# wenet-e2e/wesep

Measured on AMD Instinct MI355X. Metric: utterances/sec (4 s, 16 kHz, 2-spk) fwd+bwd, pBSRNN, higher is better.
Workload: dtype bf16x3+fp16x2+fp16x1 split products (+fp8 lo terms), fp32 accumulate; 1 GPU; pBSRNN FiLM multi-fuse, 6 repeats, feature_dim 128, fixed 256-d embeddings; fwd + SI-SDR + bwd + per-tensor clip + Adam-L2; bf16x3 (x-projections, projections, d(hcat), BN / mask GEMMs) + fp16x2 (recurrent products of all four recurrence kernels, d(xn)) + fp16x1 (LSTM weight gradients); 2-byte saved gates / d(gates); fp32 accumulate; BPTT kernels: W_hh as fp16 hi + block-scaled FP8 lo; the lo term; rows_per_gpu=32, global_rows=32, samples_per_row=64000, parallelism=dp1

## Files before the change

### include/wesep_hip.h

```cpp
#ifndef WESEP_HIP_H_
#define WESEP_HIP_H_

#ifdef __cplusplus
extern "C" {
#endif

#define WS_ABI_VERSION 20
#define WS_OK 0
#define WS_ERR_INVALID (-1)
#define WS_ERR_LAUNCH (-2)

int ws_abi_version(void);
const char* ws_last_error(void);

#define WS_PROF_LSTM_FWD 0
#define WS_PROF_LSTM_BWD 1
#define WS_PROF_GEMM_NT 2
#define WS_PROF_GEMM_TN 3
#define WS_PROF_NKINDS 4
int ws_prof_enable(int on);
int ws_prof_collect(int kind, double* total_ms, long long* launches);
int ws_debug_dirty_lds(float value, int nblocks, int spins, float* sink, void* stream);
int ws_debug_occupy(int nblocks, int usec, const unsigned* stop, float* sink, void* stream);

// ... 28 lines not shown
  const float* stats;
  const float* gamma;
  const float* beta;
  const ws_group_nt* groups;
  long long a_s1, a_s2, c_s1, c_s2, st_m1, st_m2, st_base;
  int a_div, c_div, st_div1, st_div2;
  int M, N, K, ldw;
  int act, ngroups, max_n, vec;
  ws_conv_view conv;
} ws_gemm_nt_args;
int ws_gemm_nt(const ws_gemm_nt_args* a, void* stream);

typedef struct ws_group_tn {
  const float* gamma;
  const float* beta;
  long long g_off, a_off, st_base, out_off, bout_off;
  int Nn, Kk, pad0_, pad1_;
} ws_group_tn;

typedef struct ws_gemm_tn_args {
  const float* G;
  const float* A;
  float* slab;
  float* bslab;
  const float* stats;
  const float* gamma;
  const float* beta;
  const ws_group_tn* groups;
  long long g_s1, g_s2, a_s1, a_s2, st_m1, st_m2, st_base;
  long long slab_stride, bslab_stride, out_off, bout_off;
  int g_div, a_div, st_div1, st_div2;
  int M, Nn, Kk, rows_per_split, nsplit;
  int shift_rows, seq_div, seq_len;
  int ngroups, max_n, max_k, vec;
  ws_conv_view conv;
} ws_gemm_tn_args;
int ws_gemm_tn(const ws_gemm_tn_args* a, void* stream);

typedef struct ws_conv_wgrad_args {
  const float* G;
  const float* X;
  float* slab;
  float* bslab;
  long long ldg, slab_stride, bslab_stride;
  int M, Nn, nsplit, tiles_per_split;
  ws_conv_view conv;
} ws_conv_wgrad_args;
int ws_conv_wgrad(const ws_conv_wgrad_args* a, void* stream);

int ws_reduce_slabs(const float* slab, int nsplit, long long stride, long long count,
                    float* out, int w, long long ldo, void* stream);

int ws_transpose(const float* src, int rows, int cols, long long lds, float* dst, void* stream);

typedef struct ws_groups_geom {
  const int* band_w;
  const int* band_off;
  long long gs1, gs2, rs;
  int ngroups, gdiv, L, W;
  int nbands, pad_;
} ws_groups_geom;
int ws_group_stats(const float* x, const ws_groups_geom* geo, float eps, float* stats, void* stream);
int ws_group_stats_len(const float* x, const ws_groups_geom* geo, const int* glen, int glen_div, float eps, float* stats,
                       void* stream);

int ws_gn_bwd_reduce(const float* x, const float* dxn, const float* stats, const float* gamma,
                     const float* const* gamma_tab, const ws_groups_geom* geo, float* ab,
                     void* stream);
int ws_gn_bwd_apply(const float* x, const float* dxn, const float* stats, const float* ab,
                    const float* gamma, const float* const* gamma_tab, const float* res,
                    const ws_groups_geom* geo, float* dx, void* stream);
int ws_gn_param_grad(const float* x, const float* dxn, const float* stats,
                     const ws_groups_geom* geo, int nsplit, float* slab, void* stream);

int ws_gn_bwd_fused(const float* x, const float* dxn, const float* stats, const float* gamma,
                    const float* res, const ws_groups_geom* geo, int nwg, float* dx, float* pslab,
                    float* pout, unsigned* counter, void* stream);
int ws_gn_bwd_fused2(const float* x, const float* dxn, const float* dxn2, const float* stats, const float* gamma,
                     const float* res, const ws_groups_geom* geo, int nwg, float* dx, float* pslab,
                     float* pout, unsigned* counter, void* stream);
int ws_gn_bwd_apply_pg(const float* x, const float* dxn, const float* stats, const float* ab,
                       const float* gamma, const float* res, const ws_groups_geom* geo, float* dx,
                       float* pslab, float* pout, unsigned* counter, void* stream);

typedef struct ws_lstm_args {
  float* gates;
  float* cbuf;
  float* hcat;
  const float* dhcat;
  const float* wpack;
  long long sq_s1, sq_s2, step_rows;
  int nseq, sq_div, L, mode;
  const unsigned* run_if;
  const float* gates_in;
  float* dgates;
  int gfmt;
  int rfmt;
  const unsigned* amax;
  float* dxn;
  long long dxn_dir_stride;
  const float* wxpack;
} ws_lstm_args;
#define WS_GATES_F32 0
#define WS_GATES_H2 1
#define WS_GATES_H2S 2
#define WS_GATES_H2F 3
#define WS_DGATES_EXP 8
#define WS_LSTM_F32_MT1 1
#define WS_LSTM_F32_MT2 2
#define WS_LSTM_BF16X3 3
#define WS_LSTM_BF16X3_BLK 4
#define WS_LSTM_BF16X3_BLK16 5
#define WS_LSTM_H 256
#define WS_LSTM_FWD_H2P 16
#define WS_LSTM_PACK_FLOATS (2 * 4 * WS_LSTM_H * WS_LSTM_H)
int ws_lstm_pack(const float* whh_f, const float* whh_r, float* pack_fwd, float* pack_bwd,
                 int mode, void* stream);
int ws_lstm_pack_bwd_f8(const float* whh_f, const float* whh_r, float* pack_bwd, void* stream);
#define WS_LSTM_DX_PACK_FLOATS (16 * (48 * 1024 + 64) / 4)
int ws_lstm_pack_dx_f8(const float* wcat, float* pack, void* stream);
int ws_lstm_fwd(const ws_lstm_args* a, void* stream);
int ws_lstm_bwd(const ws_lstm_args* a, void* stream);
typedef struct ws_lstm_cluster_args {
  float* gates;
  float* cbuf;
  float* hcat;
  const float* dhcat;
  const float* whh_f;
  const float* whh_r;
  void* xchg;
  unsigned* flags;
  unsigned* status;
  int nseq, L;
  int dbg, gfmt;
  const float* gates_in;
} ws_lstm_cluster_args;
int ws_lstm_fwd_cluster(const ws_lstm_cluster_args* a, void* stream);
typedef struct ws_lstm_cluster2_args {
  float* gates;
  float* cbuf;
  float* hcat;
  const float* xn;
  const float* wcat;
  const float* bcat;
  const float* whh_f;
  const float* whh_r;
  void* xchg;
  unsigned* tword;
  unsigned* status;
  int nseq, L;
  int dbg, rfmt;
  float* dbg_buf;
} ws_lstm_cluster2_args;
int ws_lstm_fwd_cluster2(const ws_lstm_cluster2_args* a, void* stream);
int ws_lstm_bwd_cluster(const ws_lstm_cluster_args* a, void* stream);
typedef struct ws_lstm_pair_args {
  float* gates;
  const float* cbuf;
  const float* dhcat;
  const float* wpack;
  void* xchg;
  unsigned* flags;
  unsigned* status;
  float* dbg_buf;
  int nseq, L;
  int dbg, gfmt;
  float* dgates;
  const unsigned* amax;
  int rfmt, pad_;
} ws_lstm_pair_args;
int ws_lstm_pack_pair(const float* whh_f, const float* whh_r, float* pack, void* stream);
int ws_lstm_pack_pair_f16(const float* whh_f, const float* whh_r, float* pack, void* stream);
int ws_lstm_pack_pair_f8(const float* whh_f, const float* whh_r, float* pack, void* stream);
int ws_lstm_pack_pair_f8mx(const float* whh_f, const float* whh_r, float* pack, void* stream);
int ws_lstm_bwd_pair(const ws_lstm_pair_args* a, void* stream);
int ws_lstm_cat_ih(const float* wih_f, const float* wih_r, const float* bih_f, const float* bhh_f,
                   const float* bih_r, const float* bhh_r, int n_in, float* wcat, float* bcat,
                   void* stream);

typedef struct ws_seqmap {
  long long sq_s1, sq_s2, step_rows;
  int nseq, sq_div, L;
  int nvalid;
} ws_seqmap;

int ws_pack_w(const float* W, int N, int K, long long ldw, int trans, int order, float* out,
              void* stream);
int ws_pack_w_f16(const float* W, int N, int K, long long ldw, int trans, int order, float* out,
                  void* stream);
int ws_pack_w_f16f8(const float* W, int N, int K, long long ldw, int trans, float* out, void* stream);

typedef struct ws_gemm_p2b_args {
  const float* A;
  const float* Wpack;
  const float* bias;
  float* C;
  float* A_bl;
  const float* stats;
  const float* gamma;
  const float* beta;
  ws_seqmap sm;
  long long lda, st_m1, st_m2, st_base;
  int st_div1, st_div2, N, K;
  const unsigned* run_if;
  unsigned* amax;
  void* A_bl16;
} ws_gemm_p2b_args;
int ws_gemm_p2b(const ws_gemm_p2b_args* a, void* stream);
int ws_gemm_p2b_len(const ws_gemm_p2b_args* a, const int* steps, int steps_div, void* stream);

typedef struct ws_gemm_b2p_args {
  const float* A;
  const float* Wpack;
  const float* bias;
  const float* R;
  float* C;
  ws_seqmap sm;
  long long ldc;
  int N, K;
  int a_fmt, pad_;
  const unsigned* amax;
  void* a16_out;
} ws_gemm_b2p_args;
int ws_gemm_b2p(const ws_gemm_b2p_args* a, void* stream);

typedef struct ws_gemm_tnb_args {
  const float* G;
  const float* A0;
  const float* A1;
  float* slab;
  float* bslab;
  float* aslab;
  long long slab_stride, bslab_stride, aslab_stride;
  int g_width, g_off, g_cols;
  int a0_width, a0_off, a0_cols, a0_shift;
  int a1_width, a1_off, a1_cols, a1_shift;
  int nblk, L, nsplit, blocks_per_split;
  int g_fmt;
  const unsigned* amax;
  int a_fmt, pad_;
} ws_gemm_tnb_args;
int ws_gemm_tnb(const ws_gemm_tnb_args* a, void* stream);
int ws_gemm_tnb_h16(const ws_gemm_tnb_args* a, void* stream);

typedef struct ws_bands {
  const int* band_of_bin;
  const int* band_f0;
  const int* band_bw;
  int nband, nbins;
} ws_bands;
int ws_stft_bandsplit(const float* wav, int R, int T, const ws_bands* b, float* xbs, void* stream);
int ws_stft_bandsplit_len(const float* wav, int R, int T, const int* lengths, const ws_bands* b, float* xbs, void* stream);
int ws_mask_istft_frames(const float* xbs, const float* mask3, int R, int Tf, const ws_bands* b,
                         float* frames, void* stream);
int ws_istft_ola(const float* frames, int R, int Tf, int T, float* wav, void* stream);
int ws_istft_ola_len(const float* frames, int R, int Tf, int T, const int* lengths, float* wav, void* stream);
int ws_mask_istft_bwd(const float* dwav, const float* xbs, const float* mask3, int R, int Tf,
                      int T, const ws_bands* b, float* dmask3, void* stream);

int ws_affine_fwd(const float* z, const float* a, const float* b, float a0, long long rows,
                  int rows_per_r, int N, float* out, void* stream);
int ws_affine_bwd(const float* dz, const float* z_in, const float* a, float a0, long long rows,
                  int rows_per_r, int N, int nsplit, float* dz_in, float* da_slab, float* db_slab,
                  float* da, float* db, unsigned* counter, void* stream);

int ws_sisdr_fwd(const float* est, const float* tgt, int R, int T, float eps, float* rowstat,
                 float* loss, void* stream);
int ws_sisdr_bwd(const float* est, const float* tgt, const float* rowstat, const float* gout,
                 int R, int T, float* dest, void* stream);

typedef struct ws_tensor_ref {
  float* param;
  float* grad;
  float* exp_avg;
  float* exp_avg_sq;
  long long numel;
} ws_tensor_ref;
int ws_grad_norms(const ws_tensor_ref* tab, int ntensors, float* norms, unsigned* guard, void* stream);
int ws_guard_commit(unsigned* guard, const unsigned* skip1, void* stream);
int ws_clip_adam_step(const ws_tensor_ref* tab, int ntensors, const float* norms, float clip,
                      float lr, float beta1, float beta2, float eps, float weight_decay, int step,
                      int clip_only, const unsigned* skip0, const unsigned* skip1, const unsigned* step_lag,
                      void* stream);


int ws_flat_stats(const float* x, int ngroups, long long n_per_group, float eps, int nchunk,
                  float* scratch, float* stats, void* stream);
int ws_prelu_fwd(float* x, const float* rb, const float* a, long long rows, int C, int rows_per_r,
                 float* y, void* stream);
int ws_prelu_bwd(const float* pre, const float* dy, const float* a, long long n, float* dx, float* slab,
                 int nslab, void* stream);
int ws_dwconv_fwd(const float* x, const float* stats, const float* gamma, const float* beta,
                  const float* w, const float* b, int R, int Tp, int C, int P, int dil, int st_div,
                  float* y, void* stream);
int ws_dwconv_bwd(const float* dy, const float* x, const float* stats, const float* gamma,
                  const float* beta, const float* w, int R, int Tp, int C, int P, int dil, int st_div,
                  float* dxn, int nsplit, int rows_per_split, float* slab, void* stream);
int ws_dwconv_ex_fwd(const float* x, const float* stats, const float* gamma, const float* beta,
                     const float* w, const float* b, int R, int Tp, int C, int P, int dil, int st_div, int causal,
                     float* y, void* stream);
int ws_dwconv_ex_bwd(const float* dy, const float* x, const float* stats, const float* gamma,
                     const float* beta, const float* w, int R, int Tp, int C, int P, int dil, int st_div, int causal,
                     float* dxn, int nsplit, int rows_per_split, float* slab, void* stream);
int ws_chan_sums(const float* g, const float* x, const float* stats, int st_div, int rows_per_group,
                 int ngroups, int nsplit, int C, float* slab, void* stream);
int ws_norm_ab(const float* sums, const float* gamma, int ngroups, int C, long long n_per_group,
               float* ab, void* stream);
// ... 271 lines not shown
```

### wesep_amd/_lib.py

```python
import ctypes as C
import os

import numpy as np
import torch

_HERE = os.path.dirname(os.path.abspath(__file__))
LIB_PATH = os.environ.get("WESEP_HIP_LIB") or os.path.join(_HERE, "libwesep_hip.so")

WS_OK = 0
PROF_LSTM_FWD, PROF_LSTM_BWD, PROF_GEMM_NT, PROF_GEMM_TN = 0, 1, 2, 3
LSTM_H = 256
ABI_VERSION = 20
GATES_F32, GATES_H2, GATES_H2S, GATES_H2F = 0, 1, 2, 3
DGATES_EXP = 8


def dgates_scale(amax_bits: int) -> float:
    e = (int(amax_bits) >> 23) & 0xFF
    return 1.0 if e in (0, 255) else 2.0 ** (min(max(DGATES_EXP + 254 - e, 1), 253) - 127)


LSTM_F32_MT1, LSTM_F32_MT2, LSTM_BF16X3, LSTM_BF16X3_BLK, LSTM_BF16X3_BLK16 = 1, 2, 3, 4, 5
LSTM_FWD_H2P = 16
LSTM_PACK_FLOATS = 2 * 4 * LSTM_H * LSTM_H

_p = C.c_void_p
_ll = C.c_longlong
_i = C.c_int
_f = C.c_float


class ConvView(C.Structure):
    _fields_ = [(n, _i) for n in ("on", "mode", "H", "W", "C", "Ho", "Wo", "k", "sh", "sw", "p", "dil", "ldp")]


class Conv3x3PackSrc(C.Structure):
    _fields_ = [("w", _p), ("s_row", _ll), ("s_col", _ll), ("s_tap", _ll), ("col_off", _i), ("cols", _i)]


class Conv3x3PackArgs(C.Structure):
    _fields_ = [("src", Conv3x3PackSrc * 5), ("out", _p), ("Cin", _i), ("Cout", _i), ("nsrc", _i), ("flip", _i)]


class Conv3x3Args(C.Structure):
    _fields_ = [(n, _p) for n in ("X", "W", "bias", "R", "Y")] + [(n, _ll) for n in ("ldx", "ldw", "ldy")] + \
               [(n, _i) for n in ("B", "H", "Wd", "Cin", "Cout", "pad_")]


class Conv3x3WgradArgs(C.Structure):
    _fields_ = [(n, _p) for n in ("G", "X", "slab", "bslab")] + [(n, _ll) for n in ("ldg", "ldx", "slab_stride", "bslab_stride")] + \
               [(n, _i) for n in ("B", "H", "Wd", "Wx", "sw", "Cin", "Nn", "nsplit", "tiles_per_split", "pad_")]


class HeadsArgs(C.Structure):
    _fields_ = [(n, _p) for n in ("x", "dy", "slope", "gamma", "beta", "y", "stats", "dx", "slab")] + \
               [(n, _ll) for n in ("ldx", "lddx")] + [(n, _i) for n in ("B", "T", "Tp", "Q", "nh", "ch", "nwg")] + \
               [("eps", C.c_float)]


class GemmNTArgs(C.Structure):
    _fields_ = [(n, _p) for n in ("A", "W", "bias", "C", "R", "T", "stats", "gamma", "beta", "groups")] + \
               [(n, _ll) for n in ("a_s1", "a_s2", "c_s1", "c_s2", "st_m1", "st_m2", "st_base")] + \
               [(n, _i) for n in ("a_div", "c_div", "st_div1", "st_div2", "M", "N", "K", "ldw",
                                  "act", "ngroups", "max_n", "vec")] + [("conv", ConvView)]


class GemmTNArgs(C.Structure):
    _fields_ = [(n, _p) for n in ("G", "A", "slab", "bslab", "stats", "gamma", "beta", "groups")] + \
               [(n, _ll) for n in ("g_s1", "g_s2", "a_s1", "a_s2", "st_m1", "st_m2", "st_base",
                                   "slab_stride", "bslab_stride", "out_off", "bout_off")] + \
               [(n, _i) for n in ("g_div", "a_div", "st_div1", "st_div2", "M", "Nn", "Kk",
                                  "rows_per_split", "nsplit", "shift_rows", "seq_div", "seq_len",
                                  "ngroups", "max_n", "max_k", "vec")] + [("conv", ConvView)]


class ConvWgradArgs(C.Structure):
    _fields_ = [(n, _p) for n in ("G", "X", "slab", "bslab")] + \
               [(n, _ll) for n in ("ldg", "slab_stride", "bslab_stride")] + \
               [(n, _i) for n in ("M", "Nn", "nsplit", "tiles_per_split")] + [("conv", ConvView)]


class GroupsGeom(C.Structure):
    _fields_ = [("band_w", _p), ("band_off", _p), ("gs1", _ll), ("gs2", _ll), ("rs", _ll),
                ("ngroups", _i), ("gdiv", _i), ("L", _i), ("W", _i), ("nbands", _i), ("pad_", _i)]


class LstmArgs(C.Structure):
    _fields_ = [(n, _p) for n in ("gates", "cbuf", "hcat", "dhcat", "wpack")] + \
               [(n, _ll) for n in ("sq_s1", "sq_s2", "step_rows")] + \
               [(n, _i) for n in ("nseq", "sq_div", "L", "mode")] + [("run_if", _p)] + \
               [("gates_in", _p), ("dgates", _p), ("gfmt", _i), ("rfmt", _i), ("amax", _p)] + \
               [("dxn", _p), ("dxn_dir_stride", _ll), ("wxpack", _p)]


class SeqMapC(C.Structure):
    _fields_ = [("sq_s1", _ll), ("sq_s2", _ll), ("step_rows", _ll), ("nseq", _i), ("sq_div", _i), ("L", _i), ("nvalid", _i)]


class GemmP2BArgs(C.Structure):
    _fields_ = [(n, _p) for n in ("A", "Wpack", "bias", "C", "A_bl", "stats", "gamma", "beta")] + \
               [("sm", SeqMapC)] + [(n, _ll) for n in ("lda", "st_m1", "st_m2", "st_base")] + \
               [(n, _i) for n in ("st_div1", "st_div2", "N", "K")] + [("run_if", _p), ("amax", _p), ("A_bl16", _p)]


class GemmB2PArgs(C.Structure):
    _fields_ = [(n, _p) for n in ("A", "Wpack", "bias", "R", "C")] + [("sm", SeqMapC), ("ldc", _ll), ("N", _i), ("K", _i),
                                                                         ("a_fmt", _i), ("pad_", _i), ("amax", _p), ("a16_out", _p)]


class GemmTNBArgs(C.Structure):
    _fields_ = [(n, _p) for n in ("G", "A0", "A1", "slab", "bslab", "aslab")] + \
               [(n, _ll) for n in ("slab_stride", "bslab_stride", "aslab_stride")] + \
               [(n, _i) for n in ("g_width", "g_off", "g_cols", "a0_width", "a0_off", "a0_cols", "a0_shift",
                                  "a1_width", "a1_off", "a1_cols", "a1_shift", "nblk", "L", "nsplit",
                                  "blocks_per_split", "g_fmt")] + [("amax", _p), ("a_fmt", _i), ("pad_", _i)]


class LstmClusterArgs(C.Structure):
    _fields_ = [(n, _p) for n in ("gates", "cbuf", "hcat", "dhcat", "whh_f", "whh_r", "xchg", "flags", "status")] + \
               [("nseq", _i), ("L", _i), ("dbg", _i), ("gfmt", _i), ("gates_in", _p)]


class LstmCluster2Args(C.Structure):
    _fields_ = [(n, _p) for n in ("gates", "cbuf", "hcat", "xn", "wcat", "bcat", "whh_f", "whh_r", "xchg", "tword", "status")] + \
               [("nseq", _i), ("L", _i), ("dbg", _i), ("rfmt", _i), ("dbg_buf", _p)]


class LstmPairArgs(C.Structure):
    _fields_ = [(n, _p) for n in ("gates", "cbuf", "dhcat", "wpack", "xchg", "flags", "status", "dbg_buf")] + \
               [("nseq", _i), ("L", _i), ("dbg", _i), ("gfmt", _i), ("dgates", _p), ("amax", _p), ("rfmt", _i), ("pad_", _i)]


class Bands(C.Structure):
    _fields_ = [("band_of_bin", _p), ("band_f0", _p), ("band_bw", _p), ("nband", _i), ("nbins", _i)]


GROUP_NT_DTYPE = np.dtype([("W", "<u8"), ("bias", "<u8"), ("gamma", "<u8"), ("beta", "<u8"),
                           ("a_off", "<i8"), ("c_off", "<i8"), ("st_base", "<i8"),
                           ("K", "<i4"), ("N", "<i4"), ("ldw", "<i4"), ("pad_", "<i4")])
GROUP_TN_DTYPE = np.dtype([("gamma", "<u8"), ("beta", "<u8"), ("g_off", "<i8"), ("a_off", "<i8"),
                           ("st_base", "<i8"), ("out_off", "<i8"), ("bout_off", "<i8"),
                           ("Nn", "<i4"), ("Kk", "<i4"), ("pad0_", "<i4"), ("pad1_", "<i4")])
TENSOR_REF_DTYPE = np.dtype([("param", "<u8"), ("grad", "<u8"), ("exp_avg", "<u8"),
                             ("exp_avg_sq", "<u8"), ("numel", "<i8")])
assert GROUP_NT_DTYPE.itemsize == 72 and GROUP_TN_DTYPE.itemsize == 72 and TENSOR_REF_DTYPE.itemsize == 40

class LstmFusedArgs(C.Structure):
    _fields_ = [("gates", _p), ("cbuf", _p), ("hcat", _p), ("xn", _p), ("wpack", _p), ("bias", _p),
                ("nseq", _i), ("L", _i), ("gfmt", _i), ("hfmt", _i)]


LSTM_FUSED_PACK_FLOATS = 2 * 8 * 24 * 4 * 2 * 64 * 4
LSTM_DX_PACK_FLOATS = 16 * (48 * 1024 + 64) // 4

_SIGS = {
    "ws_abi_version": (_i, []),
    "ws_last_error": (C.c_char_p, []),
    "ws_prof_enable": (_i, [_i]),
    "ws_prof_collect": (_i, [_i, C.POINTER(C.c_double), C.POINTER(_ll)]),
    "ws_debug_dirty_lds": (_i, [_f, _i, _i, _p, _p]),
    "ws_debug_occupy": (_i, [_i, _i, _p, _p, _p]),
    "ws_pack_w_f16": (_i, [_p, _i, _i, _ll, _i, _i, _p, _p]),
    "ws_pack_w_f16f8": (_i, [_p, _i, _i, _ll, _i, _p, _p]),
    "ws_gemm_nt": (_i, [C.POINTER(GemmNTArgs), _p]),
    "ws_gemm_tn": (_i, [C.POINTER(GemmTNArgs), _p]),
    "ws_reduce_slabs": (_i, [_p, _i, _ll, _ll, _p, _i, _ll, _p]),
    "ws_transpose": (_i, [_p, _i, _i, _ll, _p, _p]),
    "ws_group_stats": (_i, [_p, C.POINTER(GroupsGeom), _f, _p, _p]),
    "ws_group_stats_len": (_i, [_p, C.POINTER(GroupsGeom), _p, _i, _f, _p, _p]),
    "ws_gn_bwd_reduce": (_i, [_p, _p, _p, _p, _p, C.POINTER(GroupsGeom), _p, _p]),
    "ws_gn_bwd_apply": (_i, [_p, _p, _p, _p, _p, _p, _p, C.POINTER(GroupsGeom), _p, _p]),
    "ws_gn_param_grad": (_i, [_p, _p, _p, C.POINTER(GroupsGeom), _i, _p, _p]),
    "ws_gn_bwd_fused": (_i, [_p, _p, _p, _p, _p, C.POINTER(GroupsGeom), _i, _p, _p, _p, _p, _p]),
    "ws_gn_bwd_fused2": (_i, [_p, _p, _p, _p, _p, _p, C.POINTER(GroupsGeom), _i, _p, _p, _p, _p, _p]),
    "ws_gn_bwd_apply_pg": (_i, [_p, _p, _p, _p, _p, _p, C.POINTER(GroupsGeom), _p, _p, _p, _p, _p]),
    "ws_lstm_pack": (_i, [_p, _p, _p, _p, _i, _p]),
    "ws_lstm_fwd": (_i, [C.POINTER(LstmArgs), _p]),
    "ws_lstm_bwd": (_i, [C.POINTER(LstmArgs), _p]),
    "ws_lstm_fwd_cluster": (_i, [C.POINTER(LstmClusterArgs), _p]),
    "ws_lstm_bwd_cluster": (_i, [C.POINTER(LstmClusterArgs), _p]),
    "ws_lstm_fwd_cluster2": (_i, [C.POINTER(LstmCluster2Args), _p]),
    "ws_lstm_pack_pair": (_i, [_p, _p, _p, _p]),
    "ws_lstm_pack_pair_f16": (_i, [_p, _p, _p, _p]),
    "ws_lstm_pack_pair_f8": (_i, [_p, _p, _p, _p]),
    "ws_lstm_pack_pair_f8mx": (_i, [_p, _p, _p, _p]),
    "ws_lstm_pack_bwd_f8": (_i, [_p, _p, _p, _p]),
    "ws_lstm_pack_dx_f8": (_i, [_p, _p, _p]),
    "ws_lstm_bwd_pair": (_i, [C.POINTER(LstmPairArgs), _p]),
    "ws_lstm_cat_ih": (_i, [_p, _p, _p, _p, _p, _p, _i, _p, _p, _p]),
    "ws_pack_w": (_i, [_p, _i, _i, _ll, _i, _i, _p, _p]),
    "ws_gemm_p2b": (_i, [C.POINTER(GemmP2BArgs), _p]),
    "ws_gemm_p2b_len": (_i, [C.POINTER(GemmP2BArgs), _p, _i, _p]),
    "ws_gemm_b2p": (_i, [C.POINTER(GemmB2PArgs), _p]),
    "ws_gemm_tnb": (_i, [C.POINTER(GemmTNBArgs), _p]),
    "ws_gemm_tnb_h16": (_i, [C.POINTER(GemmTNBArgs), _p]),
    "ws_stft_bandsplit": (_i, [_p, _i, _i, C.POINTER(Bands), _p, _p]),
    "ws_stft_bandsplit_len": (_i, [_p, _i, _i, _p, C.POINTER(Bands), _p, _p]),
    "ws_mask_istft_frames": (_i, [_p, _p, _i, _i, C.POINTER(Bands), _p, _p]),
    "ws_istft_ola": (_i, [_p, _i, _i, _i, _p, _p]),
    "ws_istft_ola_len": (_i, [_p, _i, _i, _i, _p, _p, _p]),
    "ws_mask_istft_bwd": (_i, [_p, _p, _p, _i, _i, _i, C.POINTER(Bands), _p, _p]),
    "ws_affine_fwd": (_i, [_p, _p, _p, _f, _ll, _i, _i, _p, _p]),
    "ws_affine_bwd": (_i, [_p, _p, _p, _f, _ll, _i, _i, _i, _p, _p, _p, _p, _p, _p, _p]),
    "ws_sisdr_fwd": (_i, [_p, _p, _i, _i, _f, _p, _p, _p]),
    "ws_sisdr_bwd": (_i, [_p, _p, _p, _p, _i, _i, _p, _p]),
    "ws_flat_stats": (_i, [_p, _i, _ll, C.c_float, _i, _p, _p, _p]),
    "ws_prelu_fwd": (_i, [_p, _p, _p, _ll, _i, _i, _p, _p]),
    "ws_prelu_bwd": (_i, [_p, _p, _p, _ll, _p, _p, _i, _p]),
    "ws_dwconv_fwd": (_i, [_p, _p, _p, _p, _p, _p, _i, _i, _i, _i, _i, _i, _p, _p]),
    "ws_dwconv_bwd": (_i, [_p, _p, _p, _p, _p, _p, _i, _i, _i, _i, _i, _i, _p, _i, _i, _p, _p]),
    "ws_dwconv_ex_fwd": (_i, [_p, _p, _p, _p, _p, _p, _i, _i, _i, _i, _i, _i, _i, _p, _p]),
    "ws_dwconv_ex_bwd": (_i, [_p, _p, _p, _p, _p, _p, _i, _i, _i, _i, _i, _i, _i, _p, _i, _i, _p, _p]),
    "ws_chan_sums": (_i, [_p, _p, _p, _i, _i, _i, _i, _i, _p, _p]),
    "ws_norm_ab": (_i, [_p, _p, _i, _i, _ll, _p, _p]),
    "ws_norm_bwd_apply_cl": (_i, [_p, _p, _p, _p, _p, _p, _ll, _i, _i, _p, _p]),
    "ws_maskmul_fwd": (_i, [_p, _ll, _p, _ll, _i, _p, _p]),
    "ws_maskmul_bwd": (_i, [_p, _p, _ll, _p, _ll, _i, _p, _ll, _p, _p]),
    "ws_relu_mask": (_i, [_p, _p, _ll, _p]),
    "ws_ola_fwd": (_i, [_p, _p, _i, _i, _i, _i, _i, _p, _p]),
    "ws_ola_bwd": (_i, [_p, _i, _i, _i, _i, _i, _p, _p]),
    "ws_sum_partial": (_i, [_p, _ll, _p, _i, _p]),
    "ws_bn_stats": (_i, [_p, _ll, _i, C.c_float, C.c_float, _p, _p, _i, _p, _p, _p]),
    "ws_bn_prelu_fwd": (_i, [_p, _p, _p, _p, _p, _p, _ll, _i, _p, _p, _p]),
    "ws_bn_bwd": (_i, [_p, _p, _p, _p, _ll, _i, _i, _p, _p, _p, _p]),
    "ws_maxpool3_fwd": (_i, [_p, _i, _i, _i, _p, _p]),
    "ws_maxpool3_bwd": (_i, [_p, _p, _i, _i, _i, _p, _p]),
    "ws_bcast_rows": (_i, [_p, C.c_float, _i, _ll, _i, _p, _p]),
    "ws_cross_entropy": (_i, [_p, _p, _i, _i, _p, _p, _p]),
    "ws_im2col": (_i, [_p, _i, _i, _i, _i, _i, _i, _i, _ll, _p, _p]),
    "ws_col2im": (_i, [_p, _i, _i, _i, _i, _i, _i, _i, _p, _p]),
    "ws_conv_wgrad": (_i, [C.POINTER(ConvWgradArgs), _p]),
    "ws_astp_fwd": (_i, [_p, _p, _i, _i, _i, C.c_float, _p, _p, _p]),
    "ws_astp_bwd": (_i, [_p, _p, _p, _p, _p, _i, _i, _i, C.c_float, _p, _p, _p]),
    "ws_mhastp_sizes": (_i, [_i, _i, _i, _i, _i, _i, _i, _p, _p]),
    "ws_mhastp_pack": (_i, [_p, _p, _p, _p, _i, _i, _i, _i, _p, _p]),
    "ws_mhastp_fwd": (_i, [_p, _p, _i, _i, _i, _i, _i, _i, _i, _i, _p, _p, _p]),
    "ws_mhastp_bwd": (_i, [_p, _p, _p, _p, _i, _i, _i, _i, _i, _i, _i, _i, _p, _p, _p, _i, _p, _p]),
    "ws_mhastp_split_sizes": (_i, [_i, _i, _i, _i, _i, _i, _i, _p, _p]),
    "ws_mhastp_fwd_split": (_i, [_p, _p, _i, _i, _i, _i, _i, _i, _i, _i, _i, _p, _p, _p, _p]),
    "ws_mhastp_bwd_split": (_i, [_p, _p, _p, _p, _i, _i, _i, _i, _i, _i, _i, _i, _i, _p, _p, _p, _i, _p, _p]),
    "ws_rowbias_act_fwd": (_i, [_p, _p, _ll, _i, _i, _i, _p, _p]),
    "ws_act_bwd": (_i, [_p, _p, _ll, _i, _p, _p]),
    "ws_seg_sums": (_i, [_p, _p, _i, _i, _i, _i, _p, _p]),
    "ws_seg_scale": (_i, [_p, _p, _i, _i, _i, _i, _p, _p]),
    "ws_tstp_fwd": (_i, [_p, _i, _i, _i, _i, C.c_float, _p, _p]),
    "ws_tstp_bwd": (_i, [_p, _p, _p, _i, _i, _i, _i, _p, _p]),
    "ws_im2col_hw": (_i, [_p, _i, _i, _i, _i, _i, _i, _i, _i, _ll, _p, _p]),
    "ws_col2im_hw": (_i, [_p, _i, _i, _i, _i, _i, _i, _i, _i, _p, _p]),
    "ws_elu_fwd": (_i, [_p, _ll, _p, _p]),
    "ws_elu_bwd": (_i, [_p, _p, _ll, _p, _p]),
    "ws_inorm_finalize": (_i, [_p, _i, _i, _ll, C.c_float, _p, _p]),
    "ws_inorm_apply": (_i, [_p, _p, _ll, _i, _i, _p, _p]),
    "ws_inorm_bwd_apply": (_i, [_p, _p, _p, _p, _ll, _i, _i, _p, _p]),
    "ws_avgpool_fwd": (_i, [_p, _i, _i, _i, _i, _i, _p, _p]),
    "ws_avgpool_bwd": (_i, [_p, _i, _i, _i, _i, _i, _p, _p]),
    "ws_bilinear_fwd": (_i, [_p, _i, _i, _i, _i, _i, _i, _p, _p]),
    "ws_bilinear_bwd": (_i, [_p, _i, _i, _i, _i, _i, _i, _p, _p, _p]),
    "ws_scale_bf_fwd": (_i, [_p, _p, _i, _i, _i, _i, _i, _p, _p]),
    "ws_freq_linear_fwd": (_i, [_p, _p, _ll, _p, _i, _i, _i, _i, _p, _p]),
    "ws_scale_bf_bwd": (_i, [_p, _p, _p, _i, _i, _i, _i, _i, _p, _p, _p]),
    "ws_softmax_rows_fwd": (_i, [_p, _ll, _i, C.c_float, _p, _p]),
    "ws_softmax_rows_bwd": (_i, [_p, _p, _ll, _i, C.c_float, _p, _p]),
    "ws_heads_fwd": (_i, [C.POINTER(HeadsArgs), _p]),
    "ws_heads_bwd": (_i, [C.POINTER(HeadsArgs), _p]),
    "ws_conv3x3": (_i, [C.POINTER(Conv3x3Args), _p]),
    "ws_conv3x3_pack": (_i, [C.POINTER(Conv3x3PackArgs), _p]),
    "ws_conv3x3_wgrad": (_i, [C.POINTER(Conv3x3WgradArgs), _p]),
    "ws_in_act_sums": (_i, [_p, _p, _ll, _p, _i, _i, _i, _i, _i, _p, _p]),
    "ws_in_act_apply": (_i, [_p, _p, _ll, _i, _i, _i, _p, _ll, _p]),
    "ws_in_act_bwd_apply": (_i, [_p, _p, _ll, _p, _p, _ll, _i, _i, _i, _p, _ll, _p]),
    "ws_rowln_grid": (_i, [_ll, _i]),
    "ws_rowln_fwd": (_i, [_p, _p, _p, _ll, _i, C.c_float, _p, _p, _p]),
    "ws_rowln_bwd": (_i, [_p, _p, _p, _p, _p, _ll, _i, _p, _p, _p]),
    "ws_preemph_pad": (_i, [_p, _i, _i, _i, _i, C.c_float, _p, _p]),
    "ws_power_spec": (_i, [_p, _ll, _i, _i, _i, _p, _p]),
    "ws_log_eps": (_i, [_p, _ll, C.c_float, _p]),
# ... 101 lines not shown
```

### wesep_amd/blstm_core.py

```python
import math
import os
from typing import NamedTuple

import numpy as np
import torch

from . import _lib as L
from . import dev

H = L.LSTM_H
G4 = 4 * H
N = 128


def _empty(dev_, *shape):
    return torch.empty(*shape, device=dev_, dtype=torch.float32)


def _reduce_new(slab, nsplit, stride, shape):
    out = _empty(slab.device, *shape)
    dev.reduce_slabs(slab, nsplit, stride, int(np.prod(shape)), out)
    return out


# ... 282 lines not shown
            return pack
        if kind in ("hhp", "hhp16"):
            pack = _empty(d, L.LSTM_PACK_FLOATS)
            dev.lstm_pack_pair(*W("whh"), pack, f16=pair_rf if kind == "hhp16" else 0)
            return pack
        if kind in ("fused", "fused16", "fused8"):
            fpack = _empty(d, L.LSTM_FUSED_PACK_FLOATS)
            dev.lstm_pack_fused(wih_f.contiguous(), wih_r.contiguous(), *W("whh"), fpack,
                                hfmt={"fused": 0, "fused16": 1, "fused8": 5}[kind])
            return fpack
        if kind == "wih":
            out = _empty(d, 2 * G4 * N)
            dev.pack_w(W("cat")[0], 2 * G4, N, N, out, order=0)
            return out
        if kind in ("wihT", "wihT16", "wihT8"):
            out = _empty(d, N * 2 * G4)
            dev.pack_w(W("cat")[0], N, 2 * G4, N, out, trans=True, order=1, f16={"wihT": 0, "wihT16": 1, "wihT8": 2}[kind])
            return out
        if kind == "pw":
            return proj_w.contiguous()
        if kind in ("proj", "proj16"):
            out = _empty(d, N * 2 * H)
            dev.pack_w(W("pw"), N, 2 * H, 2 * H, out, order=1, f16=kind == "proj16")
            return out
        if kind == "projT":
            out = _empty(d, 2 * H * N)
            dev.pack_w(W("pw"), 2 * H, N, 2 * H, out, trans=True, order=0)
            return out
        raise KeyError(kind)


class BlstmPlan(NamedTuple):
    nb: int
    lmode: int
    cluster: bool
    fwd: str
    bptt: str
    grad: bool
    gfmt: int
    g_fmt: int
    a16: bool
    pair_rfmt: int
    band_rfmt: int
    band_dx: bool
    a_fmt: int
    h2p: bool = False


_WIHT_KIND = {0: "wihT", 1: "wihT", 2: "wihT16", 3: "wihT8"}


def make_plan(seq, device, grad, gn_geo=None, ragged=False) -> BlstmPlan:
    lmode = dev.lstm_blk_mode(seq.nseq)
    cluster = dev.lstm_cluster_ok(seq, device)
    bptt = _bptt_kind(seq, device, cluster)
    gfmt = L.GATES_F32 if bptt == "cluster" else dev.gates_fmt()
    h2 = gfmt != L.GATES_F32
    if ragged:
        fwd = "cluster" if cluster else "stream"
    elif dev.lstm_fuse_ok(seq.nseq, cluster):
        fwd = "fused"
    elif cluster:
        fwd = "cluster2" if h2 and dev.lstm_cluster2_on() else "cluster"
    else:
        fwd = "stream"
    g_fmt = {L.GATES_H2: 1, L.GATES_H2F: 2}.get(gfmt, 0)
    brf = band_rfmt(gfmt, lmode) if grad and bptt == "stream" else 0
    a16 = gfmt == L.GATES_H2F and grad and tnb_a16()
    h2p = (a16 and dev.h2p_on(device) and not ragged and fwd in ("fused", "cluster2", "stream")
           and (fwd != "fused" or bool(dev.lstm_fused_hfmt(gfmt) & 1)))
    return BlstmPlan(
        nb=dev.bl_num_blocks(seq), lmode=lmode, cluster=cluster, fwd=fwd, bptt=bptt, grad=grad, gfmt=gfmt, g_fmt=g_fmt,
        a16=a16, pair_rfmt=pair_rfmt(gfmt) if grad and bptt == "pair" else 0,
        band_rfmt=brf, band_dx=bool(brf) and gn_geo is not None and band_dx(brf, seq, gn_geo), a_fmt=dxn_fmt(g_fmt), h2p=h2p)


def consume_once(ctx, who):
    if ctx.consumed:
        raise L.WesepHipError(f"{who}: second backward through the same graph (retain_graph / multi-loss loops): "
                              "the blocked path consumes its saved gates in place; run the forward again")
    ctx.consumed = True


def blstm_forward(plan, W, x, seq, res, bias, norm=None, steps=None):
    d = x.device
    norm = norm or {}
    if steps is not None and (plan.fwd in ("fused", "cluster2") or plan.grad):
        raise L.WesepHipError(f"blstm_forward: per-sequence step counts with forward branch '{plan.fwd}', grad={plan.grad}: "
                              "only the branches over precomputed gates know them, and only the forward")
    lens = dict(steps=steps[0], steps_div=steps[1]) if steps is not None else {}
    nb, gfmt, lmode = plan.nb, plan.gfmt, plan.lmode
    h2 = gfmt != L.GATES_F32
    wcat, bcat = W("cat")
    whf, whr = W("whh")
    xn = _empty(d, nb, 32 * N)
    cbuf, hcat = _empty(d, nb, 32 * 2 * H), _empty(d, nb, 32 * 2 * H)
    gates = _empty(d, dev.blh_floats(nb, 2 * G4)) if h2 else _empty(d, nb, 32 * 2 * G4)
    xn16 = _empty(d, dev.blh_floats(nb, N)) if plan.a16 else None
    h2p = plan.h2p
    planes = dict(h2p=True) if h2p else {}
    hcat16 = _empty(d, dev.blh_floats(nb, 2 * H)) if plan.a16 and not h2p else None
    if plan.fwd == "fused":
        dev.gemm_p2b(A=x, lda=N, sm=seq, Wpack=None, N=0, C_out=None, A_bl=xn, A_bl16=xn16, **norm)
        hf = dev.lstm_fused_hfmt(gfmt)
        dev.lstm_fwd_fused(gates, cbuf, hcat, xn, W("fused8" if hf & 4 else "fused16" if hf else "fused"), bcat, seq, gfmt=gfmt,
                           hfmt=hf | (8 if h2p else 0))
    elif plan.fwd == "cluster2":
        dev.gemm_p2b(A=x, lda=N, sm=seq, Wpack=None, N=0, C_out=None, A_bl=xn, A_bl16=xn16, **norm)
        tw = dev.lstm_fwd_cluster2(gates, cbuf, hcat, xn, wcat, bcat, whf, whr, seq, dbg=_cluster_dbg(), **planes)
        pre = dev.fallback_scratch(d, nb * 32 * 2 * G4)
        dev.gemm_p2b(A=x, lda=N, sm=seq, Wpack=W("wih"), N=2 * G4, C_out=pre, bias=bcat, run_if=tw, **norm)
        dev.lstm_fwd(gates, cbuf, hcat, W("hh")[0], seq, lmode, run_if=tw, gfmt=gfmt, gates_in=pre, **planes)
        del pre
    else:
        pre = _empty(d, nb, 32 * 2 * G4) if h2 else gates
        xproj = dict(A=x, lda=N, sm=seq, Wpack=W("wih"), N=2 * G4, C_out=pre, bias=bcat, A_bl=xn, A_bl16=xn16, **norm, **lens)
        rec = dict(gfmt=gfmt, gates_in=pre) if h2 else {}
        dev.gemm_p2b(**xproj)
        if _h2_probe() & 768 and not torch.cuda.is_available():
            pre.copy_(pre.half().float() if _h2_probe() & 256 else pre.bfloat16().float())
        if plan.fwd == "cluster":
            tw = dev.lstm_fwd_cluster(gates, cbuf, hcat, whf, whr, seq, dbg=_cluster_dbg(), **rec)
            if not h2:
                dev.gemm_p2b(run_if=tw, **xproj)
            dev.lstm_fwd(gates, cbuf, hcat, W("hh")[0], seq, lmode, run_if=tw, **rec)
        else:
            dev.lstm_fwd(gates, cbuf, hcat, W("hh")[0], seq, lmode, **planes, **rec)
        del pre
    out = torch.empty_like(res)
    if h2p:
        dev.gemm_b2p(A=hcat, K=2 * H, sm=seq, Wpack=W("proj16"), C_out=out, ldc=N, bias=bias, R=res, a_fmt=4)
    else:
        dev.gemm_b2p(A=hcat, K=2 * H, sm=seq, Wpack=W("proj"), C_out=out, ldc=N, bias=bias, R=res, a16_out=hcat16)
    if _h2_probe() and not h2:
        if _h2_probe() & 1:
            _probe_round(gates, "f16")
        if _h2_probe() & 8:
            _probe_round(gates, "u16")
        if _h2_probe() & 4:
            _probe_round(cbuf, "f16")
    if plan.grad:
        W("projT")
        if not plan.band_dx:
            W(_WIHT_KIND[plan.a_fmt])
        if plan.bptt == "pair":
            W("hhp16" if plan.pair_rfmt else "hhp")
        if (plan.bptt == "stream" and not plan.band_rfmt) or (plan.bptt == "pair" and h2):
            W("hh")
        if plan.bptt == "stream" and plan.band_rfmt:
            W("hh8")
            if plan.band_dx:
                W("wx8")
    return out, (gates, cbuf, hcat, xn16 if plan.a16 else xn, hcat16)


def blstm_bptt(plan, W, gates, cbuf, hcat, dout, seq, release):
    d = dout.device
    nb, gfmt = plan.nb, plan.gfmt
    dh, dout_bl = _empty(d, nb, 32 * 2 * H), _empty(d, nb, 32 * N)
    dxn2 = None
    amax = amax_word(d) if gfmt == L.GATES_H2F else None
    dev.gemm_p2b(A=dout, lda=N, sm=seq, Wpack=W("projT"), N=2 * H, C_out=dh, A_bl=dout_bl, amax=amax)
    if _h2_probe() & 16:
        _probe_round(dh, "bf16")
    ready = mark_wgrads_ready(d) if release else None
    if plan.bptt == "cluster":
        dg = gates
        dev.lstm_bwd_cluster(gates, cbuf, dh, *W("whh"), seq)
    elif gfmt == L.GATES_F32:
        dg = gates
        if plan.bptt == "pair":
            dev.lstm_bwd_pair(gates, cbuf, dh, W("hhp"), seq, dbg=_pair_dbg())
        else:
            dev.lstm_bwd(gates, cbuf, hcat, dh, W("hh")[1], seq, plan.lmode)
    elif plan.bptt == "pair":
        dg = _empty(d, nb, 32 * 2 * G4) if gfmt == L.GATES_H2S else _empty(d, dev.blh_floats(nb, 2 * G4))
        rf = plan.pair_rfmt
        tw = dev.lstm_bwd_pair(gates, cbuf, dh, W("hhp16" if rf else "hhp"), seq, gfmt=gfmt, dgates=dg, repairable=True,
                               dbg=_pair_dbg(), amax=amax, rfmt=rf, dbg_buf=_pair_stamp_buf(d, seq.L))
        dev.lstm_bwd(gates, cbuf, hcat, dh, W("hh")[1], seq, plan.lmode, gfmt=gfmt, dgates=dg, run_if=tw, amax=amax)
    else:
        dg = _empty(d, nb, 32 * 2 * G4) if gfmt == L.GATES_H2S else gates
        brf = plan.band_rfmt
        if plan.band_dx:
            dxn2 = _empty(d, 2, dout.numel() // N, N)
        dev.lstm_bwd(gates, cbuf, hcat, dh, W("hh8") if brf else W("hh")[1], seq, plan.lmode, gfmt=gfmt,
                     dgates=dg if gfmt == L.GATES_H2S else None, amax=amax, rfmt=brf, dxn=dxn2,
                     wxpack=W("wx8") if dxn2 is not None else None)
    if _h2_probe() & 2 and gfmt == L.GATES_F32:
        _probe_round(gates, "bf16", packed=True)
    if _h2_probe() & 32 and gfmt == L.GATES_F32 and not torch.cuda.is_available():
        amax = float(dh.abs().max())
        S = 2.0 ** (10 - math.floor(math.log2(amax))) if amax > 0 and math.isfinite(amax) else 1.0
        sc = gates * S
        _PROBE_SAT[0] += int((sc.abs() > 65504.0).sum())
        _PROBE_SAT[1] = max(_PROBE_SAT[1], float(sc.abs().max()) / 65504.0)
        gates.copy_(sc.clamp(-65504.0, 65504.0).half().float() / S)
    if ready is not None:
        flush_deferred_wgrads(d, ready)
    return dg, dout_bl, amax, dxn2


def weight_grads(gates, xn, hcat, dout_bl, seq, nb, g_fmt=0, amax=None, hcat16=None, h2p=False):
    d = gates.device
    if h2p:
        hcat16 = dev.h2p_hi(hcat, nb)
    a_fmt = 1 if hcat16 is not None else 0
    if _h2_probe() & 192 and not torch.cuda.is_available() and not a_fmt:
        rnd = (lambda t: t.half().float()) if _h2_probe() & 64 else (lambda t: t.bfloat16().float())
        xn, hcat = rnd(xn), rnd(hcat)
    if os.environ.get("WESEP_PROBE_SKIP_WGRAD") == "1":
        z_ = lambda *s_: torch.zeros(*s_, device=d)
        return [z_(G4, N), z_(G4, H), z_(G4), z_(G4), z_(G4, N), z_(G4, H), z_(G4), z_(G4), z_(N, 2 * H), z_(N)]
    if _h2_probe() & 1024 and not torch.cuda.is_available() and amax is not None:
        S = L.dgates_scale(int(amax.reshape(-1)[0]))
        hcat = hcat.half().float()
# ... 50 lines not shown
```

### wesep_amd/csrc/common.h

```cpp
#pragma once
#include <hip/hip_runtime.h>
#include <stdint.h>

#include "../../include/wesep_hip.h"

typedef float f32x4 __attribute__((ext_vector_type(4)));
typedef float f32x16 __attribute__((ext_vector_type(16)));

#define WS_WAVE 64

#define WS_SEL_LO16 0x05040100u
#define WS_SEL_HI16 0x07060302u

void ws_set_error(const char* fmt, ...);
int ws_check_launch(const char* what);

#define WS_REQUIRE(cond, ...)            \
  do {                                   \
    if (!(cond)) {                       \
      ws_set_error(__VA_ARGS__);         \
      return WS_ERR_INVALID;             \
    }                                    \
  } while (0)

void ws_prof_begin(int kind, hipStream_t s);
void ws_prof_end(int kind, hipStream_t s);

int ws_launch_gemm_nt_bf16(const ws_gemm_nt_args* a, dim3 grid, hipStream_t s);
int ws_launch_gemm_tn_bf16(const ws_gemm_tn_args* a, dim3 grid, hipStream_t s);

int ws_launch_lstm_pack_bf16(const float* whh_f, const float* whh_r, float* pack_fwd, float* pack_bwd,
                             hipStream_t s);
int ws_launch_lstm_fwd_bf16(const ws_lstm_args* a, hipStream_t s);
int ws_launch_lstm_bwd_bf16(const ws_lstm_args* a, hipStream_t s);
int ws_launch_lstm_pack_s16(const float* whh_f, const float* whh_r, float* pack_fwd, float* pack_bwd,
                            hipStream_t s);
int ws_launch_lstm_fwd_s16(const ws_lstm_args* a, hipStream_t s);
int ws_launch_lstm_bwd_s16(const ws_lstm_args* a, hipStream_t s);

__device__ __forceinline__ float ws_wave_sum(float v) {
#pragma unroll
  for (int o = 32; o > 0; o >>= 1) v += __shfl_xor(v, o, 64);
  return v;
}

__device__ __forceinline__ float ws_block_sum(float v, float* red) {
  v = ws_wave_sum(v);
  const int lane = threadIdx.x & 63, w = threadIdx.x >> 6, nw = blockDim.x >> 6;
  __syncthreads();
  if (lane == 0) red[w] = v;
  __syncthreads();
  float t = 0.f;
  for (int i = 0; i < nw; ++i) t += red[i];
  return t;
}

__device__ __forceinline__ float ws_dgates_scale(unsigned amax_bits) {
  const int e = (int)((amax_bits >> 23) & 0xffu);
  if (e == 0 || e == 255) return 1.f;
  const int se = min(max(WS_DGATES_EXP + 254 - e, 1), 253);
  return __uint_as_float((unsigned)se << 23);
}
__device__ __forceinline__ float ws_dgates_scale_inv(unsigned amax_bits) {
  const float s = ws_dgates_scale(amax_bits);
  return __uint_as_float((unsigned)(254 - (int)(__float_as_uint(s) >> 23)) << 23);
}

__device__ __forceinline__ void ws_st_agent(float* p, float v) {
  __hip_atomic_store(p, v, __ATOMIC_RELAXED, __HIP_MEMORY_SCOPE_AGENT);
}
__device__ __forceinline__ float ws_ld_agent(const float* p) {
  return __hip_atomic_load(p, __ATOMIC_RELAXED, __HIP_MEMORY_SCOPE_AGENT);
}

#if defined(__HIP_DEVICE_COMPILE__) && !defined(__gfx942__) && !defined(__gfx950__)
#error "ws_last_block / ws_tree_sum256 rely on gfx942 / gfx950 memory ordering (vmcnt tracks stores; sc1 = write-through)"
#endif
__device__ __forceinline__ bool ws_last_block(unsigned* counter, unsigned nblocks) {
  __shared__ unsigned last_s;
  asm volatile("s_waitcnt vmcnt(0)" ::: "memory");
  __syncthreads();
  if (threadIdx.x == 0) {
    const unsigned t = __hip_atomic_fetch_add(counter, 1u, __ATOMIC_RELAXED, __HIP_MEMORY_SCOPE_AGENT);
    last_s = t == nblocks - 1u;
    if (last_s) __hip_atomic_store(counter, 0u, __ATOMIC_RELAXED, __HIP_MEMORY_SCOPE_AGENT);
  }
  __syncthreads();
  return last_s != 0u;
}

__device__ __forceinline__ void ws_tree_sum256(float* pslab, unsigned nblocks, float* pout, unsigned* counters) {
  const unsigned grp = blockIdx.x >> 5, ngrp = (nblocks + 31u) >> 5;
  const unsigned in_grp = min(32u, nblocks - grp * 32u);
  if (!ws_last_block(counters + 1 + grp, in_grp)) return;
  float t = 0.f;
  for (unsigned k = 0; k < in_grp; ++k) t += ws_ld_agent(pslab + (long long)(grp * 32u + k) * 256 + threadIdx.x);
  ws_st_agent(pslab + (long long)(nblocks + grp) * 256 + threadIdx.x, t);
  if (!ws_last_block(counters, ngrp)) return;
  float s = 0.f;
  for (unsigned g = 0; g < ngrp; ++g) s += ws_ld_agent(pslab + (long long)(nblocks + g) * 256 + threadIdx.x);
  pout[threadIdx.x] = s;
}

__device__ __forceinline__ float ws_sigmoid(float x) { return 1.f / (1.f + expf(-x)); }

__device__ __forceinline__ long long ws_row_off(int m, int div, long long s1, long long s2) {
  const int q = m / div;
  return (long long)q * s1 + (long long)(m - q * div) * s2;
}
```

### wesep_amd/csrc/elementwise.hip

```cpp
#include "common.h"

__global__ void affine_fwd_kernel(const float* z, const float* __restrict__ a,
                                  const float* __restrict__ b, float a0, long long rows,
                                  int rows_per_r, int N, float* out) {
  const long long total4 = rows * N / 4;
  const int n4 = N / 4;
  for (long long i = blockIdx.x * (long long)blockDim.x + threadIdx.x; i < total4;
       i += (long long)gridDim.x * blockDim.x) {
    const long long row = i / n4;
    const int c = (int)(i - row * n4) * 4;
    const int r = (int)(row / rows_per_r);
    f32x4 v = *reinterpret_cast<const f32x4*>(z + i * 4);
    f32x4 av = {a0, a0, a0, a0}, bv = {0.f, 0.f, 0.f, 0.f};
    if (a) av += *reinterpret_cast<const f32x4*>(a + (long long)r * N + c);
    if (b) bv = *reinterpret_cast<const f32x4*>(b + (long long)r * N + c);
    *reinterpret_cast<f32x4*>(out + i * 4) = v * av + bv;
  }
}

extern "C" int ws_affine_fwd(const float* z, const float* a, const float* b, float a0,
                             long long rows, int rows_per_r, int N, float* out, void* stream) {
  WS_REQUIRE(z && out && rows > 0 && rows_per_r > 0 && N > 0 && N % 4 == 0, "ws_affine_fwd: bad args");
  long long blocks = (rows * N / 4 + 255) / 256;
  if (blocks > 16384) blocks = 16384;
  hipLaunchKernelGGL(affine_fwd_kernel, dim3((unsigned)blocks), dim3(256), 0, (hipStream_t)stream,
                     z, a, b, a0, rows, rows_per_r, N, out);
  return ws_check_launch("ws_affine_fwd");
}

__global__ __launch_bounds__(256) void affine_bwd_kernel(
    const float* __restrict__ dz, const float* __restrict__ z_in, const float* __restrict__ a,
    float a0, int rows_per_r, int N, int nsplit, float* __restrict__ dz_in,
    float* __restrict__ da_slab, float* __restrict__ db_slab, float* __restrict__ da, float* __restrict__ db,
    unsigned* counter) {
  __shared__ float sh[2][128];
  const int r = blockIdx.x, split = blockIdx.y, R = gridDim.x;
  const int col = threadIdx.x & 127, rl = threadIdx.x >> 7;
  float sa = 0.f, sb = 0.f;
  if (col < N) {
    const float scale = a0 + (a ? a[(long long)r * N + col] : 0.f);
    const int chunk = (rows_per_r + nsplit - 1) / nsplit;
    const int lo = split * chunk, hi = min(rows_per_r, lo + chunk);
    for (int j = lo + rl; j < hi; j += 2) {
      const long long o = ((long long)r * rows_per_r + j) * N + col;
      const float g = dz[o];
      if (da_slab) sa += g * z_in[o];
      sb += g;
      if (dz_in) dz_in[o] = g * scale;
    }
  }
  if (rl == 1) {
    sh[0][col] = sa;
    sh[1][col] = sb;
  }
  __syncthreads();
  if (rl == 0 && col < N) {
    const long long o = ((long long)split * R + r) * N + col;
    if (counter) {
      if (da_slab) ws_st_agent(da_slab + o, sa + sh[0][col]);
      if (db_slab) ws_st_agent(db_slab + o, sb + sh[1][col]);
    } else {
      if (da_slab) da_slab[o] = sa + sh[0][col];
      if (db_slab) db_slab[o] = sb + sh[1][col];
    }
  }
  if (counter && ws_last_block(counter + r, (unsigned)nsplit)) {
    float* dst = rl == 0 ? da : db;
    const float* src = rl == 0 ? da_slab : db_slab;
    if (dst && col < N) {
      float t = 0.f;
      for (int k = 0; k < nsplit; ++k) t += ws_ld_agent(src + ((long long)k * R + r) * N + col);
      dst[(long long)r * N + col] = t;
    }
  }
}

__global__ __launch_bounds__(256) void affine_bwd4_kernel(
    const float* __restrict__ dz, const float* __restrict__ z_in, const float* __restrict__ a,
    float a0, int rows_per_r, int N, int nsplit, float* __restrict__ dz_in,
    float* __restrict__ da_slab, float* __restrict__ db_slab, float* __restrict__ da, float* __restrict__ db,
    unsigned* counter) {
  __shared__ f32x4 sh[2][8][32];
  const int r = blockIdx.x, split = blockIdx.y, R = gridDim.x;
  const int c4 = threadIdx.x & 31, rl = threadIdx.x >> 5;
  f32x4 sa = {0.f, 0.f, 0.f, 0.f}, sb = {0.f, 0.f, 0.f, 0.f};
  const bool live = 4 * c4 < N;
  if (live) {
    f32x4 scale = {a0, a0, a0, a0};
    if (a) scale += *reinterpret_cast<const f32x4*>(a + (long long)r * N + 4 * c4);
    const int chunk = (rows_per_r + nsplit - 1) / nsplit;
    const int lo = split * chunk, hi = min(rows_per_r, lo + chunk);
    const long long base = (long long)r * rows_per_r * N + 4 * c4;
    for (int j = lo + rl; j < hi; j += 16) {
      const bool two = j + 8 < hi;
      const long long o0 = base + (long long)j * N, o1 = base + (long long)(two ? j + 8 : j) * N;
      const f32x4 g0 = *reinterpret_cast<const f32x4*>(dz + o0);
      f32x4 g1 = *reinterpret_cast<const f32x4*>(dz + o1);
      if (da_slab) {
        const f32x4 z0 = *reinterpret_cast<const f32x4*>(z_in + o0);
// ... 253 lines not shown
```

### wesep_amd/csrc/gemm_blk.hip

```cpp
#include <stdlib.h>

#include <type_traits>

#include "common.h"

typedef __bf16 bf16x8 __attribute__((ext_vector_type(8)));
typedef unsigned int u32x4 __attribute__((ext_vector_type(4)));
typedef unsigned int u32x2 __attribute__((ext_vector_type(2)));
typedef float f32x2 __attribute__((ext_vector_type(2)));
typedef _Float16 f16x8 __attribute__((ext_vector_type(8)));
typedef _Float16 f16x2 __attribute__((ext_vector_type(2)));
typedef int i32x4 __attribute__((ext_vector_type(4)));
typedef int v8i __attribute__((ext_vector_type(8)));
typedef __fp16 h16x2 __attribute__((ext_vector_type(2)));

__device__ __forceinline__ f32x16 mfma32(bf16x8 a, bf16x8 b, f32x16 c) {
  return __builtin_amdgcn_mfma_f32_32x32x16_bf16(a, b, c, 0, 0, 0);
}

__device__ __forceinline__ void split8(const float* v, bf16x8& hi, bf16x8& lo) {
#pragma unroll
  for (int j = 0; j < 8; ++j) {
    hi[j] = (__bf16)v[j];
    lo[j] = (__bf16)(v[j] - (float)hi[j]);
// ... 78 lines not shown
  if (order == 0) {
    ks = r % nks;
    nt = r / nks;
  } else {
    nt = r % nnt;
    ks = r / nnt;
  }
  const int n = 32 * nt + (lane & 31), k0 = 16 * ks + 8 * (lane >> 5);
  f16x8 hi, lo;
#pragma unroll
  for (int j = 0; j < 8; ++j) {
    const float v = WS_PACK16_SCALE * (trans ? W[(long long)(k0 + j) * ldw + n] : W[(long long)n * ldw + k0 + j]);
    hi[j] = (_Float16)v;
    lo[j] = (_Float16)(v - (float)hi[j]);
  }
  const long long u = (order == 0 ? ((long long)nt * nks + ks) : ((long long)ks * nnt + nt)) * 2;
  f16x8* o = reinterpret_cast<f16x8*>(out);
  o[u * 64 + lane] = hi;
  o[(u + 1) * 64 + lane] = lo;
}

extern "C" int ws_pack_w_f16(const float* W, int N, int K, long long ldw, int trans, int order, float* out,
                             void* stream) {
  WS_REQUIRE(W && out && N > 0 && K > 0 && N % 32 == 0 && K % 16 == 0, "ws_pack_w_f16: N %% 32, K %% 16 (N=%d K=%d)", N, K);
  WS_REQUIRE(order == 0 || order == 1, "ws_pack_w_f16: order");
  hipLaunchKernelGGL(pack_w16_kernel, dim3((N * K / 8 + 255) / 256), dim3(256), 0, (hipStream_t)stream, W, N, K, ldw,
                     trans, order, reinterpret_cast<_Float16*>(out));
  return ws_check_launch("ws_pack_w_f16");
}

__global__ __launch_bounds__(256) void pack_w16f8_kernel(const float* __restrict__ W, int K, long long ldw, int trans,
                                                         unsigned char* __restrict__ out) {
  const int st = blockIdx.x, nt = threadIdx.x >> 6, lane = threadIdx.x & 63, n = 32 * nt + (lane & 31);
  unsigned char* sb = out + (long long)st * 24576;
  float res[32];
  float mx = 0.f;
#pragma unroll
  for (int i = 0; i < 4; ++i) {
    f16x8 hi;
#pragma unroll
    for (int j = 0; j < 8; ++j) {
      const int k = 64 * st + 16 * i + 8 * (lane >> 5) + j;
      const float v = WS_PACK16_SCALE * (trans ? W[(long long)k * ldw + n] : W[(long long)n * ldw + k]);
      hi[j] = (_Float16)v;
      res[8 * i + j] = v - (float)hi[j];
      mx = fmaxf(mx, fabsf(res[8 * i + j]));
    }
    reinterpret_cast<f16x8*>(sb)[(i * 4 + nt) * 64 + lane] = hi;
  }
#pragma unroll
  for (int o = 32; o >= 1; o >>= 1) mx = fmaxf(mx, __shfl_xor(mx, o));
  int E = mx > 0.f ? ((__float_as_int(mx) >> 23) & 255) - 127 - 7 : 0;
  E = max(E, -126);
  const float inv = __int_as_float((127 - E) << 23);
  unsigned int* o8 = reinterpret_cast<unsigned int*>(sb + 16384 + nt * 2048 + lane * 16);
#pragma unroll
  for (int j = 0; j < 32; j += 4) {
    int c = 0;
    c = __builtin_amdgcn_cvt_pk_fp8_f32(res[j] * inv, res[j + 1] * inv, c, false);
    c = __builtin_amdgcn_cvt_pk_fp8_f32(res[j + 2] * inv, res[j + 3] * inv, c, true);
    o8[(j >> 4) * 256 + ((j & 15) >> 2)] = (unsigned int)c;
  }
  if (lane == 0) (out + (long long)(K / 64) * 24576)[st * 4 + nt] = (unsigned char)(127 + E);
}

extern "C" int ws_pack_w_f16f8(const float* W, int N, int K, long long ldw, int trans, float* out, void* stream) {
  WS_REQUIRE(W && out && N == 128 && K > 0 && K % 64 == 0, "ws_pack_w_f16f8: N = 128, K %% 64 (N=%d K=%d)", N, K);
  hipLaunchKernelGGL(pack_w16f8_kernel, dim3(K / 64), dim3(256), 0, (hipStream_t)stream, W, K, ldw, trans,
                     reinterpret_cast<unsigned char*>(out));
  return ws_check_launch("ws_pack_w_f16f8");
}

extern "C" int ws_pack_w(const float* W, int N, int K, long long ldw, int trans, int order, float* out,
                         void* stream) {
  WS_REQUIRE(W && out && N > 0 && K > 0 && N % 32 == 0 && K % 16 == 0, "ws_pack_w: N %% 32, K %% 16 (N=%d K=%d)",
             N, K);
  WS_REQUIRE(order == 0 || order == 1, "ws_pack_w: order");
  hipLaunchKernelGGL(pack_w_kernel, dim3((N * K / 8 + 255) / 256), dim3(256), 0, (hipStream_t)stream, W, N, K, ldw,
                     trans, order, reinterpret_cast<__bf16*>(out));
  return ws_check_launch("ws_pack_w");
}

#define P2B_K 128
template <bool LEN>
__global__ __launch_bounds__(512, 4) void gemm_p2b_kernel(const ws_gemm_p2b_args p, const int* __restrict__ steps,
                                                          int steps_div) {
  __shared__ __attribute__((aligned(16))) u32x4 wl[2][2048];
  if (p.run_if && *p.run_if == 0u) return;
  const int tid = threadIdx.x, lane = tid & 63, i = lane & 31, half = lane >> 5;
  const int w = __builtin_amdgcn_readfirstlane(tid >> 6);
  const int nblk = ((p.sm.nseq + 31) / 32) * p.sm.L;
  const int b = blockIdx.x * 8 + w;
  const bool active = b < nblk;
  const int bb = active ? b : nblk - 1;
  bool valid;
  const long long pos = seq_pos(p.sm, bb, i, valid);
  if (LEN) {
    const int tile = bb / p.sm.L, step = bb - tile * p.sm.L;
    const int nv = p.sm.nvalid > 0 ? p.sm.nvalid : p.sm.nseq;
    valid = valid && step < steps[min(tile * 32 + i, nv - 1) / steps_div];
  }

  bf16x8 xh[8], xl[8];
  {
    const float* arow = p.A + pos * p.lda;
    float mean = 0.f, rstd = 1.f;
    if (p.stats) {
      const long long s = (pos / p.st_div1) * p.st_m1 + (pos % p.st_div2) * p.st_m2 + p.st_base;
      mean = p.stats[2 * s];
      rstd = p.stats[2 * s + 1];
    }
    float* eb = p.A_bl ? p.A_bl + (long long)bb * (32 * P2B_K) + i * 4 : nullptr;
    unsigned short* eb16 = p.A_bl16 ? reinterpret_cast<unsigned short*>(p.A_bl16) + (long long)bb * (32 * P2B_K) + i * 4 : nullptr;
#pragma unroll
    for (int ks = 0; ks < 8; ++ks) {
      const int k0 = 16 * ks + 8 * half;
      f32x4 v0 = *reinterpret_cast<const f32x4*>(arow + k0);
      f32x4 v1 = *reinterpret_cast<const f32x4*>(arow + k0 + 4);
      if (p.stats) {
        const f32x4 g0 = *reinterpret_cast<const f32x4*>(p.gamma + k0), g1 = *reinterpret_cast<const f32x4*>(p.gamma + k0 + 4);
        const f32x4 b0 = *reinterpret_cast<const f32x4*>(p.beta + k0), b1 = *reinterpret_cast<const f32x4*>(p.beta + k0 + 4);
        v0 = (v0 - mean) * rstd * g0 + b0;
        v1 = (v1 - mean) * rstd * g1 + b1;
      }
      if (!valid) {
        v0 = f32x4{0.f, 0.f, 0.f, 0.f};
        v1 = v0;
      }
      const float v[8] = {v0[0], v0[1], v0[2], v0[3], v1[0], v1[1], v1[2], v1[3]};
      split8(v, xh[ks], xl[ks]);
      if (eb && active) {
        u32x4 c0, c1;
        pack8(xh[ks], xl[ks], c0, c1);
        *reinterpret_cast<u32x4*>(eb + (k0 / 4) * 128) = c0;
        *reinterpret_cast<u32x4*>(eb + (k0 / 4 + 1) * 128) = c1;
      }
      if (eb16 && active) {
        const f16x2 h0 = {(_Float16)v[0], (_Float16)v[1]}, h1 = {(_Float16)v[2], (_Float16)v[3]};
        const f16x2 h2 = {(_Float16)v[4], (_Float16)v[5]}, h3 = {(_Float16)v[6], (_Float16)v[7]};
        *reinterpret_cast<u32x2*>(eb16 + (k0 / 4) * 128) = u32x2{__builtin_bit_cast(unsigned, h0), __builtin_bit_cast(unsigned, h1)};
        *reinterpret_cast<u32x2*>(eb16 + (k0 / 4 + 1) * 128) = u32x2{__builtin_bit_cast(unsigned, h2), __builtin_bit_cast(unsigned, h3)};
      }
    }
  }

  const int nstage = p.N / 64;
  if (nstage == 0) return;
  const u32x4* wsrc = reinterpret_cast<const u32x4*>(p.Wpack);
  u32x4 wreg[4];
#pragma unroll
  for (int q = 0; q < 4; ++q) wreg[q] = wsrc[tid + 512 * q];
#pragma unroll
  for (int q = 0; q < 4; ++q) wl[0][tid + 512 * q] = wreg[q];
  __syncthreads();
  float* cblk = p.C + (long long)bb * 32 * p.N + i * 4;
  float cmax = 0.f;
  for (int st = 0; st < nstage; ++st) {
    const int cur = st & 1;
    if (st + 1 < nstage) {
#pragma unroll
      for (int q = 0; q < 4; ++q) wreg[q] = wsrc[(long long)(st + 1) * 2048 + tid + 512 * q];
    }
#pragma unroll
    for (int t2 = 0; t2 < 2; ++t2) {
      const u32x4* wt = &wl[cur][t2 * 1024 + lane];
      f32x16 acc;
#pragma unroll
      for (int ks = 0; ks < 8; ++ks) {
        const bf16x8 ah = __builtin_bit_cast(bf16x8, wt[(ks * 2) * 64]);
        const bf16x8 al = __builtin_bit_cast(bf16x8, wt[(ks * 2 + 1) * 64]);
        if (ks == 0) {
          const f32x16 zero = {0.f, 0.f, 0.f, 0.f, 0.f, 0.f, 0.f, 0.f, 0.f, 0.f, 0.f, 0.f, 0.f, 0.f, 0.f, 0.f};
          acc = mfma32(ah, xh[ks], zero);
        } else {
          acc = mfma32(ah, xh[ks], acc);
        }
        acc = mfma32(al, xh[ks], acc);
        acc = mfma32(ah, xl[ks], acc);
      }
      if (active) {
        const int n0 = st * 64 + t2 * 32;
#pragma unroll
        for (int j = 0; j < 4; ++j) {
          const int n = n0 + 8 * j + 4 * half;
          f32x4 v = {acc[4 * j], acc[4 * j + 1], acc[4 * j + 2], acc[4 * j + 3]};
          if (p.bias) v += *reinterpret_cast<const f32x4*>(p.bias + n);
          if (!valid) v = f32x4{0.f, 0.f, 0.f, 0.f};
          *reinterpret_cast<f32x4*>(cblk + (n / 4) * 128) = v;
          cmax = fmaxf(fmaxf(cmax, fmaxf(fabsf(v[0]), fabsf(v[1]))), fmaxf(fabsf(v[2]), fabsf(v[3])));
        }
      }
    }
    if (st + 1 < nstage) {
#pragma unroll
      for (int q = 0; q < 4; ++q) wl[cur ^ 1][tid + 512 * q] = wreg[q];
    }
    __syncthreads();
  }
  if (p.amax) {
#pragma unroll
    for (int o = 32; o > 0; o >>= 1) cmax = fmaxf(cmax, __shfl_xor(cmax, o, 64));
    if (lane == 0) atomicMax(p.amax, __float_as_uint(cmax));
  }
}

static int gemm_p2b_launch(const char* who, const ws_gemm_p2b_args* a, const int* steps, int steps_div, void* stream) {
  WS_REQUIRE(a && a->A && ((a->Wpack && a->C) || (a->N == 0 && (a->A_bl || a->A_bl16))), "%s: null pointer", who);
  WS_REQUIRE(a->K == P2B_K, "%s: K must be %d (got %d)", who, P2B_K, a->K);
  WS_REQUIRE(a->N >= 0 && a->N % 64 == 0, "%s: N %% 64 (N=%d)", who, a->N);
  WS_REQUIRE(a->lda >= a->K && a->lda % 4 == 0, "%s: lda", who);
  WS_REQUIRE(a->sm.nseq > 0 && a->sm.L > 0 && a->sm.sq_div > 0, "%s: bad sequence map", who);
  WS_REQUIRE(!a->stats || (a->gamma && a->beta && a->st_div1 > 0 && a->st_div2 > 0), "%s: norm args", who);
  const int nblk = ((a->sm.nseq + 31) / 32) * a->sm.L;
  hipStream_t s = (hipStream_t)stream;
  const bool timed = a->run_if == nullptr;
  if (timed) ws_prof_begin(WS_PROF_GEMM_NT, s);
  if (steps)
    hipLaunchKernelGGL((gemm_p2b_kernel<true>), dim3((nblk + 7) / 8), dim3(512), 0, s, *a, steps, steps_div);
  else
    hipLaunchKernelGGL((gemm_p2b_kernel<false>), dim3((nblk + 7) / 8), dim3(512), 0, s, *a, steps, steps_div);
  if (timed) ws_prof_end(WS_PROF_GEMM_NT, s);
  return ws_check_launch(who);
}

extern "C" int ws_gemm_p2b(const ws_gemm_p2b_args* a, void* stream) {
  return gemm_p2b_launch("ws_gemm_p2b", a, nullptr, 1, stream);
}

extern "C" int ws_gemm_p2b_len(const ws_gemm_p2b_args* a, const int* steps, int steps_div, void* stream) {
  WS_REQUIRE(steps && steps_div > 0, "ws_gemm_p2b_len: steps table / steps_div");
  return gemm_p2b_launch("ws_gemm_p2b_len", a, steps, steps_div, stream);
}

template <int A16>
__global__ __launch_bounds__(512, 4) void gemm_b2p_kernel(const ws_gemm_b2p_args p) {
  __shared__ __attribute__((aligned(16))) u32x4 wl[2][2048];
  __shared__ long long posl[8][32];
  const int tid = threadIdx.x, lane = tid & 63, i = lane & 31, half = lane >> 5;
  const int w = __builtin_amdgcn_readfirstlane(tid >> 6);
  const int nblk = ((p.sm.nseq + 31) / 32) * p.sm.L;
  const int b = blockIdx.x * 8 + w;
  const bool active = b < nblk;
  const int bb = active ? b : nblk - 1;
  {
    bool valid;
    const long long pos = seq_pos(p.sm, bb, i, valid);
    if (half == 0) posl[w][i] = valid ? pos : -1;
  }
  const int K = p.K, nstage = K / 64;
  typedef typename std::conditional<A16 != 0, u32x2, f32x4>::type acell;
  typedef typename std::conditional<A16 != 0, unsigned short, float>::type aelem;
  constexpr int SU = A16 == 3 ? 1536 : 2048, NQ = SU / 512;
  const int* wsc = reinterpret_cast<const int*>(reinterpret_cast<const unsigned char*>(p.Wpack) + (long long)nstage * 24576);
  int sc_n = A16 == 3 ? wsc[0] : 0;
  const float inv_s = A16 == 4 ? 1.f / WS_PACK16_SCALE : A16 >= 2 ? ws_dgates_scale_inv(*p.amax) * (1.f / WS_PACK16_SCALE) : 1.f;
  const long long lo_plane = (long long)nblk * 32 * K;
  const aelem* ab = reinterpret_cast<const aelem*>(p.A) + (long long)bb * 32 * K + i * 4 + 2 * half * 128;
  const __amdgpu_buffer_rsrc_t wsr = __builtin_amdgcn_make_buffer_rsrc(const_cast<float*>(p.Wpack), 0, (unsigned)nstage * SU * 16u,
                                                                        0x00020000);
  auto wstage = [&](int st, int buf) {
#pragma unroll
    for (int q = 0; q < NQ; ++q)
      __builtin_amdgcn_raw_ptr_buffer_load_lds(wsr, (__attribute__((address_space(3))) void*)&wl[buf][(w * NQ + q) * 64], 16, lane * 16,
                                               (st * SU + (w * NQ + q) * 64) * 16, 0, 0);
  };
  constexpr int HS = (A16 == 0 || A16 == 4) ? 2 : 1, KH = 4 / HS;
  constexpr int NP = A16 == 4 ? 2 : 1;
  acell an[NP * 2 * KH];
  auto load_a = [&](int st, int hs) {
    const aelem* a2 = ab + ((long long)st * 16 + hs * KH * 4) * 128;
#pragma unroll
    for (int pl = 0; pl < NP; ++pl)
#pragma unroll
      for (int ks = 0; ks < KH; ++ks) {
        an[pl * 2 * KH + 2 * ks] = *reinterpret_cast<const acell*>(a2 + pl * lo_plane + (4 * ks) * 128);
        an[pl * 2 * KH + 2 * ks + 1] = *reinterpret_cast<const acell*>(a2 + pl * lo_plane + (4 * ks + 1) * 128);
      }
  };
  wstage(0, 0);
  load_a(0, 0);
  asm volatile("s_waitcnt vmcnt(0)" ::: "memory");
  __syncthreads();

  f32x16 acc[4];
#pragma unroll
  for (int t = 0; t < 4; ++t)
#pragma unroll
    for (int r = 0; r < 16; ++r) acc[t][r] = 0.f;

  for (int st = 0; st < nstage; ++st) {
    const int cur = st & 1;
    const int sc = __builtin_amdgcn_readfirstlane(sc_n);
    v8i a8;
#pragma unroll
    for (int hs = 0; hs < HS; ++hs) {
    acell ac[NP * 2 * KH];
#pragma unroll
    for (int q = 0; q < NP * 2 * KH; ++q) ac[q] = an[q];
    if (hs == 0 && st + 1 < nstage) {
      wstage(st + 1, cur ^ 1);
      if constexpr (A16 == 3) sc_n = wsc[st + 1];
    }
    if (hs + 1 < HS) load_a(st, hs + 1);
    else if (st + 1 < nstage) load_a(st + 1, 0);
#pragma unroll
    for (int ksl = 0; ksl < KH; ++ksl) {
      const int ks = hs * KH + ksl;
      bf16x8 ah, al;
      if constexpr (A16 == 1) {
        const u32x2 c0 = __builtin_bit_cast(u32x2, ac[2 * ksl]), c1 = __builtin_bit_cast(u32x2, ac[2 * ksl + 1]);
        ah = __builtin_bit_cast(bf16x8, u32x4{c0[0], c0[1], c1[0], c1[1]});
      } else if constexpr (A16 == 3) {
        const u32x2 c0 = __builtin_bit_cast(u32x2, ac[2 * ksl]), c1 = __builtin_bit_cast(u32x2, ac[2 * ksl + 1]);
        const f16x8 a16 = __builtin_bit_cast(f16x8, u32x4{c0[0], c0[1], c1[0], c1[1]});
        typedef short s16x2 __attribute__((ext_vector_type(2)));
#pragma unroll
        for (int h2 = 0; h2 < 2; ++h2) {
          s16x2 c = {0, 0};
          c = __builtin_amdgcn_cvt_scalef32_pk_fp8_f16(c, f16x2{a16[4 * h2], a16[4 * h2 + 1]}, 256.f, false);
          c = __builtin_amdgcn_cvt_scalef32_pk_fp8_f16(c, f16x2{a16[4 * h2 + 2], a16[4 * h2 + 3]}, 256.f, true);
          a8[2 * ks + h2] = __builtin_bit_cast(int, c);
        }
        const u32x4* wt = &wl[cur][ks * 256 + lane];
#pragma unroll
        for (int nt = 0; nt < 4; ++nt)
          acc[nt] = __builtin_amdgcn_mfma_f32_32x32x16_f16(a16, __builtin_bit_cast(f16x8, wt[nt * 64]), acc[nt], 0, 0, 0);
        if (ks == 3) {
          const u32x4* w8 = &wl[cur][1024 + lane];
          auto frag = [&](int nt) {
            return __builtin_shufflevector(__builtin_bit_cast(i32x4, w8[(2 * nt) * 64]), __builtin_bit_cast(i32x4, w8[(2 * nt + 1) * 64]),
// ... 5 lines not shown
          acc[3] = __builtin_amdgcn_mfma_scale_f32_32x32x64_f8f6f4(a8, frag(3), acc[3], 0, 0, 0, 127 + 8, 3, sc);
        }
        continue;
      } else if constexpr (A16 == 4) {
        const u32x2 c0 = __builtin_bit_cast(u32x2, ac[2 * ksl]), c1 = __builtin_bit_cast(u32x2, ac[2 * ksl + 1]);
        const u32x2 l0 = __builtin_bit_cast(u32x2, ac[2 * KH + 2 * ksl]), l1 = __builtin_bit_cast(u32x2, ac[2 * KH + 2 * ksl + 1]);
        const f16x8 a_hi = __builtin_bit_cast(f16x8, u32x4{c0[0], c0[1], c1[0], c1[1]});
        const f16x8 a_lo = __builtin_bit_cast(f16x8, u32x4{l0[0], l0[1], l1[0], l1[1]});
        const u32x4* wt = &wl[cur][ks * 512 + lane];
#pragma unroll
        for (int nt = 0; nt < 4; ++nt) {
          const f16x8 w_hi = __builtin_bit_cast(f16x8, wt[(nt * 2) * 64]);
          acc[nt] = __builtin_amdgcn_mfma_f32_32x32x16_f16(a_hi, w_hi, acc[nt], 0, 0, 0);
          acc[nt] = __builtin_amdgcn_mfma_f32_32x32x16_f16(a_hi, __builtin_bit_cast(f16x8, wt[(nt * 2 + 1) * 64]), acc[nt], 0, 0, 0);
          acc[nt] = __builtin_amdgcn_mfma_f32_32x32x16_f16(a_lo, w_hi, acc[nt], 0, 0, 0);
        }
        continue;
      } else if constexpr (A16 == 2) {
        const u32x2 c0 = __builtin_bit_cast(u32x2, ac[2 * ksl]), c1 = __builtin_bit_cast(u32x2, ac[2 * ksl + 1]);
        const f16x8 a16 = __builtin_bit_cast(f16x8, u32x4{c0[0], c0[1], c1[0], c1[1]});
        const u32x4* wt = &wl[cur][ks * 512 + lane];
#pragma unroll
        for (int nt = 0; nt < 4; ++nt) {
          acc[nt] = __builtin_amdgcn_mfma_f32_32x32x16_f16(a16, __builtin_bit_cast(f16x8, wt[(nt * 2) * 64]), acc[nt], 0, 0, 0);
          acc[nt] = __builtin_amdgcn_mfma_f32_32x32x16_f16(a16, __builtin_bit_cast(f16x8, wt[(nt * 2 + 1) * 64]), acc[nt], 0, 0, 0);
        }
        continue;
      } else {
        unpack8(__builtin_bit_cast(u32x4, ac[2 * ksl]), __builtin_bit_cast(u32x4, ac[2 * ksl + 1]), ah, al);
        if (p.a16_out && active) {
          unsigned short* o16 = reinterpret_cast<unsigned short*>(p.a16_out) + (long long)bb * 32 * K + i * 4 +
                                (long long)(st * 16 + 4 * ks + 2 * half) * 128;
#pragma unroll
          for (int c = 0; c < 2; ++c) {
            const u32x4 cell = __builtin_bit_cast(u32x4, ac[2 * ksl + c]);
            _Float16 h[4];
#pragma unroll
            for (int j = 0; j < 4; ++j)
              h[j] = (_Float16)(__uint_as_float(cell[j] & 0xffff0000u) + __uint_as_float(cell[j] << 16));
            const f16x2 p0 = {h[0], h[1]}, p1 = {h[2], h[3]};
            *reinterpret_cast<u32x2*>(o16 + c * 128) = u32x2{__builtin_bit_cast(unsigned, p0), __builtin_bit_cast(unsigned, p1)};
          }
        }
      }
      const u32x4* wt = &wl[cur][ks * 512 + lane];
#pragma unroll
      for (int nt = 0; nt < 4; ++nt) {
        const bf16x8 bh = __builtin_bit_cast(bf16x8, wt[(nt * 2) * 64]);
        const bf16x8 bl = __builtin_bit_cast(bf16x8, wt[(nt * 2 + 1) * 64]);
        acc[nt] = mfma32(ah, bh, acc[nt]);
        if constexpr (A16 != 1) acc[nt] = mfma32(al, bh, acc[nt]);
        acc[nt] = mfma32(ah, bl, acc[nt]);
      }
    }
    }
    asm volatile("s_waitcnt vmcnt(0)" ::: "memory");
    __syncthreads();
  }

  float* stg = reinterpret_cast<float*>(&wl[0][0]) + w * 2048;
#pragma unroll
  for (int pass = 0; pass < 2; ++pass) {
#pragma unroll
    for (int t = 0; t < 2; ++t) {
      const int nt = 2 * pass + t;
      const float bv = p.bias ? p.bias[nt * 32 + i] : 0.f;
#pragma unroll
      for (int r = 0; r < 16; ++r) {
        const int m = (r & 3) + 8 * (r >> 2) + 4 * half;
        stg[m * 64 + t * 32 + i] = (A16 >= 2 ? acc[nt][r] * inv_s : acc[nt][r]) + bv;
      }
    }
    __syncthreads();
    const int c4 = lane & 15, r0 = lane >> 4;
    f32x4 v[8];
    long long off[8];
#pragma unroll
    for (int k = 0; k < 8; ++k) {
      const int m = r0 + 4 * k;
      const long long pos = posl[w][m];
      off[k] = (active && pos >= 0) ? pos * p.ldc + pass * 64 + 4 * c4 : -1;
      v[k] = *reinterpret_cast<const f32x4*>(stg + m * 64 + 4 * c4);
    }
    if (p.R) {
#pragma unroll
      for (int k = 0; k < 8; ++k)
        if (off[k] >= 0) v[k] += *reinterpret_cast<const f32x4*>(p.R + off[k]);
    }
#pragma unroll
    for (int k = 0; k < 8; ++k)
      if (off[k] >= 0) *reinterpret_cast<f32x4*>(p.C + off[k]) = v[k];
    __syncthreads();
  }
}

extern "C" int ws_gemm_b2p(const ws_gemm_b2p_args* a, void* stream) {
  WS_REQUIRE(a && a->A && a->Wpack && a->C, "ws_gemm_b2p: null pointer");
  WS_REQUIRE(a->N == 128, "ws_gemm_b2p: N must be 128 (got %d)", a->N);
  WS_REQUIRE(a->a_fmt >= 0 && a->a_fmt <= 4 && (a->a_fmt < 2 || a->a_fmt == 4 || a->amax), "ws_gemm_b2p: a_fmt %d (2 / 3 need amax)",
             a->a_fmt);
  WS_REQUIRE(a->a_fmt == 0 || !a->a16_out, "ws_gemm_b2p: a16_out goes with a_fmt 0 (got a_fmt %d)", a->a_fmt);
  WS_REQUIRE(a->K > 0 && a->K % 64 == 0, "ws_gemm_b2p: K %% 64 (K=%d)", a->K);
  WS_REQUIRE(a->ldc >= a->N && a->ldc % 4 == 0, "ws_gemm_b2p: ldc >= N and ldc %% 4 == 0 (16-byte row pieces)");
  WS_REQUIRE(a->sm.nseq > 0 && a->sm.L > 0 && a->sm.sq_div > 0, "ws_gemm_b2p: bad sequence map");
  const int nblk = ((a->sm.nseq + 31) / 32) * a->sm.L;
  hipStream_t s = (hipStream_t)stream;
  ws_prof_begin(WS_PROF_GEMM_NT, s);
  if (a->a_fmt == 4)
    hipLaunchKernelGGL(gemm_b2p_kernel<4>, dim3((nblk + 7) / 8), dim3(512), 0, s, *a);
  else if (a->a_fmt == 3)
    hipLaunchKernelGGL(gemm_b2p_kernel<3>, dim3((nblk + 7) / 8), dim3(512), 0, s, *a);
  else if (a->a_fmt == 2)
    hipLaunchKernelGGL(gemm_b2p_kernel<2>, dim3((nblk + 7) / 8), dim3(512), 0, s, *a);
  else if (a->a_fmt == 1)
    hipLaunchKernelGGL(gemm_b2p_kernel<1>, dim3((nblk + 7) / 8), dim3(512), 0, s, *a);
  else
    hipLaunchKernelGGL(gemm_b2p_kernel<0>, dim3((nblk + 7) / 8), dim3(512), 0, s, *a);
  ws_prof_end(WS_PROF_GEMM_NT, s);
  return ws_check_launch("ws_gemm_b2p");
}

typedef __bf16 bf16x4 __attribute__((ext_vector_type(4)));
#define TB_LD 40

typedef __bf16 bf16x2 __attribute__((ext_vector_type(2)));

template <int TA, bool ASUM>
__global__ __launch_bounds__(512, 2) void gemm_tnb_kernel(const ws_gemm_tnb_args p) {
  constexpr int NCOL = 128 * (1 + TA);
  constexpr int PLANE = NCOL * TB_LD;
  constexpr int NG = (1 + TA) / 2;
  constexpr int TN = TA == 1 ? 1 : TA;
  __shared__ __attribute__((aligned(16))) __bf16 ldsA[2 * PLANE];
  __shared__ __attribute__((aligned(16))) __bf16 ldsB[2 * PLANE];
  const int tid = threadIdx.x, lane = tid & 63, l31 = lane & 31, half = lane >> 5;
  const int w = __builtin_amdgcn_readfirstlane(tid >> 6);
  const int wm = w >> 2, wn = w & 3;
  const int gt = blockIdx.y, split = blockIdx.x;
  const int L = p.L;
  const int b_begin = split * p.blocks_per_split;
  const int b_end = min(p.nblk, b_begin + p.blocks_per_split);

  const float* gbase[NG];
  long long gstride[NG];
  int gshift[NG], gcol[NG];
#pragma unroll
  for (int r = 0; r < NG; ++r) {
    const int g = tid + 512 * r;
    const int part = g >> 8, quad = (g >> 3) & 31, sg = g & 7;
    gcol[r] = part * 128 + 4 * quad;
    if (part == 0) {
      gbase[r] = p.G + (long long)((p.g_off + gt * 128) / 4 + quad) * 128 + sg * 16;
      gstride[r] = 32LL * p.g_width;
      gshift[r] = 0;
    } else {
      const int c0 = (part - 1) * 128;
      const bool s1 = c0 >= p.a0_cols;
      const float* base = s1 ? p.A1 : p.A0;
      const int off = s1 ? p.a1_off + c0 - p.a0_cols : p.a0_off + c0;
      gbase[r] = base + (long long)(off / 4 + quad) * 128 + sg * 16;
      gstride[r] = 32LL * (s1 ? p.a1_width : p.a0_width);
      gshift[r] = s1 ? p.a1_shift : p.a0_shift;
    }
  }
  const int sg = tid & 7;

  f32x4 rq[2][NG][4];
  bool use[2][NG];
  auto load_block = [&](int b, int slot) {
    const int tile = b / L, step = b - tile * L;
#pragma unroll
    for (int r = 0; r < NG; ++r) {
      const int sa = step + gshift[r];
      use[slot][r] = sa >= 0 && sa < L;
      const float* src = gbase[r] + (long long)(use[slot][r] ? b + gshift[r] : b) * gstride[r];
#pragma unroll
      for (int j = 0; j < 4; ++j) rq[slot][r][j] = *reinterpret_cast<const f32x4*>(src + 4 * j);
    }
  };
  float csum[NG][4];
#pragma unroll
  for (int r = 0; r < NG; ++r)
#pragma unroll
    for (int c = 0; c < 4; ++c) csum[r][c] = 0.f;
  auto store_piece = [&](int slot, __bf16* lds, unsigned live, int pc) {
    const int r = pc >> 2, c = pc & 3;
    unsigned e[4];
#pragma unroll
    for (int j = 0; j < 4; ++j) {
      const float f = rq[slot][r][j][c];
      e[j] = __float_as_uint(f);
    }
    if (r > 0) {
      const unsigned m = use[slot][r] ? 0xffffffffu : 0u;
#pragma unroll
      for (int j = 0; j < 4; ++j) e[j] &= m;
    }
    if (r == 0 || ASUM) {
      const bf16x2 ones = __builtin_bit_cast(bf16x2, live);
#pragma unroll
      for (int j = 0; j < 4; ++j)
        csum[r][c] = __builtin_amdgcn_fdot2_f32_bf16(__builtin_bit_cast(bf16x2, e[j]), ones, csum[r][c], false);
// ... 461 lines not shown
```

### wesep_amd/csrc/norm.hip

```cpp
#include "common.h"

struct GroupView {
  long long base;
  int W;
  int band;
};

__device__ __forceinline__ GroupView group_view(const ws_groups_geom& geo, int g) {
  GroupView v;
  v.band = g % geo.nbands;
  v.W = geo.band_w ? geo.band_w[v.band] : geo.W;
  v.base = (long long)(g / geo.gdiv) * geo.gs1 + (long long)(g % geo.gdiv) * geo.gs2 +
           (geo.band_off ? geo.band_off[v.band] : 0);
  return v;
}

static bool geom_vec4(const ws_groups_geom* g) {
  return !g->band_w && !g->band_off && g->W % 4 == 0 && g->rs % 4 == 0 && g->gs1 % 4 == 0 && g->gs2 % 4 == 0;
}

template <bool V4>
__global__ __launch_bounds__(256) void group_stats_kernel(const float* __restrict__ x,
                                                          const ws_groups_geom geo, float eps,
                                                          float* __restrict__ stats,
                                                          const int* __restrict__ glen, int glen_div) {
  __shared__ float red[16];
  const int g = blockIdx.x;
  const GroupView v = group_view(geo, g);
  const int n = (glen ? min(max(glen[g / glen_div], 1), geo.L) : geo.L) * v.W;
  const float* xb = x + v.base;
  float s = 0.f;
  if (V4) {
    const int w4 = v.W >> 2;
    for (int i = threadIdx.x; i < (n >> 2); i += 256) {
      const int row = i / w4, c4 = i - row * w4;
      const f32x4 t = *reinterpret_cast<const f32x4*>(xb + (long long)row * geo.rs + 4 * c4);
      s += (t[0] + t[1]) + (t[2] + t[3]);
    }
  } else {
    for (int i = threadIdx.x; i < n; i += 256) {
      const int row = i / v.W, col = i - row * v.W;
      s += xb[(long long)row * geo.rs + col];
    }
  }
  const float mean = ws_block_sum(s, red) / (float)n;
  float q = 0.f;
  if (V4) {
    const int w4 = v.W >> 2;
    for (int i = threadIdx.x; i < (n >> 2); i += 256) {
      const int row = i / w4, c4 = i - row * w4;
      const f32x4 t = *reinterpret_cast<const f32x4*>(xb + (long long)row * geo.rs + 4 * c4) - mean;
      q += (t[0] * t[0] + t[1] * t[1]) + (t[2] * t[2] + t[3] * t[3]);
    }
  } else
  for (int i = threadIdx.x; i < n; i += 256) {
    const int row = i / v.W, col = i - row * v.W;
    const float dv = xb[(long long)row * geo.rs + col] - mean;
    q += dv * dv;
  }
  const float var = ws_block_sum(q, red) / (float)n;
  if (threadIdx.x == 0) {
    stats[2 * (long long)g] = mean;
    stats[2 * (long long)g + 1] = 1.f / sqrtf(var + eps);
  }
}

static int geom_check(const ws_groups_geom* geo, const char* who) {
  WS_REQUIRE(geo && geo->ngroups > 0 && geo->gdiv > 0 && geo->L > 0 && geo->W > 0 && geo->nbands > 0,
             "%s: bad geometry", who);
  return WS_OK;
}

static int group_stats_launch(const char* who, const float* x, const ws_groups_geom* geo, const int* glen, int glen_div,
                              float eps, float* stats, void* stream) {
  int rc = geom_check(geo, who);
  if (rc != WS_OK) return rc;
  WS_REQUIRE(x && stats, "%s: null pointer", who);
  if (geom_vec4(geo))
    hipLaunchKernelGGL((group_stats_kernel<true>), dim3(geo->ngroups), dim3(256), 0, (hipStream_t)stream, x,
                       *geo, eps, stats, glen, glen_div);
  else
    hipLaunchKernelGGL((group_stats_kernel<false>), dim3(geo->ngroups), dim3(256), 0, (hipStream_t)stream, x,
                       *geo, eps, stats, glen, glen_div);
  return ws_check_launch(who);
}

extern "C" int ws_group_stats(const float* x, const ws_groups_geom* geo, float eps, float* stats,
                              void* stream) {
  return group_stats_launch("ws_group_stats", x, geo, nullptr, 1, eps, stats, stream);
}

extern "C" int ws_group_stats_len(const float* x, const ws_groups_geom* geo, const int* glen, int glen_div, float eps,
                                  float* stats, void* stream) {
  WS_REQUIRE(glen && glen_div > 0, "ws_group_stats_len: glen table / glen_div");
  return group_stats_launch("ws_group_stats_len", x, geo, glen, glen_div, eps, stats, stream);
}

template <bool V4>
__global__ __launch_bounds__(256) void gn_bwd_reduce_kernel(
    const float* __restrict__ x, const float* __restrict__ dxn, const float* __restrict__ stats,
    const float* __restrict__ gamma, const float* const* __restrict__ gamma_tab,
    const ws_groups_geom geo, float* __restrict__ ab) {
  __shared__ float red[16];
  const int g = blockIdx.x;
  const GroupView v = group_view(geo, g);
  const float* gm = gamma_tab ? gamma_tab[v.band] : gamma;
  const int n = geo.L * v.W;
  const float mean = stats[2 * (long long)g], rstd = stats[2 * (long long)g + 1];
  float s1 = 0.f, s2 = 0.f;
  if (V4) {
    const int w4 = v.W >> 2;
    for (int i = threadIdx.x; i < (n >> 2); i += 256) {
      const int row = i / w4, c4 = i - row * w4;
      const long long o = v.base + (long long)row * geo.rs + 4 * c4;
      const f32x4 dg = *reinterpret_cast<const f32x4*>(dxn + o) * *reinterpret_cast<const f32x4*>(gm + 4 * c4);
      const f32x4 xh = (*reinterpret_cast<const f32x4*>(x + o) - mean) * rstd;
      s1 += (dg[0] + dg[1]) + (dg[2] + dg[3]);
      s2 += (dg[0] * xh[0] + dg[1] * xh[1]) + (dg[2] * xh[2] + dg[3] * xh[3]);
    }
  } else
  for (int i = threadIdx.x; i < n; i += 256) {
    const int row = i / v.W, col = i - row * v.W;
    const long long o = v.base + (long long)row * geo.rs + col;
    const float dg = dxn[o] * gm[col];
    s1 += dg;
    s2 += dg * (x[o] - mean) * rstd;
  }
  s1 = ws_block_sum(s1, red);
  s2 = ws_block_sum(s2, red);
  if (threadIdx.x == 0) {
    ab[2 * (long long)g] = s1 / (float)n;
    ab[2 * (long long)g + 1] = s2 / (float)n;
  }
}

extern "C" int ws_gn_bwd_reduce(const float* x, const float* dxn, const float* stats,
                                const float* gamma, const float* const* gamma_tab,
                                const ws_groups_geom* geo, float* ab, void* stream) {
  int rc = geom_check(geo, "ws_gn_bwd_reduce");
  if (rc != WS_OK) return rc;
  WS_REQUIRE(x && dxn && stats && ab && (gamma || gamma_tab), "ws_gn_bwd_reduce: null pointer");
  if (geom_vec4(geo))
    hipLaunchKernelGGL((gn_bwd_reduce_kernel<true>), dim3(geo->ngroups), dim3(256), 0, (hipStream_t)stream,
                       x, dxn, stats, gamma, gamma_tab, *geo, ab);
  else
    hipLaunchKernelGGL((gn_bwd_reduce_kernel<false>), dim3(geo->ngroups), dim3(256), 0, (hipStream_t)stream,
                       x, dxn, stats, gamma, gamma_tab, *geo, ab);
  return ws_check_launch("ws_gn_bwd_reduce");
}

__global__ __launch_bounds__(256) void gn_bwd_apply_pg_kernel(
    const float* __restrict__ x, const float* dxn, const float* __restrict__ stats, const float* __restrict__ ab,
    const float* __restrict__ gamma, const float* __restrict__ res, const ws_groups_geom geo, float* dx,
    float* __restrict__ pslab, float* __restrict__ pout, unsigned* counter) {
  __shared__ f32x4 sh[2][8][32];
  const int g = blockIdx.x;
  const GroupView v = group_view(geo, g);
  const int n = geo.L * 128;
  const float mean = stats[2 * (long long)g], rstd = stats[2 * (long long)g + 1];
  const float a0 = ab[2 * (long long)g], a1 = ab[2 * (long long)g + 1];
  const int c4 = threadIdx.x & 31, rl = threadIdx.x >> 5;
  const f32x4 gm = *reinterpret_cast<const f32x4*>(gamma + 4 * c4);
  f32x4 sg = {0.f, 0.f, 0.f, 0.f}, sb = {0.f, 0.f, 0.f, 0.f};
  for (int row = rl; row < geo.L; row += 8) {
    const long long o = v.base + (long long)row * geo.rs + 4 * c4;
    const f32x4 d = *reinterpret_cast<const f32x4*>(dxn + o);
    const f32x4 xh = (*reinterpret_cast<const f32x4*>(x + o) - mean) * rstd;
    f32x4 r = (d * gm - a0 - xh * a1) * rstd;
    if (res) r += *reinterpret_cast<const f32x4*>(res + o);
    *reinterpret_cast<f32x4*>(dx + o) = r;
    sg += d * xh;
    sb += d;
  }
  (void)n;
  sh[0][rl][c4] = sg;
  sh[1][rl][c4] = sb;
  __syncthreads();
  if (rl < 2) {
    f32x4 t = sh[rl][0][c4];
#pragma unroll
    for (int r = 1; r < 8; ++r) t += sh[rl][r][c4];
    float* o = pslab + ((long long)g * 2 + rl) * 128 + 4 * c4;
#pragma unroll
    for (int q = 0; q < 4; ++q) ws_st_agent(o + q, t[q]);
  }
  ws_tree_sum256(pslab, gridDim.x, pout, counter);
}

extern "C" int ws_gn_bwd_apply_pg(const float* x, const float* dxn, const float* stats, const float* ab,
                                  const float* gamma, const float* res, const ws_groups_geom* geo, float* dx,
                                  float* pslab, float* pout, unsigned* counter, void* stream) {
  int rc = geom_check(geo, "ws_gn_bwd_apply_pg");
  if (rc != WS_OK) return rc;
  WS_REQUIRE(x && dxn && stats && ab && dx && gamma && pslab && pout && counter, "ws_gn_bwd_apply_pg: null pointer");
  WS_REQUIRE(geom_vec4(geo) && geo->nbands == 1 && geo->W == 128, "ws_gn_bwd_apply_pg: single-band groups of 128-float rows");
  hipLaunchKernelGGL(gn_bwd_apply_pg_kernel, dim3(geo->ngroups), dim3(256), 0, (hipStream_t)stream, x, dxn, stats, ab,
                     gamma, res, *geo, dx, pslab, pout, counter);
  return ws_check_launch("ws_gn_bwd_apply_pg");
}

template <bool V4>
__global__ __launch_bounds__(256) void gn_bwd_apply_kernel(
    const float* __restrict__ x, const float* dxn, const float* __restrict__ stats,
    const float* __restrict__ ab, const float* __restrict__ gamma,
    const float* const* __restrict__ gamma_tab, const float* __restrict__ res,
    const ws_groups_geom geo, float* dx) {
  const int g = blockIdx.x;
  const GroupView v = group_view(geo, g);
  const float* gm = gamma_tab ? gamma_tab[v.band] : gamma;
  const int n = geo.L * v.W;
  const float mean = stats[2 * (long long)g], rstd = stats[2 * (long long)g + 1];
  const float a0 = ab[2 * (long long)g], a1 = ab[2 * (long long)g + 1];
  if (V4) {
    const int w4 = v.W >> 2;
    for (int i = threadIdx.x; i < (n >> 2); i += 256) {
      const int row = i / w4, c4 = i - row * w4;
      const long long o = v.base + (long long)row * geo.rs + 4 * c4;
      const f32x4 xh = (*reinterpret_cast<const f32x4*>(x + o) - mean) * rstd;
      f32x4 r = (*reinterpret_cast<const f32x4*>(dxn + o) * *reinterpret_cast<const f32x4*>(gm + 4 * c4) - a0 - xh * a1) * rstd;
      if (res) r += *reinterpret_cast<const f32x4*>(res + o);
      *reinterpret_cast<f32x4*>(dx + o) = r;
    }
    return;
  }
  for (int i = threadIdx.x; i < n; i += 256) {
    const int row = i / v.W, col = i - row * v.W;
    const long long o = v.base + (long long)row * geo.rs + col;
    const float xh = (x[o] - mean) * rstd;
    float r = rstd * (dxn[o] * gm[col] - a0 - xh * a1);
    if (res) r += res[o];
    dx[o] = r;
  }
}

extern "C" int ws_gn_bwd_apply(const float* x, const float* dxn, const float* stats,
                               const float* ab, const float* gamma, const float* const* gamma_tab,
                               const float* res, const ws_groups_geom* geo, float* dx,
                               void* stream) {
  int rc = geom_check(geo, "ws_gn_bwd_apply");
  if (rc != WS_OK) return rc;
  WS_REQUIRE(x && dxn && stats && ab && dx && (gamma || gamma_tab), "ws_gn_bwd_apply: null pointer");
  if (geom_vec4(geo))
    hipLaunchKernelGGL((gn_bwd_apply_kernel<true>), dim3(geo->ngroups), dim3(256), 0, (hipStream_t)stream, x,
                       dxn, stats, ab, gamma, gamma_tab, res, *geo, dx);
  else
    hipLaunchKernelGGL((gn_bwd_apply_kernel<false>), dim3(geo->ngroups), dim3(256), 0, (hipStream_t)stream, x,
                       dxn, stats, ab, gamma, gamma_tab, res, *geo, dx);
  return ws_check_launch("ws_gn_bwd_apply");
}

__global__ __launch_bounds__(256) void gn_param_grad_kernel(const float* __restrict__ x,
                                                            const float* __restrict__ dxn,
                                                            const float* __restrict__ stats,
                                                            const ws_groups_geom geo, int nsplit,
                                                            float* __restrict__ slab) {
  __shared__ float sh[2][128];
  const int band = blockIdx.x, split = blockIdx.y;
  const int col = threadIdx.x & 127, rl = threadIdx.x >> 7;
  const int per_band = geo.ngroups / geo.nbands;
  float sg = 0.f, sb = 0.f;
  for (int j = split; j < per_band; j += nsplit) {
    const int g = j * geo.nbands + band;
    const GroupView v = group_view(geo, g);
    if (col >= v.W) continue;
    const float mean = stats[2 * (long long)g], rstd = stats[2 * (long long)g + 1];
    for (int row = rl; row < geo.L; row += 2) {
      const long long o = v.base + (long long)row * geo.rs + col;
      const float dv = dxn[o];
      sg += dv * (x[o] - mean) * rstd;
      sb += dv;
    }
  }
  if (rl == 1) {
    sh[0][col] = sg;
    sh[1][col] = sb;
  }
  __syncthreads();
  if (rl == 0 && col < geo.W) {
    float* out = slab + ((long long)(split * geo.nbands + band) * 2) * geo.W;
    out[col] = sg + sh[0][col];
    out[geo.W + col] = sb + sh[1][col];
// ... 265 lines not shown
```

### wesep_amd/dev.py

```python
import ctypes as C
import os
from typing import NamedTuple, Optional

import numpy as np
import torch

from . import _lib as L

BIG = 1 << 30


def gemm_mode() -> str:
    return os.environ.get("WESEP_GEMM", "bf16x3")


def _mode_bit(mode):
    return 4 if (mode or gemm_mode()) == "bf16x3" else 0
GN_EPS = float(np.finfo(np.float32).eps)


class Rows(NamedTuple):
    div: int
    s1: int
    s2: int
# ... 100 lines not shown

def gemm_tn(*, G, g_rows: Rows, A, a_rows: Rows, M: int, slab, slab_stride: int, nsplit: int,
            rows_per_split: int, Nn=0, Kk=0, bslab=None, bslab_stride=0, out_off=0, bout_off=0,
            stats=None, gamma=None, beta=None, stat_map: Optional[StatMap] = None,
            shift_rows=0, seq_div=1, seq_len=1, groups=None, ngroups=0, max_n=0, max_k=0, vec=1,
            g_off=0, a_off=0, mode=None, conv: Optional[ConvView] = None):
    for n, t in (("G", G), ("A", A), ("slab", slab), ("bslab", bslab), ("stats", stats),
                 ("gamma", gamma), ("beta", beta)):
        _chk(t, n)
    a = L.GemmTNArgs()
    a.G, a.A, a.slab, a.bslab = _p(G, g_off), _p(A, a_off), _p(slab), _p(bslab)
    a.stats, a.gamma, a.beta = _p(stats), _p(gamma), _p(beta)
    a.groups = C.c_void_p(groups.data_ptr()) if groups is not None else None
    a.g_div, a.g_s1, a.g_s2 = g_rows
    a.a_div, a.a_s1, a.a_s2 = a_rows
    sm = stat_map or StatMap(1, 0, 1, 0, 0)
    a.st_div1, a.st_m1, a.st_div2, a.st_m2, a.st_base = sm
    a.slab_stride, a.bslab_stride, a.out_off, a.bout_off = slab_stride, bslab_stride, out_off, bout_off
    a.M, a.Nn, a.Kk, a.rows_per_split, a.nsplit = M, Nn, Kk, rows_per_split, nsplit
    a.shift_rows, a.seq_div, a.seq_len = shift_rows, seq_div, seq_len
    a.ngroups, a.max_n, a.max_k, a.vec = ngroups, max_n, max_k, vec | _mode_bit(mode)
    _set_conv(a, conv)
    if ALG is not None and groups is None:
        a_elems = (M // (conv.Ho * conv.Wo)) * conv.H * conv.W * conv.C if conv is not None else M * Kk
        _alg("gemm_tn", 4 * (a_elems + M * Nn + nsplit * Nn * Kk), 2 * M * Nn * Kk)
    L.check(L.lib().ws_gemm_tn(C.byref(a), L.stream_ptr()), "ws_gemm_tn")


CONV_WGRAD_MAXK = 768


def conv_wgrad_ok(Nn: int, conv: ConvView) -> bool:
    return conv.mode == 0 and 4 <= Nn <= 32 and Nn % 4 == 0 and conv.C % 4 == 0 and conv.k <= 5


def conv_wgrad(*, G, ldg: int, X, M: int, Nn: int, conv: ConvView, slab, nsplit: int, tiles_per_split: int, bslab=None):
    for n, t in (("G", G), ("X", X), ("slab", slab), ("bslab", bslab)):
        _chk(t, n)
    a = L.ConvWgradArgs()
    a.G, a.X, a.slab, a.bslab = _p(G), _p(X), _p(slab), _p(bslab)
    Kk = conv.k * conv.k * conv.C
    a.ldg, a.slab_stride, a.bslab_stride = ldg, Nn * Kk, Nn
    a.M, a.Nn, a.nsplit, a.tiles_per_split = M, Nn, nsplit, tiles_per_split
    _set_conv(a, conv)
    _alg("gemm_tn", 4 * ((M // (conv.Ho * conv.Wo)) * conv.H * conv.W * conv.C + M * Nn + nsplit * Nn * Kk), 2 * M * Nn * Kk)
    L.check(L.lib().ws_conv_wgrad(C.byref(a), L.stream_ptr()), "ws_conv_wgrad")


def reduce_slabs(slab, nsplit: int, stride: int, count: int, out, w=0, ldo=0, out_off=0):
    _chk(slab, "slab")
    _chk(out, "out")
    L.check(L.lib().ws_reduce_slabs(_p(slab), nsplit, stride, count, _p(out, out_off), w, ldo,
                                    L.stream_ptr()), "ws_reduce_slabs")


def transpose(src, rows: int, cols: int, lds: int, dst, src_off=0, dst_off=0):
    _chk(src, "src")
    _chk(dst, "dst")
    L.check(L.lib().ws_transpose(_p(src, src_off), rows, cols, lds, _p(dst, dst_off), L.stream_ptr()),
            "ws_transpose")


class Geom(NamedTuple):
    ngroups: int
    gdiv: int
    gs1: int
    gs2: int
    rs: int
    L: int
    W: int
    nbands: int = 1
    band_w: Optional[torch.Tensor] = None
    band_off: Optional[torch.Tensor] = None

    def c(self):
        g = L.GroupsGeom()
        g.band_w = C.c_void_p(self.band_w.data_ptr()) if self.band_w is not None else None
        g.band_off = C.c_void_p(self.band_off.data_ptr()) if self.band_off is not None else None
        g.gs1, g.gs2, g.rs = self.gs1, self.gs2, self.rs
        g.ngroups, g.gdiv, g.L, g.W, g.nbands = self.ngroups, self.gdiv, self.L, self.W, self.nbands
        return g


def group_stats(x, geo: Geom, stats, eps=GN_EPS, glen=None, glen_div=1):
    _chk(x, "x")
    _chk(stats, "stats")
    g = geo.c()
    if glen is not None:
        _chk_lens(glen, -(-geo.ngroups // glen_div), "ws_group_stats_len")
        L.check(L.lib().ws_group_stats_len(_p(x), C.byref(g), _tab(glen), glen_div, eps, _p(stats), L.stream_ptr()),
                "ws_group_stats_len")
        return
    L.check(L.lib().ws_group_stats(_p(x), C.byref(g), eps, _p(stats), L.stream_ptr()), "ws_group_stats")


def _chk_lens(t, n, who):
    _chk(t, f"{who}: length table", torch.int32)
    if t.numel() < n:
        raise L.WesepHipError(f"{who}: the length table has {t.numel()} entries, the call needs {n}")


def ragged_tables(lengths, T, device, hop=128, min_len=257):
    ln = [int(v) for v in (lengths.tolist() if hasattr(lengths, "tolist") else lengths)]
    bad = [(r, v) for r, v in enumerate(ln) if v < min_len or v > T]
    if not ln or bad:
        raise L.WesepHipError(f"lengths outside [{min_len}, T = {T}] (row, value): {bad[:4]}" if bad else "lengths: empty")
    t = torch.tensor([ln, [1 + v // hop for v in ln]], dtype=torch.int32)
    t = t.to(device)
    return t[0].contiguous(), t[1].contiguous()


def _tab(t):
    return C.c_void_p(t.data_ptr()) if t is not None else None


def _word(t):
    return C.c_void_p(t.data_ptr()) if t is not None else None


def gn_bwd_reduce(x, dxn, stats, geo: Geom, ab, gamma=None, gamma_tab=None):
    for n, t in (("x", x), ("dxn", dxn), ("stats", stats), ("ab", ab), ("gamma", gamma)):
        _chk(t, n)
    g = geo.c()
    L.check(L.lib().ws_gn_bwd_reduce(_p(x), _p(dxn), _p(stats), _p(gamma), _tab(gamma_tab),
                                     C.byref(g), _p(ab), L.stream_ptr()), "ws_gn_bwd_reduce")


def gn_bwd_apply(x, dxn, stats, ab, geo: Geom, dx, gamma=None, gamma_tab=None, res=None):
    for n, t in (("x", x), ("dxn", dxn), ("stats", stats), ("ab", ab), ("gamma", gamma),
                 ("res", res), ("dx", dx)):
        _chk(t, n)
    g = geo.c()
    L.check(L.lib().ws_gn_bwd_apply(_p(x), _p(dxn), _p(stats), _p(ab), _p(gamma), _tab(gamma_tab),
                                    _p(res), C.byref(g), _p(dx), L.stream_ptr()), "ws_gn_bwd_apply")


def gn_bwd_fused_ok(geo: Geom) -> bool:
    return (os.environ.get("WESEP_GN_FUSED", "1") != "0" and geo.nbands == 1 and geo.W == 128 and geo.band_w is None
            and geo.band_off is None and 2 <= geo.L <= 32 and geo.L % 2 == 0 and geo.rs % 4 == 0
            and geo.gs1 % 4 == 0 and geo.gs2 % 4 == 0)


def gn_bwd_fused(x, dxn, stats, geo: Geom, gamma, dx, nwg: int, pslab, res=None, pout=None, counter=None, dxn2=None):
    for n, t in (("x", x), ("dxn", dxn), ("dxn2", dxn2), ("stats", stats), ("gamma", gamma), ("res", res), ("dx", dx),
                 ("pslab", pslab), ("pout", pout)):
        _chk(t, n)
    g = geo.c()
    L.check(L.lib().ws_gn_bwd_fused2(_p(x), _p(dxn), _p(dxn2), _p(stats), _p(gamma), _p(res), C.byref(g), nwg, _p(dx),
                                     _p(pslab), _p(pout), _word(counter), L.stream_ptr()), "ws_gn_bwd_fused")


def tree_groups(nblocks: int) -> int:
    return -(-nblocks // 32)


def gn_bwd_apply_pg_ok(geo: Geom) -> bool:
    return (os.environ.get("WESEP_GN_FUSED", "1") != "0" and geo.nbands == 1 and geo.W == 128 and geo.band_w is None
            and geo.band_off is None and geo.rs % 4 == 0 and geo.gs1 % 4 == 0 and geo.gs2 % 4 == 0)


def gn_bwd_apply_pg(x, dxn, stats, ab, geo: Geom, dx, gamma, pslab, pout, counter, res=None):
    for n, t in (("x", x), ("dxn", dxn), ("stats", stats), ("ab", ab), ("gamma", gamma), ("res", res), ("dx", dx),
                 ("pslab", pslab), ("pout", pout)):
        _chk(t, n)
    g = geo.c()
    L.check(L.lib().ws_gn_bwd_apply_pg(_p(x), _p(dxn), _p(stats), _p(ab), _p(gamma), _p(res), C.byref(g), _p(dx),
                                       _p(pslab), _p(pout), _word(counter), L.stream_ptr()), "ws_gn_bwd_apply_pg")


def gn_param_grad(x, dxn, stats, geo: Geom, nsplit: int, slab):
    for n, t in (("x", x), ("dxn", dxn), ("stats", stats), ("slab", slab)):
        _chk(t, n)
    g = geo.c()
    L.check(L.lib().ws_gn_param_grad(_p(x), _p(dxn), _p(stats), C.byref(g), nsplit, _p(slab),
                                     L.stream_ptr()), "ws_gn_param_grad")


class SeqMap(NamedTuple):
    nseq: int
    div: int
    s1: int
    s2: int
    step_rows: int
    L: int
    nvalid: int = 0


def lstm_mode(nseq: int) -> int:
    if os.environ.get("WESEP_LSTM", "bf16x3") == "bf16x3":
        return L.LSTM_BF16X3
    return L.LSTM_F32_MT2 if nseq >= 8192 else L.LSTM_F32_MT1


def lstm_blk_mode(nseq: int) -> int:
    env = os.environ.get("WESEP_LSTM_SEQS")
    if env:
        return L.LSTM_BF16X3_BLK16 if env == "16" else L.LSTM_BF16X3_BLK
    return L.LSTM_BF16X3_BLK16 if 2 * (-(-nseq // 32)) <= 128 else L.LSTM_BF16X3_BLK


def lstm_pack(whh_f, whh_r, pack_fwd, pack_bwd, mode=L.LSTM_BF16X3):
    for n, t in (("whh_f", whh_f), ("whh_r", whh_r), ("pack_fwd", pack_fwd), ("pack_bwd", pack_bwd)):
        _chk(t, n)
    L.check(L.lib().ws_lstm_pack(_p(whh_f), _p(whh_r), _p(pack_fwd), _p(pack_bwd), mode,
                                 L.stream_ptr()), "ws_lstm_pack")


def lstm_pack_bwd_f8(whh_f, whh_r, pack_bwd):
    for n, t in (("whh_f", whh_f), ("whh_r", whh_r), ("pack_bwd", pack_bwd)):
        _chk(t, n)
    L.check(L.lib().ws_lstm_pack_bwd_f8(_p(whh_f), _p(whh_r), _p(pack_bwd), L.stream_ptr()), "ws_lstm_pack_bwd_f8")


def lstm_pack_dx_f8(wcat, pack):
    for n, t in (("wcat", wcat), ("pack", pack)):
        _chk(t, n)
    L.check(L.lib().ws_lstm_pack_dx_f8(_p(wcat), _p(pack), L.stream_ptr()), "ws_lstm_pack_dx_f8")


def lstm_cat_ih(wih_f, wih_r, bih_f, bhh_f, bih_r, bhh_r, n_in, wcat, bcat):
    for t in (wih_f, wih_r, bih_f, bhh_f, bih_r, bhh_r, wcat, bcat):
        _chk(t, "lstm_cat_ih arg")
    L.check(L.lib().ws_lstm_cat_ih(_p(wih_f), _p(wih_r), _p(bih_f), _p(bhh_f), _p(bih_r), _p(bhh_r),
                                   n_in, _p(wcat), _p(bcat), L.stream_ptr()), "ws_lstm_cat_ih")


def _bptt_bytes(gfmt: int) -> int:
    return {L.GATES_F32: 40, L.GATES_H2: 24, L.GATES_H2S: 32, L.GATES_H2F: 24}[gfmt]


def gates_fmt() -> int:
    return {"h2": L.GATES_H2F, "h2b": L.GATES_H2, "h2s": L.GATES_H2S, "f32": L.GATES_F32}[os.environ.get("WESEP_GATES", "h2")]


def blh_floats(nblocks: int, C_: int) -> int:
    return nblocks * 32 * C_ // 2


def _lstm_args(gates, cbuf, hcat, wpack, sm: SeqMap, mode, dhcat=None, run_if=None, gfmt=0, gates_in=None, dgates=None,
               amax=None, rfmt=0, dxn=None, wxpack=None):
    for n, t in (("gates", gates), ("cbuf", cbuf), ("hcat", hcat), ("wpack", wpack), ("dhcat", dhcat),
                 ("gates_in", gates_in), ("dgates", dgates), ("dxn", dxn), ("wxpack", wxpack)):
        _chk(t, n)
    a = L.LstmArgs()
    a.gates, a.cbuf, a.hcat, a.dhcat, a.wpack = _p(gates), _p(cbuf), _p(hcat), _p(dhcat), _p(wpack)
    a.sq_s1, a.sq_s2, a.step_rows = sm.s1, sm.s2, sm.step_rows
    a.nseq, a.sq_div, a.L, a.mode = sm.nseq, sm.div, sm.L, mode
    a.run_if = C.c_void_p(run_if.data_ptr()) if run_if is not None else None
# ... 415 lines not shown
    pos = torch.div(sq, sm.div, rounding_mode="floor") * sm.s1 + (sq % sm.div) * sm.s2 + step * sm.step_rows
    return (pos * valid).reshape(-1), valid.reshape(-1)


def bls_pack(x: torch.Tensor) -> torch.Tensor:
    hi = x.to(torch.bfloat16)
    lo = (x - hi.float()).to(torch.bfloat16)
    bits = (hi.view(torch.int16).to(torch.int32) << 16) | (lo.view(torch.int16).to(torch.int32) & 0xffff)
    return bits.view(torch.float32)


def bls_unpack(x: torch.Tensor) -> torch.Tensor:
    bits = x.contiguous().view(torch.int32)
    return (bits & -65536).view(torch.float32) + (bits << 16).view(torch.float32)


def to_blocked(x: torch.Tensor, sm: SeqMap, split=False) -> torch.Tensor:
    pos, valid = bl_positions(sm, x.device)
    C_ = x.shape[1]
    rows = x[pos] * valid[:, None].to(x.dtype)
    out = rows.view(-1, 32, C_ // 4, 4).permute(0, 2, 1, 3).contiguous()
    return bls_pack(out) if split else out


def from_blocked(xb: torch.Tensor, sm: SeqMap, P: int, split=False) -> torch.Tensor:
    if split:
        xb = bls_unpack(xb)
    pos, valid = bl_positions(sm, xb.device)
    nblk, Cq = xb.shape[0], xb.shape[1]
    rows = xb.permute(0, 2, 1, 3).reshape(nblk * 32, Cq * 4)
    out = torch.zeros(P, Cq * 4, device=xb.device, dtype=xb.dtype)
    out[pos[valid]] = rows[valid]
    return out


def blh_bf16_pack(xb: torch.Tensor) -> torch.Tensor:
    return xb.to(torch.bfloat16).contiguous().view(torch.float32)


def blh_f16_pack(xb: torch.Tensor) -> torch.Tensor:
    return xb.to(torch.float16).contiguous().view(torch.float32)


def blh_f16_unpack(buf: torch.Tensor, nblk: int, C_: int) -> torch.Tensor:
    return buf.reshape(-1)[: nblk * 32 * C_ // 2].view(torch.float16).view(nblk, C_ // 4, 32, 4).float()


def blh_bf16_unpack(buf: torch.Tensor, nblk: int, C_: int) -> torch.Tensor:
    return buf.reshape(-1)[: nblk * 32 * C_ // 2].view(torch.bfloat16).view(nblk, C_ // 4, 32, 4).float()


def blh_gates_unpack(buf: torch.Tensor, nblk: int) -> torch.Tensor:
    Cq = 2 * 4 * L.LSTM_H // 4
    code = (buf.reshape(-1)[: nblk * 32 * Cq * 2].view(torch.int16).to(torch.int32) & 0xFFFF).view(nblk, Cq, 32, 4).double()
    s_sig = float(torch.tensor(1.0 / 65535.0, dtype=torch.float32))
    s_tanh = float(torch.tensor(1.0 / 32767.5, dtype=torch.float32))
    is_g = ((torch.arange(Cq, device=buf.device) >> 6) & 3 == 2).view(1, Cq, 1, 1)
    return torch.where(is_g, code * s_tanh - 1.0, code * s_sig).float()


def _smc(sm: SeqMap):
    c = L.SeqMapC()
    c.sq_s1, c.sq_s2, c.step_rows, c.nseq, c.sq_div, c.L = sm.s1, sm.s2, sm.step_rows, sm.nseq, sm.div, sm.L
    c.nvalid = sm.nvalid
    return c


def pack_w(W, N: int, K: int, ldw: int, out, trans=False, order=0, w_off=0, f16=False):
    _chk(W, "W")
    _chk(out, "out")
    if out.numel() < N * K:
        raise L.WesepHipError("pack_w: output too small")
    if int(f16) == 2:
        if order != 1:
            raise L.WesepHipError("pack_w: the fp16 + FP8 pack exists in the b2p order only")
        L.check(L.lib().ws_pack_w_f16f8(_p(W, w_off), N, K, ldw, int(trans), _p(out), L.stream_ptr()), "ws_pack_w_f16f8")
        return
    fn = L.lib().ws_pack_w_f16 if f16 else L.lib().ws_pack_w
    L.check(fn(_p(W, w_off), N, K, ldw, int(trans), order, _p(out), L.stream_ptr()), "ws_pack_w_f16" if f16 else "ws_pack_w")


def gemm_p2b(*, A, lda: int, sm: SeqMap, Wpack, N: int, C_out, K=128, bias=None, A_bl=None, stats=None,
             gamma=None, beta=None, stat_map: Optional[StatMap] = None, run_if=None, amax=None, A_bl16=None, steps=None,
             steps_div=1):
    for n, t in (("A", A), ("Wpack", Wpack), ("bias", bias), ("C", C_out), ("A_bl", A_bl), ("stats", stats),
                 ("gamma", gamma), ("beta", beta), ("A_bl16", A_bl16)):
        _chk(t, n)
    a = L.GemmP2BArgs()
    a.A, a.Wpack, a.bias, a.C, a.A_bl = _p(A), _p(Wpack), _p(bias), _p(C_out), _p(A_bl)
    a.stats, a.gamma, a.beta = _p(stats), _p(gamma), _p(beta)
    a.sm = _smc(sm)
    st = stat_map or StatMap(1, 0, 1, 0, 0)
    a.st_div1, a.st_m1, a.st_div2, a.st_m2, a.st_base = st
    a.lda, a.N, a.K = lda, N, K
    a.run_if = C.c_void_p(run_if.data_ptr()) if run_if is not None else None
    a.amax = C.c_void_p(amax.data_ptr()) if amax is not None else None
    a.A_bl16 = _p(A_bl16)
    if ALG is not None and run_if is None:
        rows = (getattr(sm, "nvalid", 0) or sm.nseq) * sm.L
        _alg("gemm_nt", rows * (4 * K + 4 * N + (4 * K if A_bl is not None else 0) + (2 * K if A_bl16 is not None else 0)) + 4 * N * K,
             2 * rows * N * K)
    if steps is not None:
        _chk_lens(steps, -(-(getattr(sm, "nvalid", 0) or sm.nseq) // steps_div), "ws_gemm_p2b_len")
        L.check(L.lib().ws_gemm_p2b_len(C.byref(a), _tab(steps), steps_div, L.stream_ptr()), "ws_gemm_p2b_len")
        return
    L.check(L.lib().ws_gemm_p2b(C.byref(a), L.stream_ptr()), "ws_gemm_p2b")


def gemm_b2p(*, A, K: int, sm: SeqMap, Wpack, C_out, ldc: int, N=128, bias=None, R=None, a_fmt=0, amax=None, a16_out=None):
    for n, t in (("A", A), ("Wpack", Wpack), ("bias", bias), ("C", C_out), ("R", R), ("a16_out", a16_out)):
        _chk(t, n)
    if a16_out is not None and a_fmt != 0:
        raise L.WesepHipError("gemm_b2p: a16_out goes with a_fmt = 0 (split-pair A)")
    a = L.GemmB2PArgs()
    a.A, a.Wpack, a.bias, a.R, a.C = _p(A), _p(Wpack), _p(bias), _p(R), _p(C_out)
    a.sm = _smc(sm)
    a.ldc, a.N, a.K, a.a_fmt = ldc, N, K, a_fmt
    a.amax = C.c_void_p(amax.data_ptr()) if amax is not None else None
    a.a16_out = _p(a16_out)
    if ALG is not None:
        rows = (getattr(sm, "nvalid", 0) or sm.nseq) * sm.L
        _alg("gemm_nt", rows * ((4 if a_fmt in (0, 4) else 2) * K + 4 * N * (1 + (R is not None)) + (2 * K if a16_out is not None else 0))
             + 4 * N * K, 2 * rows * N * K)
    L.check(L.lib().ws_gemm_b2p(C.byref(a), L.stream_ptr()), "ws_gemm_b2p")


def tnb_splits(nblk: int, gtiles: int):
    cap = int(os.environ.get("WESEP_TNB_MAXSPLIT", "64"))
    nsplit = max(1, min(cap, int(os.environ.get("WESEP_TNB_WGS", "256")) // gtiles, nblk))
    if nsplit >= 8:
        nsplit -= nsplit % 8
    bps = -(-nblk // nsplit)
    return nsplit, bps


def gemm_tnb(*, G, g_width: int, g_off: int, g_cols: int, A0, a0_width: int, a0_off: int, a0_cols: int,
             nblk: int, L_: int, slab, nsplit: int, blocks_per_split: int, a0_shift=0, A1=None, a1_width=0,
             a1_off=0, a1_cols=0, a1_shift=0, bslab=None, aslab=None, g_fmt=0, amax=None, a_fmt=0):
    for n, t in (("G", G), ("A0", A0), ("A1", A1), ("slab", slab), ("bslab", bslab), ("aslab", aslab)):
        _chk(t, n)
    a = L.GemmTNBArgs()
    a.G, a.A0, a.A1, a.slab, a.bslab, a.aslab = _p(G), _p(A0), _p(A1), _p(slab), _p(bslab), _p(aslab)
    a.slab_stride = g_cols * (a0_cols + a1_cols)
    a.bslab_stride = g_cols
    a.aslab_stride = a0_cols + a1_cols
    a.g_width, a.g_off, a.g_cols = g_width, g_off, g_cols
    a.a0_width, a.a0_off, a.a0_cols, a.a0_shift = a0_width, a0_off, a0_cols, a0_shift
    a.a1_width, a.a1_off, a.a1_cols, a.a1_shift = a1_width, a1_off, a1_cols, a1_shift
    a.nblk, a.L, a.nsplit, a.blocks_per_split, a.g_fmt, a.a_fmt = nblk, L_, nsplit, blocks_per_split, g_fmt, a_fmt
    a.amax = C.c_void_p(amax.data_ptr()) if amax is not None else None
    if ALG is not None:
        rows, acols = nblk * 32, a0_cols + a1_cols
        _alg("gemm_tn", rows * ((2 if g_fmt else 4) * g_cols + (2 if a_fmt else 4) * acols) + 4 * nsplit * g_cols * acols,
             2 * rows * g_cols * acols)
    L.check(L.lib().ws_gemm_tnb(C.byref(a), L.stream_ptr()), "ws_gemm_tnb")


def h2p_on(device) -> bool:
    env = os.environ.get("WESEP_H2P")
    return env != "0" if env is not None else device.type == "cuda"


def h2p_hi(hcat, nblk: int, C_: int = 2 * L.LSTM_H):
    return hcat.reshape(-1)[: blh_floats(nblk, C_)]


def h2p_unpack(hcat, nblk: int, C_: int = 2 * L.LSTM_H):
    n = blh_floats(nblk, C_)
    flat = hcat.reshape(-1)
    return blh_f16_unpack(flat[:n], nblk, C_), blh_f16_unpack(flat[n:2 * n], nblk, C_)


def gemm_tnb_h16(*, G, g_width: int, g_off: int, g_cols: int, A0, a0_width: int, a0_off: int, nblk: int, L_: int, slab,
                 nsplit: int, blocks_per_split: int, amax, aslab=None):
    for n, t in (("G", G), ("A0", A0), ("slab", slab), ("aslab", aslab)):
        _chk(t, n)
    if amax is None:
        raise L.WesepHipError("gemm_tnb_h16: amax (the scale word of this backward) is required")
    a = L.GemmTNBArgs()
    a.G, a.A0, a.slab, a.aslab = _p(G), _p(A0), _p(slab), _p(aslab)
    a.slab_stride, a.bslab_stride, a.aslab_stride = g_cols * 128, g_cols, 128
    a.g_width, a.g_off, a.g_cols = g_width, g_off, g_cols
    a.a0_width, a.a0_off, a.a0_cols = a0_width, a0_off, 128
    a.nblk, a.L, a.nsplit, a.blocks_per_split = nblk, L_, nsplit, blocks_per_split
    a.amax = C.c_void_p(amax.data_ptr())
    if ALG is not None:
        rows = nblk * 32
        _alg("gemm_tn", rows * (2 * g_cols + 4 * 128) + 4 * nsplit * g_cols * 128, 2 * rows * g_cols * 128)
    L.check(L.lib().ws_gemm_tnb_h16(C.byref(a), L.stream_ptr()), "ws_gemm_tnb_h16")


LN_EPS = 1e-5


def _call(name, *args):
    L.check(getattr(L.lib(), name)(*args, L.stream_ptr()), name)


def flat_stats(x, ngroups: int, n_per_group: int, stats, eps=LN_EPS, nchunk=None):
    if nchunk is None:
        nchunk = max(1, min(max(1, 512 // ngroups), n_per_group // 16384))
    scratch = torch.empty(ngroups, nchunk, 4, device=x.device, dtype=torch.float32)
    for n, t in (("x", x), ("stats", stats)):
        _chk(t, n)
    _call("ws_flat_stats", _p(x), ngroups, n_per_group, eps, nchunk, _p(scratch), _p(stats))

# ... 1105 lines not shown
```

### wesep_amd/functional.py

```python
import os

import numpy as np
import torch

from . import _lib as L
from . import dev
from .dev import BIG, Geom, Rows, SeqMap, StatMap, flat
from .blstm_core import (G4, H, PAIR_STAMPS, PackCache, WeightPacks, WGradBox, WGradCarrierFn, _NO_CACHE,
                         _PROBE_SAT, _cluster_dbg, _empty, _h2_probe, _pair_dbg, _pending, _probe_round, _reduce_new,
                         _side_stream, amax_word, band_dx, band_rfmt, blstm_bptt, blstm_dxn, blstm_forward,
                         blstm_weight_grads, consume_once, defer_wgrad, dxn_fmt, flush_deferred_wgrads, keep_for_side,
                         make_plan, mark_wgrads_ready, pair_rfmt, tnb_a16, weight_grads, wgrad_hold, zero_words)

NBIN = 257
HOP = 128


def _need_cuda(t, who):
    if not t.is_cuda:
        raise L.WesepHipError(f"{who}: wesep_amd has no CPU path; move the model and inputs to the GPU")


def _view_maps(view, R, K, Tf, N):
    if view == "time":
# ... 39 lines not shown
        out = torch.empty_like(z)
        pw = proj_w.contiguous()
        dev.gemm_nt(A=hcat, a_rows=flat(2 * H), M=P, N=N, K=2 * H, W=pw, ldw=2 * H, bias=proj_b,
                    R=z, C_out=out, c_rows=flat(N))
        ctx.save_for_backward(z, stats, gates, cbuf, hcat, wcat, pack_b, norm_w, norm_b, pw)
        ctx.view, ctx.mt = view, mt
        return out

    @staticmethod
    def backward(ctx, dout):
        z, stats, gates, cbuf, hcat, wcat, pack_b, norm_w, norm_b, pw = ctx.saved_tensors
        dout = dout.contiguous()
        R, K, Tf, N = z.shape
        P = R * K * Tf
        d = z.device
        geo, smap, seq, (seq_div, seq_len) = _view_maps(ctx.view, R, K, Tf, N)
        nsplit, rps = dev.tn_splits(P)
        projT = _empty(d, 2 * H, N)
        dev.transpose(pw, N, 2 * H, 2 * H, projT)
        dhcat = _empty(d, P, 2 * H)
        dev.gemm_nt(A=dout, a_rows=flat(N), M=P, N=2 * H, K=N, W=projT, ldw=N, C_out=dhcat,
                    c_rows=flat(2 * H))
        slab, bslab = _empty(d, nsplit, N * 2 * H), _empty(d, nsplit, N)
        dev.gemm_tn(G=dout, g_rows=flat(N), A=hcat, a_rows=flat(2 * H), M=P, Nn=N, Kk=2 * H, slab=slab,
                    slab_stride=N * 2 * H, bslab=bslab, bslab_stride=N, nsplit=nsplit, rows_per_split=rps)
        dproj_w = _reduce_new(slab, nsplit, N * 2 * H, (N, 2 * H))
        dproj_b = _reduce_new(bslab, nsplit, N, (N,))
        dev.lstm_bwd(gates, cbuf, hcat, dhcat, pack_b, seq, ctx.mt)
        del dhcat
        dwhh = []
        slab = _empty(d, nsplit, G4 * H)
        for di in (0, 1):
            dev.gemm_tn(G=gates, g_rows=flat(2 * G4), g_off=di * G4, A=hcat, a_rows=flat(2 * H),
                        a_off=di * H, M=P, Nn=G4, Kk=H, slab=slab, slab_stride=G4 * H, nsplit=nsplit,
                        rows_per_split=rps, shift_rows=(-seq.step_rows if di == 0 else seq.step_rows),
                        seq_div=seq_div, seq_len=seq_len)
            dwhh.append(_reduce_new(slab, nsplit, G4 * H, (G4, H)))
        slab, bslab = _empty(d, nsplit, 2 * G4 * N), _empty(d, nsplit, 2 * G4)
        dev.gemm_tn(G=gates, g_rows=flat(2 * G4), A=z, a_rows=flat(N), M=P, Nn=2 * G4, Kk=N, slab=slab,
                    slab_stride=2 * G4 * N, bslab=bslab, bslab_stride=2 * G4, nsplit=nsplit,
                    rows_per_split=rps, stats=stats, gamma=norm_w, beta=norm_b, stat_map=smap)
        dwcat = _reduce_new(slab, nsplit, 2 * G4 * N, (2 * G4, N))
        dbcat = _reduce_new(bslab, nsplit, 2 * G4, (2 * G4,))
        del slab, bslab
        wcatT = _empty(d, N, 2 * G4)
        dev.transpose(wcat, 2 * G4, N, N, wcatT)
        dxn = _empty(d, P, N)
        dev.gemm_nt(A=gates, a_rows=flat(2 * G4), M=P, N=N, K=2 * G4, W=wcatT, ldw=2 * G4, C_out=dxn,
                    c_rows=flat(N))
        ab = _empty(d, geo.ngroups, 2)
        dev.gn_bwd_reduce(z, dxn, stats, geo, ab, gamma=norm_w)
        ns2 = min(256, geo.ngroups)
        pslab = _empty(d, ns2, 2, N)
        dev.gn_param_grad(z, dxn, stats, geo, ns2, pslab)
        dgb = _reduce_new(pslab, ns2, 2 * N, (2, N))
        dz = torch.empty_like(z)
        dev.gn_bwd_apply(z, dxn, stats, ab, geo, dz, gamma=norm_w, res=dout)
        return (dz, None, dgb[0], dgb[1],
                dwcat[:G4], dwhh[0], dbcat[:G4], dbcat[:G4].clone(),
                dwcat[G4:], dwhh[1], dbcat[G4:], dbcat[G4:].clone(),
                dproj_w, dproj_b)


def resrnn_mode() -> str:
    return os.environ.get("WESEP_RESRNN", "blocked")


def wgrad_overlap() -> bool:
    return os.environ.get("WESEP_WGRAD_OVERLAP", "1") != "0"


_TIME_LEFT = {}


def reset_deferred_wgrads(device):
    _pending(device).clear()
    _TIME_LEFT[(device.type, device.index)] = 0


def tail_flush() -> bool:
    return os.environ.get("WESEP_TAIL_FLUSH", "1") != "0"


def _resrnn_blk_fwd(z, view, norm_w, norm_b, wparams, cache, grad, frames=None):
    _need_cuda(z, "ResRNN")
    wih_f, whh_f, proj_b = wparams[0], wparams[1], wparams[9]
    R, K, Tf, N = z.shape
    if tuple(whh_f.shape) != (G4, H) or tuple(wih_f.shape) != (G4, N) or N != 128:
        raise L.WesepHipError(f"blocked ResRNN kernels are built for input 128 / hidden {H}; got "
                              f"{tuple(wih_f.shape)}, {tuple(whh_f.shape)}")
    d = z.device
    geo, smap, seq, _ = _view_maps(view, R, K, Tf, N)
    ragged = frames is not None and view == "time"
    stats = _empty(d, geo.ngroups, 2)
    if ragged:
        dev.group_stats(z, geo, stats, glen=frames, glen_div=K)
    else:
        dev.group_stats(z, geo, stats)
    cache = cache if cache is not None else _NO_CACHE
    sig = cache.begin(wparams)
    plan = make_plan(seq, d, grad, gn_geo=geo, ragged=ragged) if ragged else make_plan(seq, d, grad, gn_geo=geo)
    W = WeightPacks(cache, sig, plan.lmode, plan.pair_rfmt, *wparams[:9])
    steps = dict(steps=(frames, K)) if ragged else {}
    out, saved = blstm_forward(plan, W, z, seq, res=z, bias=proj_b,
                               norm=dict(stats=stats, gamma=norm_w, beta=norm_b, stat_map=smap), **steps)
    return out, stats, plan, W, saved


class ResRNNBlkFn(torch.autograd.Function):

    @staticmethod
    def forward(ctx, z, dummy, box, cache, view, norm_w, norm_b, wih_f, whh_f, bih_f, bhh_f, wih_r, whh_r, bih_r,
                bhh_r, proj_w, proj_b):
        z = z.contiguous()
        d = z.device
        out, stats, plan, W, saved = _resrnn_blk_fwd(
            z, view, norm_w, norm_b, (wih_f, whh_f, bih_f, bhh_f, wih_r, whh_r, bih_r, bhh_r, proj_w, proj_b), cache,
            any(ctx.needs_input_grad))
        ctx.save_for_backward(z, stats, norm_w, *saved)
        if view == "time" and box is not None and plan.grad:
            key = (d.type, d.index)
            _TIME_LEFT[key] = _TIME_LEFT.get(key, 0) + 1
        ctx.view, ctx.box, ctx.plan, ctx.packs = view, box, plan, W
        ctx.consumed = False
        return out

    @staticmethod
    def backward(ctx, dout):
        consume_once(ctx, "ResRNN")
        z, stats, norm_w, gates, cbuf, hcat, xn, hcat16 = ctx.saved_tensors
        plan, W, box = ctx.plan, ctx.packs, ctx.box
        dout = dout.contiguous()
        R, K, Tf, N = z.shape
        P = R * K * Tf
        d = z.device
        geo, smap, seq, _ = _view_maps(ctx.view, R, K, Tf, N)
        dg, dout_bl, amax, dxn2 = blstm_bptt(plan, W, gates, cbuf, hcat, dout, seq, release=ctx.view == "time")
        wg = blstm_weight_grads(plan, dg, xn, hcat, dout_bl, amax, hcat16, seq, box)
        del dout_bl
        if box is not None and ctx.view == "time":
            key = (d.type, d.index)
            _TIME_LEFT[key] = _TIME_LEFT.get(key, 1) - 1
            if _TIME_LEFT[key] <= 0 and tail_flush():
                flush_deferred_wgrads(d)
        dxn, dxn_r = blstm_dxn(plan, W, dg, amax, dxn2, seq, P)
        dz = torch.empty_like(z)
        dgb = _empty(d, 2, N)
        if dev.gn_bwd_fused_ok(geo):
            ns2 = min(1024, -(-geo.ngroups // 4))
            pslab = _empty(d, ns2 + dev.tree_groups(ns2), 2, N)
            dev.gn_bwd_fused(z, dxn, stats, geo, norm_w, dz, ns2, pslab, res=dout, pout=dgb,
                             counter=zero_words(d, 1 + dev.tree_groups(ns2)), dxn2=dxn_r)
        elif dev.gn_bwd_apply_pg_ok(geo):
            ab = _empty(d, geo.ngroups, 2)
            dev.gn_bwd_reduce(z, dxn, stats, geo, ab, gamma=norm_w)
            pslab = _empty(d, geo.ngroups + dev.tree_groups(geo.ngroups), 2, N)
            dev.gn_bwd_apply_pg(z, dxn, stats, ab, geo, dz, norm_w, pslab, dgb, zero_words(d, 1 + dev.tree_groups(geo.ngroups)),
                                res=dout)
        else:
            ab = _empty(d, geo.ngroups, 2)
            dev.gn_bwd_reduce(z, dxn, stats, geo, ab, gamma=norm_w)
            ns2 = min(1024, geo.ngroups)
            pslab = _empty(d, ns2, 2, N)
            dev.gn_param_grad(z, dxn, stats, geo, ns2, pslab)
            dev.gn_bwd_apply(z, dxn, stats, ab, geo, dz, gamma=norm_w, res=dout)
            dgb = _reduce_new(pslab, ns2, 2 * N, (2, N))
        gd = torch.zeros((), device=d) if box is not None else None
        return (dz, gd, None, None, None, dgb[0], dgb[1]) + tuple(wg)


def pack_prefetch() -> bool:
    return os.environ.get("WESEP_PACK_PREFETCH", "0") == "1"


def prefetch_packs(layers):
    layers = [(c, p) for c, p in layers if c is not None and c.lmode is not None and p[0].is_cuda]
    if not layers or not pack_prefetch() or not torch.cuda.is_available():
        return
    d = layers[0][1][0].device
    todo = []
    for cache, params in layers:
        sig = cache.begin(params)
        if cache.kinds_prev and not cache.items:
            todo.append((cache, sig, params))
    if not todo:
        return
    side = _side_stream(d)
    gate = torch.cuda.Event()
    gate.record(torch.cuda.current_stream())
    with torch.no_grad(), torch.cuda.stream(side):
        side.wait_event(gate)
        for cache, sig, params in todo:
            W = WeightPacks(cache, sig, cache.lmode, cache.pair_rf, *(p.detach() for p in params[:9]))
            for kind in list(cache.kinds_prev):
                W(kind)
            ready = torch.cuda.Event()
            ready.record(side)
            cache.ready, cache.waited = ready, {side.cuda_stream}


def make_wgrad_carrier(params, blocked=None):
    if blocked is None:
        blocked = resrnn_mode() == "blocked"
    if not (wgrad_overlap() and blocked and torch.is_grad_enabled()
            and params[0].is_cuda and all(p.requires_grad for p in params)):
        return None
    box = WGradBox()
    return WGradCarrierFn.apply(box, *params), box


def resrnn(z, view, norm_w, norm_b, *params, carrier=None, cache=None, frames=None):
    if frames is not None:
        if torch.is_grad_enabled() or resrnn_mode() != "blocked":
            raise L.WesepHipError("ResRNN: per-row lengths are an inference feature of the blocked path "
                                  "(torch.no_grad(), WESEP_RESRNN=blocked); training batches are cropped by the collate function")
        return _resrnn_blk_fwd(z.contiguous(), view, norm_w, norm_b, tuple(p.detach() for p in params), cache, False,
                               frames=frames)[0]
    if resrnn_mode() != "blocked":
        return ResRNNFn.apply(z, view, norm_w, norm_b, *params)
    if carrier is None:
        return ResRNNBlkFn.apply(z, None, None, cache, view, norm_w, norm_b, *params)
    dummy, box = carrier
    return ResRNNBlkFn.apply(z, dummy, box, cache, view, norm_w, norm_b, *(p.detach() for p in params))


def _w2d(w):
    return w.reshape(w.shape[0], -1).contiguous()


def _lin_fwd(x, W, b, act=0, w_off=0, ldw=None, K=None):
    M = x.shape[0]
    Nout = W.shape[0]
    K = K if K is not None else W.shape[1]
    ldw = ldw if ldw is not None else W.shape[1]
    y = _empty(x.device, M, Nout)
    vec = 3 if (K % 4 == 0 and ldw % 4 == 0 and w_off % 4 == 0 and x.shape[1] % 4 == 0) else 0
    dev.gemm_nt(A=x, a_rows=flat(x.shape[1]), M=M, N=Nout, K=K, W=W, ldw=ldw, bias=b, C_out=y,
                c_rows=flat(Nout), act=act, vec=vec, w_off=w_off)
    return y


def _lin_bwd_w(dy, x, with_bias=True):
    M, Nout = dy.shape
    K = x.shape[1]
    pad = (-Nout) % 4
    if pad:
        dyp = torch.zeros(M, Nout + pad, device=dy.device, dtype=torch.float32)
        dyp[:, :Nout] = dy
        dy = dyp
    Np = Nout + pad
    rps = -(-M // 32) * 32
    dW = _empty(dy.device, Np, K)
    db = _empty(dy.device, Np) if with_bias else None
    dev.gemm_tn(G=dy, g_rows=flat(Np), A=x, a_rows=flat(K), M=M, Nn=Np, Kk=K, slab=dW,
                slab_stride=Np * K, bslab=db, bslab_stride=Np, nsplit=1, rows_per_split=rps,
                vec=1 if K % 4 == 0 else 0)
    if pad:
        dW = dW[:Nout].contiguous()
        db = db[:Nout].contiguous() if with_bias else None
    return dW, db


def _lin_bwd_x(dy, W, T=None, src_off=0, rows=None, cols=None, lds=None):
    rows = rows if rows is not None else W.shape[0]
    cols = cols if cols is not None else W.shape[1]
    lds = lds if lds is not None else W.shape[1]
    WT = _empty(dy.device, cols, rows)
    dev.transpose(W, rows, cols, lds, WT, src_off=src_off)
    dx = _empty(dy.device, dy.shape[0], cols)
    vec = 3 if rows % 4 == 0 else 0
    dev.gemm_nt(A=dy, a_rows=flat(rows), M=dy.shape[0], N=cols, K=rows, W=WT, ldw=rows, C_out=dx,
                c_rows=flat(cols), T=T, vec=vec)
    return dx


class LinearFn(torch.autograd.Function):
    @staticmethod
    def forward(ctx, x, W, b):
        _need_cuda(x, "Linear")
        x, W2 = x.contiguous(), _w2d(W)
        ctx.save_for_backward(x, W2)
        ctx.wshape = W.shape
        return _lin_fwd(x, W2, b)

    @staticmethod
    def backward(ctx, dy):
        x, W2 = ctx.saved_tensors
        dy = dy.contiguous()
        dW, db = _lin_bwd_w(dy, x)
        dx = _lin_bwd_x(dy, W2) if ctx.needs_input_grad[0] else None
        return dx, dW.view(ctx.wshape), db


class SpkTransformFn(torch.autograd.Function):

    @staticmethod
    def forward(ctx, e, w0, b0, w1, b1, w3, b3):
        _need_cuda(e, "SpeakerTransform")
        e = e.contiguous()
        W0, W1, W3 = _w2d(w0), _w2d(w1), _w2d(w3)
        h0 = _lin_fwd(e, W0, b0)
        h1 = _lin_fwd(h0, W1, b1, act=1)
        y = _lin_fwd(h1, W3, b3)
        ctx.save_for_backward(e, h0, h1, W0, W1, W3)
        ctx.shapes = (w0.shape, w1.shape, w3.shape)
        return y
# ... 402 lines not shown
```

### wesep_amd/models/bsrnn.py

```python
from typing import Optional

import numpy as np
import torch
import torch.nn as nn

from .. import dev
from .. import functional as F_
from .._lib import WesepHipError
from ..modules.common.speaker import SpeakerFuseLayer, SpeakerTransform

_EPS = float(torch.finfo(torch.float32).eps)


class ResRNN(nn.Module):

    def __init__(self, input_size, hidden_size, bidirectional=True):
        super().__init__()
        if not bidirectional:
            raise NotImplementedError("wesep_amd ResRNN kernels are bidirectional (reference default)")
        self.input_size, self.hidden_size, self.eps = input_size, hidden_size, _EPS
        self.norm = nn.GroupNorm(1, input_size, self.eps)
        self.rnn = nn.LSTM(input_size, hidden_size, 1, batch_first=True, bidirectional=True)
        self.proj = nn.Linear(hidden_size * 2, input_size)
        self._packs = F_.PackCache()

    def invalidate_packs(self):
        self._packs = F_.PackCache()

    def _apply(self, fn, recurse=True):
        self._packs = F_.PackCache()
        return super()._apply(fn, recurse)

    def _load_from_state_dict(self, *args, **kwargs):
        self._packs = F_.PackCache()
        return super()._load_from_state_dict(*args, **kwargs)

    def _wparams(self):
        r = self.rnn
        return (r.weight_ih_l0, r.weight_hh_l0, r.bias_ih_l0, r.bias_hh_l0,
                r.weight_ih_l0_reverse, r.weight_hh_l0_reverse, r.bias_ih_l0_reverse, r.bias_hh_l0_reverse,
                self.proj.weight, self.proj.bias)

    def make_carrier(self):
        return F_.make_wgrad_carrier(self._wparams())

    def forward(self, z, view="time", carrier=None, frames=None):
        if frames is not None:
            return F_.resrnn(z, view, self.norm.weight, self.norm.bias, *self._wparams(), cache=self._packs, frames=frames)
        return F_.resrnn(z, view, self.norm.weight, self.norm.bias, *self._wparams(), carrier=carrier,
                         cache=self._packs)


class BSNet(nn.Module):

    def __init__(self, in_channel, nband=7, bidirectional=True):
        super().__init__()
        self.nband = nband
        self.feature_dim = in_channel // nband
        self.band_rnn = ResRNN(self.feature_dim, self.feature_dim * 2, bidirectional)
        self.band_comm = ResRNN(self.feature_dim, self.feature_dim * 2, bidirectional)

    def forward(self, z, dummy: Optional[torch.Tensor] = None, carriers=None, frames=None):
        c_t, c_b = carriers if carriers is not None else (None, None)
        if frames is not None:
            return self.band_comm(self.band_rnn(z, "time", frames=frames), "band")
        return self.band_comm(self.band_rnn(z, "time", c_t), "band", c_b)


class FuseSeparation(nn.Module):

    def __init__(self, nband=7, num_repeat=6, feature_dim=128, spk_emb_dim=256, spk_fuse_type="concat",
                 multi_fuse=True):
        super().__init__()
        self.multi_fuse, self.nband, self.feature_dim = multi_fuse, nband, feature_dim
        self.separation = nn.ModuleList([])
        fuse = lambda: SpeakerFuseLayer(embed_dim=spk_emb_dim, feat_dim=feature_dim, fuse_type=spk_fuse_type)
        if multi_fuse:
            for _ in range(num_repeat):
                self.separation.append(fuse())
                self.separation.append(BSNet(nband * feature_dim, nband))
        else:
            self.separation.append(fuse())
            for _ in range(num_repeat):
                self.separation.append(BSNet(nband * feature_dim, nband))

    def make_carriers(self, device):
        if device.type == "cuda":
            F_.reset_deferred_wgrads(device)
            if torch.is_grad_enabled():
                F_.prefetch_packs([(m._packs, m._wparams()) for l in self.separation if isinstance(l, BSNet)
                                   for m in (l.band_rnn, l.band_comm)])
        return {i: (l.band_rnn.make_carrier(), l.band_comm.make_carrier())
                for i, l in enumerate(self.separation) if isinstance(l, BSNet)}

    def forward(self, z, spk_embedding, nch=None, carriers=None, frames=None):
        if carriers is None:
            carriers = self.make_carriers(z.device)
        for i, layer in enumerate(self.separation):
            if isinstance(layer, BSNet) and frames is not None:
                z = layer(z, frames=frames)
            elif isinstance(layer, BSNet):
                z = layer(z, spk_embedding, carriers[i])
            else:
                z = layer(z, spk_embedding)
        return z


class BSRNN(nn.Module):
    def __init__(self, spk_emb_dim=256, sr=16000, win=512, stride=128, feature_dim=128, num_repeat=6,
                 use_spk_transform=True, use_bidirectional=True, spk_fuse_type="concat", multi_fuse=True,
                 joint_training=True, multi_task=False, spksInTrain=251, spk_model=None,
                 spk_model_init=None, spk_model_freeze=False, spk_args=None, spk_feat=False,
                 feat_type="consistent"):
        super().__init__()
        if (win, stride) != (512, 128):
            raise NotImplementedError("wesep_amd STFT kernels are built for win=512, stride=128")
        if feature_dim != 128:
            raise NotImplementedError("wesep_amd LSTM kernels are built for feature_dim=128 (hidden 256)")
        if joint_training and not spk_feat and feat_type != "consistent":
            raise NotImplementedError("joint_training with spk_feat=False: only feat_type='consistent' exists in the "
                                      "reference (bsrnn.py:231) and is built")
        self.sr, self.win, self.stride = sr, win, stride
        self.group = win // 2
        self.enc_dim = win // 2 + 1
        self.feature_dim = feature_dim
        self.eps = _EPS
        self.spk_emb_dim = spk_emb_dim
        self.joint_training, self.spk_feat, self.feat_type = joint_training, spk_feat, feat_type
        self.spk_model_freeze, self.multi_task = spk_model_freeze, multi_task

        nyq = sr / 2.0
        bw = lambda hz: int(np.floor(hz / nyq * self.enc_dim))
        self.band_width = [bw(100)] * 15 + [bw(200)] * 10 + [bw(500)] * 5 + [bw(2000)]
        self.band_width.append(self.enc_dim - int(np.sum(self.band_width)))
        self.nband = len(self.band_width)
        if max(self.band_width) * 2 > 128:
            raise NotImplementedError("band wider than 64 bins")

        self.spk_transform = SpeakerTransform() if use_spk_transform else nn.Identity()

        if joint_training:
            from .resnet import get_speaker_model
            self.spk_model = get_speaker_model(spk_model)(**(spk_args or {}))
            if spk_model_init:
                pretrained = torch.load(spk_model_init, map_location="cpu")
                state = self.spk_model.state_dict()
                for key in state.keys():
                    if key in pretrained.keys():
                        state[key] = pretrained[key]
                    else:
                        print("not %s loaded" % key)
                self.spk_model.load_state_dict(state)
            if spk_model_freeze:
                for param in self.spk_model.parameters():
                    param.requires_grad = False
            if not spk_feat:
                from ..modules.common.frontend import MelSpectrogram, PreEmphasis
                self.preEmphasis = PreEmphasis()
                self.spk_encoder = MelSpectrogram(sample_rate=sr, n_fft=win, win_length=win, hop_length=stride,
                                                  f_min=20, n_mels=(spk_args or {})["feat_dim"])
            else:
                self.preEmphasis = nn.Identity()
                self.spk_encoder = nn.Identity()
            self.pred_linear = nn.Linear(spk_emb_dim, spksInTrain) if multi_task else nn.Identity()

        self.BN = nn.ModuleList([
            nn.Sequential(nn.GroupNorm(1, b * 2, self.eps), nn.Conv1d(b * 2, feature_dim, 1))
            for b in self.band_width])
        self.separator = FuseSeparation(nband=self.nband, num_repeat=num_repeat, feature_dim=feature_dim,
                                        spk_emb_dim=spk_emb_dim, spk_fuse_type=spk_fuse_type,
                                        multi_fuse=multi_fuse)
        self.mask = nn.ModuleList([
            nn.Sequential(nn.GroupNorm(1, feature_dim, _EPS), nn.Conv1d(feature_dim, feature_dim * 4, 1),
                          nn.Tanh(), nn.Conv1d(feature_dim * 4, feature_dim * 4, 1), nn.Tanh(),
                          nn.Conv1d(feature_dim * 4, b * 4, 1))
            for b in self.band_width])
        self._plans = {}

    def _bn_params(self):
        out = []
        for seq in self.BN:
            out += [seq[0].weight, seq[0].bias, seq[1].weight, seq[1].bias]
        return out

    def _mask_params(self):
        out = []
        for seq in self.mask:
# ... 67 lines not shown
```

### wesep_amd/modules/common/speaker.py

```python
import torch.nn as nn

from ... import functional as F_


class SpeakerTransform(nn.Module):

    def __init__(self, embed_dim=256, num_layers=3, hid_dim=128):
        super().__init__()
        if num_layers != 3:
            raise NotImplementedError("SpeakerTransform kernels cover the reference default num_layers=3")
        layers = [nn.Conv1d(embed_dim, hid_dim, 1)]
        for _ in range(num_layers - 2):
            layers += [nn.Conv1d(hid_dim, hid_dim, 1), nn.Tanh()]
        layers.append(nn.Conv1d(hid_dim, embed_dim, 1))
        self.transforms = nn.Sequential(*layers)

    def forward(self, x):
        squeeze = x.dim() == 3
        if squeeze:
            x = x.squeeze(-1)
        t = self.transforms
        y = F_.SpkTransformFn.apply(x, t[0].weight, t[0].bias, t[1].weight, t[1].bias, t[3].weight, t[3].bias)
        return y.unsqueeze(-1) if squeeze else y


class LinearLayer(nn.Module):
    def __init__(self, in_features, out_features, bias=True):
        super().__init__()
        self.linear = nn.Linear(in_features, out_features, bias)

    def forward(self, x, dummy=None):
        return F_.LinearFn.apply(x, self.linear.weight, self.linear.bias)


class FiLM(nn.Module):

    def __init__(self, feat_size, embed_size, num_film_layers=1, layer_norm=False):
        super().__init__()
        if num_film_layers != 1 or layer_norm:
            raise NotImplementedError("FiLM kernels cover num_film_layers=1, layer_norm=False (reference use)")
        self.feat_size, self.embed_size, self.num_film_layers = feat_size, embed_size, num_film_layers
        self.layer_norm = None
        self.gamma_fcs = nn.ModuleList([nn.Linear(embed_size, feat_size)])
        self.beta_fcs = nn.ModuleList([nn.Linear(embed_size, feat_size)])
        self.init_weights()

    def init_weights(self):
        for fc in list(self.gamma_fcs) + list(self.beta_fcs):
            nn.init.zeros_(fc.weight)
            nn.init.zeros_(fc.bias)

    def forward(self, embed, x):
        g = F_.LinearFn.apply(embed, self.gamma_fcs[0].weight, self.gamma_fcs[0].bias)
        b = F_.LinearFn.apply(embed, self.beta_fcs[0].weight, self.beta_fcs[0].bias)
        return F_.AffineFn.apply(x, g, b, 1.0)


class SpeakerFuseLayer(nn.Module):
    def __init__(self, embed_dim=256, feat_dim=512, fuse_type="concat"):
        super().__init__()
        assert fuse_type in ["concat", "additive", "multiply", "FiLM", "None"]
        self.fuse_type = fuse_type
        if fuse_type == "concat":
            self.fc = LinearLayer(embed_dim + feat_dim, feat_dim)
        elif fuse_type in ("additive", "multiply"):
            self.fc = LinearLayer(embed_dim, feat_dim)
        elif fuse_type == "FiLM":
            self.fc = FiLM(feat_dim, embed_dim)
        else:
            raise ValueError("Fuse type not defined.")

    def forward(self, x, embed):
        if embed.dim() == 4:
            embed = embed[:, 0, :, 0]
        embed = embed.contiguous()
        if self.fuse_type == "concat":
            return F_.ConcatFuseFn.apply(x, embed, self.fc.linear.weight, self.fc.linear.bias)
        if self.fuse_type == "additive":
            return F_.AffineFn.apply(x, None, self.fc(embed), 1.0)
        if self.fuse_type == "multiply":
            return F_.AffineFn.apply(x, self.fc(embed), None, 0.0)
        return self.fc(embed, x)
```

Measured before the change: 360.3 utterances/s.

## Fold FiLM affine into next BSNet's norm stats, x-projection and residual

Instead of materializing the FiLM output z*(a0+a)+b before each BSNet, the speaker FiLM operands are passed into the time-view ResRNN. There they are applied on the fly in the group-norm stats, the p2b input GEMM, the b2p residual add and the GN backward kernels, which also produce dgamma/dbeta-style da/db per row. This removes a full elementwise read/write pass over the activation in forward and the separate AffineFn backward. In exchange, several kernels gain extra per-element loads and FILM template variants.

```diff
diff --git a/include/wesep_hip.h b/include/wesep_hip.h
--- a/include/wesep_hip.h
+++ b/include/wesep_hip.h
@@ -134,6 +134,20 @@
 int ws_gn_bwd_apply_pg(const float* x, const float* dxn, const float* stats, const float* ab,
                        const float* gamma, const float* res, const ws_groups_geom* geo, float* dx,
                        float* pslab, float* pout, unsigned* counter, void* stream);
+
+typedef struct ws_film_desc {
+  const float* a;
+  const float* b;
+  float a0;
+  int rows_per_r;
+} ws_film_desc;
+int ws_group_stats_film(const float* z, const ws_film_desc* film, const ws_groups_geom* geo, float eps, float* stats, void* stream);
+int ws_gn_bwd_reduce_film(const float* z, const ws_film_desc* film, const float* dxn, const float* stats, const float* gamma,
+                          const ws_groups_geom* geo, float* ab, void* stream);
+int ws_gn_bwd_apply_pg_film(const float* z, const ws_film_desc* film, const float* dxn, const float* stats, const float* ab,
+                            const float* gamma, const float* res, const ws_groups_geom* geo, float* dx, float* pslab,
+                            float* pout, unsigned* counter, float* fslab, float* da, float* db, unsigned* fcounter,
+                            void* stream);
 
 typedef struct ws_lstm_args {
   float* gates;
@@ -275,6 +289,8 @@
   void* a16_out;
 } ws_gemm_b2p_args;
 int ws_gemm_b2p(const ws_gemm_b2p_args* a, void* stream);
+int ws_gemm_p2b_film(const ws_gemm_p2b_args* a, const ws_film_desc* film, void* stream);
+int ws_gemm_b2p_film(const ws_gemm_b2p_args* a, const ws_film_desc* film, void* stream);
 
 typedef struct ws_gemm_tnb_args {
   const float* G;
diff --git a/wesep_amd/_lib.py b/wesep_amd/_lib.py
--- a/wesep_amd/_lib.py
+++ b/wesep_amd/_lib.py
@@ -106,6 +106,10 @@
 class GemmB2PArgs(C.Structure):
     _fields_ = [(n, _p) for n in ("A", "Wpack", "bias", "R", "C")] + [("sm", SeqMapC), ("ldc", _ll), ("N", _i), ("K", _i),
                                                                          ("a_fmt", _i), ("pad_", _i), ("amax", _p), ("a16_out", _p)]
+
+
+class FilmDesc(C.Structure):
+    _fields_ = [("a", _p), ("b", _p), ("a0", _f), ("rows_per_r", _i)]
 
 
 class GemmTNBArgs(C.Structure):
@@ -174,6 +178,10 @@
     "ws_gn_bwd_fused": (_i, [_p, _p, _p, _p, _p, C.POINTER(GroupsGeom), _i, _p, _p, _p, _p, _p]),
     "ws_gn_bwd_fused2": (_i, [_p, _p, _p, _p, _p, _p, C.POINTER(GroupsGeom), _i, _p, _p, _p, _p, _p]),
     "ws_gn_bwd_apply_pg": (_i, [_p, _p, _p, _p, _p, _p, C.POINTER(GroupsGeom), _p, _p, _p, _p, _p]),
+    "ws_group_stats_film": (_i, [_p, C.POINTER(FilmDesc), C.POINTER(GroupsGeom), _f, _p, _p]),
+    "ws_gn_bwd_reduce_film": (_i, [_p, C.POINTER(FilmDesc), _p, _p, _p, C.POINTER(GroupsGeom), _p, _p]),
+    "ws_gn_bwd_apply_pg_film": (_i, [_p, C.POINTER(FilmDesc), _p, _p, _p, _p, _p, C.POINTER(GroupsGeom), _p, _p, _p, _p,
+                                     _p, _p, _p, _p, _p]),
     "ws_lstm_pack": (_i, [_p, _p, _p, _p, _i, _p]),
     "ws_lstm_fwd": (_i, [C.POINTER(LstmArgs), _p]),
     "ws_lstm_bwd": (_i, [C.POINTER(LstmArgs), _p]),
@@ -192,6 +200,8 @@
     "ws_gemm_p2b": (_i, [C.POINTER(GemmP2BArgs), _p]),
     "ws_gemm_p2b_len": (_i, [C.POINTER(GemmP2BArgs), _p, _i, _p]),
     "ws_gemm_b2p": (_i, [C.POINTER(GemmB2PArgs), _p]),
+    "ws_gemm_p2b_film": (_i, [C.POINTER(GemmP2BArgs), C.POINTER(FilmDesc), _p]),
+    "ws_gemm_b2p_film": (_i, [C.POINTER(GemmB2PArgs), C.POINTER(FilmDesc), _p]),
     "ws_gemm_tnb": (_i, [C.POINTER(GemmTNBArgs), _p]),
     "ws_gemm_tnb_h16": (_i, [C.POINTER(GemmTNBArgs), _p]),
     "ws_stft_bandsplit": (_i, [_p, _i, _i, C.POINTER(Bands), _p, _p]),
diff --git a/wesep_amd/blstm_core.py b/wesep_amd/blstm_core.py
--- a/wesep_amd/blstm_core.py
+++ b/wesep_amd/blstm_core.py
@@ -388,9 +388,14 @@
     ctx.consumed = True
 
 
-def blstm_forward(plan, W, x, seq, res, bias, norm=None, steps=None):
+def blstm_forward(plan, W, x, seq, res, bias, norm=None, steps=None, film=None):
     d = x.device
-    norm = norm or {}
+    norm = dict(norm or {})
+    if film is not None:
+        if res is not x or steps is not None:
+            raise L.WesepHipError("blstm_forward: film= folds ONE affine into operand and residual (res is x), no step counts")
+        norm["film"] = film
+    rk = dict(film=film) if film is not None else {}
     if steps is not None and (plan.fwd in ("fused", "cluster2") or plan.grad):
         raise L.WesepHipError(f"blstm_forward: per-sequence step counts with forward branch '{plan.fwd}', grad={plan.grad}: "
                               "only the branches over precomputed gates know them, and only the forward")
@@ -435,9 +440,9 @@
         del pre
     out = torch.empty_like(res)
     if h2p:
-        dev.gemm_b2p(A=hcat, K=2 * H, sm=seq, Wpack=W("proj16"), C_out=out, ldc=N, bias=bias, R=res, a_fmt=4)
-    else:
-        dev.gemm_b2p(A=hcat, K=2 * H, sm=seq, Wpack=W("proj"), C_out=out, ldc=N, bias=bias, R=res, a16_out=hcat16)
+        dev.gemm_b2p(A=hcat, K=2 * H, sm=seq, Wpack=W("proj16"), C_out=out, ldc=N, bias=bias, R=res, a_fmt=4, **rk)
+    else:
+        dev.gemm_b2p(A=hcat, K=2 * H, sm=seq, Wpack=W("proj"), C_out=out, ldc=N, bias=bias, R=res, a16_out=hcat16, **rk)
     if _h2_probe() and not h2:
         if _h2_probe() & 1:
             _probe_round(gates, "f16")
diff --git a/wesep_amd/csrc/common.h b/wesep_amd/csrc/common.h
--- a/wesep_amd/csrc/common.h
+++ b/wesep_amd/csrc/common.h
@@ -104,6 +104,15 @@
 
 __device__ __forceinline__ float ws_sigmoid(float x) { return 1.f / (1.f + expf(-x)); }
 
+__device__ __forceinline__ float ws_film(float z, float a, float b, float a0) { return __builtin_fmaf(z, a0 + a, b); }
+__device__ __forceinline__ f32x4 ws_film(const f32x4 z, const f32x4 a, const f32x4 b, float a0) {
+  return f32x4{ws_film(z[0], a[0], b[0], a0), ws_film(z[1], a[1], b[1], a0), ws_film(z[2], a[2], b[2], a0),
+               ws_film(z[3], a[3], b[3], a0)};
+}
+__device__ __forceinline__ f32x4 ws_film_row(const float* p, long long r, int c) {
+  return p ? *reinterpret_cast<const f32x4*>(p + r * 128 + c) : f32x4{0.f, 0.f, 0.f, 0.f};
+}
+
 __device__ __forceinline__ long long ws_row_off(int m, int div, long long s1, long long s2) {
   const int q = m / div;
   return (long long)q * s1 + (long long)(m - q * div) * s2;
diff --git a/wesep_amd/csrc/elementwise.hip b/wesep_amd/csrc/elementwise.hip
--- a/wesep_amd/csrc/elementwise.hip
+++ b/wesep_amd/csrc/elementwise.hip
@@ -11,10 +11,10 @@
     const int c = (int)(i - row * n4) * 4;
     const int r = (int)(row / rows_per_r);
     f32x4 v = *reinterpret_cast<const f32x4*>(z + i * 4);
-    f32x4 av = {a0, a0, a0, a0}, bv = {0.f, 0.f, 0.f, 0.f};
-    if (a) av += *reinterpret_cast<const f32x4*>(a + (long long)r * N + c);
+    f32x4 av = {0.f, 0.f, 0.f, 0.f}, bv = {0.f, 0.f, 0.f, 0.f};
+    if (a) av = *reinterpret_cast<const f32x4*>(a + (long long)r * N + c);
     if (b) bv = *reinterpret_cast<const f32x4*>(b + (long long)r * N + c);
-    *reinterpret_cast<f32x4*>(out + i * 4) = v * av + bv;
+    *reinterpret_cast<f32x4*>(out + i * 4) = ws_film(v, av, bv, a0);
   }
 }
 
diff --git a/wesep_amd/csrc/gemm_blk.hip b/wesep_amd/csrc/gemm_blk.hip
--- a/wesep_amd/csrc/gemm_blk.hip
+++ b/wesep_amd/csrc/gemm_blk.hip
@@ -184,9 +184,9 @@
 }
 
 #define P2B_K 128
-template <bool LEN>
+template <bool LEN, bool FILM = false>
 __global__ __launch_bounds__(512, 4) void gemm_p2b_kernel(const ws_gemm_p2b_args p, const int* __restrict__ steps,
-                                                          int steps_div) {
+                                                          int steps_div, const ws_film_desc fm) {
   __shared__ __attribute__((aligned(16))) u32x4 wl[2][2048];
   if (p.run_if && *p.run_if == 0u) return;
   const int tid = threadIdx.x, lane = tid & 63, i = lane & 31, half = lane >> 5;
@@ -212,6 +212,7 @@
       mean = p.stats[2 * s];
       rstd = p.stats[2 * s + 1];
     }
+    const long long frow = FILM ? pos / fm.rows_per_r : 0;
     float* eb = p.A_bl ? p.A_bl + (long long)bb * (32 * P2B_K) + i * 4 : nullptr;
     unsigned short* eb16 = p.A_bl16 ? reinterpret_cast<unsigned short*>(p.A_bl16) + (long long)bb * (32 * P2B_K) + i * 4 : nullptr;
 #pragma unroll
@@ -219,6 +220,10 @@
       const int k0 = 16 * ks + 8 * half;
       f32x4 v0 = *reinterpret_cast<const f32x4*>(arow + k0);
       f32x4 v1 = *reinterpret_cast<const f32x4*>(arow + k0 + 4);
+      if constexpr (FILM) {
+        v0 = ws_film(v0, ws_film_row(fm.a, frow, k0), ws_film_row(fm.b, frow, k0), fm.a0);
+        v1 = ws_film(v1, ws_film_row(fm.a, frow, k0 + 4), ws_film_row(fm.b, frow, k0 + 4), fm.a0);
+      }
       if (p.stats) {
         const f32x4 g0 = *reinterpret_cast<const f32x4*>(p.gamma + k0), g1 = *reinterpret_cast<const f32x4*>(p.gamma + k0 + 4);
         const f32x4 b0 = *reinterpret_cast<const f32x4*>(p.beta + k0), b1 = *reinterpret_cast<const f32x4*>(p.beta + k0 + 4);
@@ -306,7 +311,8 @@
   }
 }
 
-static int gemm_p2b_launch(const char* who, const ws_gemm_p2b_args* a, const int* steps, int steps_div, void* stream) {
+static int gemm_p2b_launch(const char* who, const ws_gemm_p2b_args* a, const int* steps, int steps_div, void* stream,
+                           const ws_film_desc* film = nullptr) {
   WS_REQUIRE(a && a->A && ((a->Wpack && a->C) || (a->N == 0 && (a->A_bl || a->A_bl16))), "%s: null pointer", who);
   WS_REQUIRE(a->K == P2B_K, "%s: K must be %d (got %d)", who, P2B_K, a->K);
   WS_REQUIRE(a->N >= 0 && a->N % 64 == 0, "%s: N %% 64 (N=%d)", who, a->N);
@@ -317,16 +323,25 @@
   hipStream_t s = (hipStream_t)stream;
   const bool timed = a->run_if == nullptr;
   if (timed) ws_prof_begin(WS_PROF_GEMM_NT, s);
-  if (steps)
-    hipLaunchKernelGGL((gemm_p2b_kernel<true>), dim3((nblk + 7) / 8), dim3(512), 0, s, *a, steps, steps_div);
+  const ws_film_desc off = {nullptr, nullptr, 0.f, 1};
+  if (film)
+    hipLaunchKernelGGL((gemm_p2b_kernel<false, true>), dim3((nblk + 7) / 8), dim3(512), 0, s, *a, steps, steps_div, *film);
+  else if (steps)
+    hipLaunchKernelGGL((gemm_p2b_kernel<true>), dim3((nblk + 7) / 8), dim3(512), 0, s, *a, steps, steps_div, off);
   else
-    hipLaunchKernelGGL((gemm_p2b_kernel<false>), dim3((nblk + 7) / 8), dim3(512), 0, s, *a, steps, steps_div);
+    hipLaunchKernelGGL((gemm_p2b_kernel<false>), dim3((nblk + 7) / 8), dim3(512), 0, s, *a, steps, steps_div, off);
   if (timed) ws_prof_end(WS_PROF_GEMM_NT, s);
   return ws_check_launch(who);
 }
 
 extern "C" int ws_gemm_p2b(const ws_gemm_p2b_args* a, void* stream) {
   return gemm_p2b_launch("ws_gemm_p2b", a, nullptr, 1, stream);
+}
+
+extern "C" int ws_gemm_p2b_film(const ws_gemm_p2b_args* a, const ws_film_desc* film, void* stream) {
+  if (!film || (!film->a && !film->b)) return ws_gemm_p2b(a, stream);
+  WS_REQUIRE(film->rows_per_r > 0 && a && a->lda == P2B_K, "ws_gemm_p2b_film: rows_per_r > 0, lda = %d (a row = a position)", P2B_K);
+  return gemm_p2b_launch("ws_gemm_p2b_film", a, nullptr, 1, stream, film);
 }
 
 extern "C" int ws_gemm_p2b_len(const ws_gemm_p2b_args* a, const int* steps, int steps_div, void* stream) {
@@ -334,10 +349,11 @@
   return gemm_p2b_launch("ws_gemm_p2b_len", a, steps, steps_div, stream);
 }
 
-template <int A16>
-__global__ __launch_bounds__(512, 4) void gemm_b2p_kernel(const ws_gemm_b2p_args p) {
+template <int A16, bool FILM = false>
+__global__ __launch_bounds__(512, 4) void gemm_b2p_kernel(const ws_gemm_b2p_args p, const ws_film_desc fm) {
   __shared__ __attribute__((aligned(16))) u32x4 wl[2][2048];
   __shared__ long long posl[8][32];
+  __shared__ int frowl[FILM ? 8 : 1][32];
   const int tid = threadIdx.x, lane = tid & 63, i = lane & 31, half = lane >> 5;
   const int w = __builtin_amdgcn_readfirstlane(tid >> 6);
   const int nblk = ((p.sm.nseq + 31) / 32) * p.sm.L;
@@ -348,6 +364,9 @@
     bool valid;
     const long long pos = seq_pos(p.sm, bb, i, valid);
     if (half == 0) posl[w][i] = valid ? pos : -1;
+    if constexpr (FILM) {
+      if (half == 0) frowl[w][i] = (int)(pos / fm.rows_per_r);
+    }
   }
   const int K = p.K, nstage = K / 64;
   typedef typename std::conditional<A16 != 0, u32x2, f32x4>::type acell;
@@ -519,7 +538,14 @@
       off[k] = (active && pos >= 0) ? pos * p.ldc + pass * 64 + 4 * c4 : -1;
       v[k] = *reinterpret_cast<const f32x4*>(stg + m * 64 + 4 * c4);
     }
-    if (p.R) {
+    if constexpr (FILM) {
+#pragma unroll
+      for (int k = 0; k < 8; ++k)
+        if (off[k] >= 0) {
+          const int fr = frowl[w][r0 + 4 * k], c = pass * 64 + 4 * c4;
+          v[k] += ws_film(*reinterpret_cast<const f32x4*>(p.R + off[k]), ws_film_row(fm.a, fr, c), ws_film_row(fm.b, fr, c), fm.a0);
+        }
+    } else if (p.R) {
 #pragma unroll
       for (int k = 0; k < 8; ++k)
         if (off[k] >= 0) v[k] += *reinterpret_cast<const f32x4*>(p.R + off[k]);
@@ -531,30 +557,46 @@
   }
 }
 
-extern "C" int ws_gemm_b2p(const ws_gemm_b2p_args* a, void* stream) {
-  WS_REQUIRE(a && a->A && a->Wpack && a->C, "ws_gemm_b2p: null pointer");
-  WS_REQUIRE(a->N == 128, "ws_gemm_b2p: N must be 128 (got %d)", a->N);
-  WS_REQUIRE(a->a_fmt >= 0 && a->a_fmt <= 4 && (a->a_fmt < 2 || a->a_fmt == 4 || a->amax), "ws_gemm_b2p: a_fmt %d (2 / 3 need amax)",
+static int gemm_b2p_launch(const char* who, const ws_gemm_b2p_args* a, const ws_film_desc* film, void* stream);
+
+extern "C" int ws_gemm_b2p(const ws_gemm_b2p_args* a, void* stream) { return gemm_b2p_launch("ws_gemm_b2p", a, nullptr, stream); }
+
+extern "C" int ws_gemm_b2p_film(const ws_gemm_b2p_args* a, const ws_film_desc* film, void* stream) {
+  if (!film || (!film->a && !film->b)) return ws_gemm_b2p(a, stream);
+  WS_REQUIRE(a && (a->a_fmt == 0 || a->a_fmt == 4) && a->R && a->ldc == 128 && film->rows_per_r > 0,
+             "ws_gemm_b2p_film: the projections (a_fmt 0 / 4) with a residual, ldc = 128 (a row = a position), rows_per_r > 0");
+  return gemm_b2p_launch("ws_gemm_b2p_film", a, film, stream);
+}
+
+static int gemm_b2p_launch(const char* who, const ws_gemm_b2p_args* a, const ws_film_desc* film, void* stream) {
+  WS_REQUIRE(a && a->A && a->Wpack && a->C, "%s: null pointer", who);
+  WS_REQUIRE(a->N == 128, "%s: N must be 128 (got %d)", who, a->N);
+  WS_REQUIRE(a->a_fmt >= 0 && a->a_fmt <= 4 && (a->a_fmt < 2 || a->a_fmt == 4 || a->amax), "%s: a_fmt %d (2 / 3 need amax)", who,
              a->a_fmt);
-  WS_REQUIRE(a->a_fmt == 0 || !a->a16_out, "ws_gemm_b2p: a16_out goes with a_fmt 0 (got a_fmt %d)", a->a_fmt);
-  WS_REQUIRE(a->K > 0 && a->K % 64 == 0, "ws_gemm_b2p: K %% 64 (K=%d)", a->K);
-  WS_REQUIRE(a->ldc >= a->N && a->ldc % 4 == 0, "ws_gemm_b2p: ldc >= N and ldc %% 4 == 0 (16-byte row pieces)");
-  WS_REQUIRE(a->sm.nseq > 0 && a->sm.L > 0 && a->sm.sq_div > 0, "ws_gemm_b2p: bad sequence map");
+  WS_REQUIRE(a->a_fmt == 0 || !a->a16_out, "%s: a16_out goes with a_fmt 0 (got a_fmt %d)", who, a->a_fmt);
+  WS_REQUIRE(a->K > 0 && a->K % 64 == 0, "%s: K %% 64 (K=%d)", who, a->K);
+  WS_REQUIRE(a->ldc >= a->N && a->ldc % 4 == 0, "%s: ldc >= N and ldc %% 4 == 0 (16-byte row pieces)", who);
+  WS_REQUIRE(a->sm.nseq > 0 && a->sm.L > 0 && a->sm.sq_div > 0, "%s: bad sequence map", who);
   const int nblk = ((a->sm.nseq + 31) / 32) * a->sm.L;
   hipStream_t s = (hipStream_t)stream;
+  const ws_film_desc off = {nullptr, nullptr, 0.f, 1};
   ws_prof_begin(WS_PROF_GEMM_NT, s);
-  if (a->a_fmt == 4)
-    hipLaunchKernelGGL(gemm_b2p_kernel<4>, dim3((nblk + 7) / 8), dim3(512), 0, s, *a);
+  if (film && a->a_fmt == 4)
+    hipLaunchKernelGGL((gemm_b2p_kernel<4, true>), dim3((nblk + 7) / 8), dim3(512), 0, s, *a, *film);
+  else if (film)
+    hipLaunchKernelGGL((gemm_b2p_kernel<0, true>), dim3((nblk + 7) / 8), dim3(512), 0, s, *a, *film);
+  else if (a->a_fmt == 4)
+    hipLaunchKernelGGL(gemm_b2p_kernel<4>, dim3((nblk + 7) / 8), dim3(512), 0, s, *a, off);
   else if (a->a_fmt == 3)
-    hipLaunchKernelGGL(gemm_b2p_kernel<3>, dim3((nblk + 7) / 8), dim3(512), 0, s, *a);
+    hipLaunchKernelGGL(gemm_b2p_kernel<3>, dim3((nblk + 7) / 8), dim3(512), 0, s, *a, off);
   else if (a->a_fmt == 2)
-    hipLaunchKernelGGL(gemm_b2p_kernel<2>, dim3((nblk + 7) / 8), dim3(512), 0, s, *a);
+    hipLaunchKernelGGL(gemm_b2p_kernel<2>, dim3((nblk + 7) / 8), dim3(512), 0, s, *a, off);
   else if (a->a_fmt == 1)
-    hipLaunchKernelGGL(gemm_b2p_kernel<1>, dim3((nblk + 7) / 8), dim3(512), 0, s, *a);
+    hipLaunchKernelGGL(gemm_b2p_kernel<1>, dim3((nblk + 7) / 8), dim3(512), 0, s, *a, off);
   else
-    hipLaunchKernelGGL(gemm_b2p_kernel<0>, dim3((nblk + 7) / 8), dim3(512), 0, s, *a);
+    hipLaunchKernelGGL(gemm_b2p_kernel<0>, dim3((nblk + 7) / 8), dim3(512), 0, s, *a, off);
   ws_prof_end(WS_PROF_GEMM_NT, s);
-  return ws_check_launch("ws_gemm_b2p");
+  return ws_check_launch(who);
 }
 
 typedef __bf16 bf16x4 __attribute__((ext_vector_type(4)));
diff --git a/wesep_amd/csrc/norm.hip b/wesep_amd/csrc/norm.hip
--- a/wesep_amd/csrc/norm.hip
+++ b/wesep_amd/csrc/norm.hip
@@ -19,17 +19,61 @@
   return !g->band_w && !g->band_off && g->W % 4 == 0 && g->rs % 4 == 0 && g->gs1 % 4 == 0 && g->gs2 % 4 == 0;
 }
 
-template <bool V4>
+struct FilmQuad {
+  f32x4 a, b;
+  long long p0;
+  bool uni;
+  __device__ __forceinline__ FilmQuad(const ws_film_desc& fm, const ws_groups_geom& geo, long long base, int c4) {
+    p0 = base >> 7;
+    const long long r = p0 / fm.rows_per_r;
+    uni = r == (p0 + (long long)(geo.L - 1) * (geo.rs >> 7)) / fm.rows_per_r;
+    a = ws_film_row(fm.a, r, 4 * c4);
+    b = ws_film_row(fm.b, r, 4 * c4);
+  }
+  __device__ __forceinline__ f32x4 operator()(const ws_film_desc& fm, const ws_groups_geom& geo, const f32x4 z, int row, int c4) {
+    if (!uni) {
+      const long long r = (p0 + (long long)row * (geo.rs >> 7)) / fm.rows_per_r;
+      a = ws_film_row(fm.a, r, 4 * c4);
+      b = ws_film_row(fm.b, r, 4 * c4);
+    }
+    return ws_film(z, a, b, fm.a0);
+  }
+};
+
+static int film_check(const ws_film_desc* fm, const ws_groups_geom* g, const char* who);
+
+template <bool V4, bool FILM = false>
 __global__ __launch_bounds__(256) void group_stats_kernel(const float* __restrict__ x,
                                                           const ws_groups_geom geo, float eps,
                                                           float* __restrict__ stats,
-                                                          const int* __restrict__ glen, int glen_div) {
+                                                          const int* __restrict__ glen, int glen_div, const ws_film_desc fm) {
   __shared__ float red[16];
   const int g = blockIdx.x;
   const GroupView v = group_view(geo, g);
   const int n = (glen ? min(max(glen[g / glen_div], 1), geo.L) : geo.L) * v.W;
   const float* xb = x + v.base;
   float s = 0.f;
+  if constexpr (FILM) {
+    FilmQuad fq(fm, geo, v.base, threadIdx.x & 31);
+    for (int i = threadIdx.x; i < (n >> 2); i += 256) {
+      const int row = i >> 5, c4 = i & 31;
+      const f32x4 t = fq(fm, geo, *reinterpret_cast<const f32x4*>(xb + (long long)row * geo.rs + 4 * c4), row, c4);
+      s += (t[0] + t[1]) + (t[2] + t[3]);
+    }
+    const float mean = ws_block_sum(s, red) / (float)n;
+    float q = 0.f;
+    for (int i = threadIdx.x; i < (n >> 2); i += 256) {
+      const int row = i >> 5, c4 = i & 31;
+      const f32x4 t = fq(fm, geo, *reinterpret_cast<const f32x4*>(xb + (long long)row * geo.rs + 4 * c4), row, c4) - mean;
+      q += (t[0] * t[0] + t[1] * t[1]) + (t[2] * t[2] + t[3] * t[3]);
+    }
+    const float var = ws_block_sum(q, red) / (float)n;
+    if (threadIdx.x == 0) {
+      stats[2 * (long long)g] = mean;
+      stats[2 * (long long)g + 1] = 1.f / sqrtf(var + eps);
+    }
+    return;
+  }
   if (V4) {
     const int w4 = v.W >> 2;
     for (int i = threadIdx.x; i < (n >> 2); i += 256) {
@@ -71,18 +115,40 @@
   return WS_OK;
 }
 
+static int film_check(const ws_film_desc* fm, const ws_groups_geom* g, const char* who) {
+  WS_REQUIRE(fm && fm->rows_per_r > 0, "%s: film descriptor / rows_per_r", who);
+  WS_REQUIRE(geom_vec4(g) && g->nbands == 1 && g->W == 128 && g->rs > 0 && g->rs % 128 == 0 && g->gs1 % 128 == 0 &&
+                 g->gs2 % 128 == 0,
+             "%s: the folded affine takes single-band groups of 128-float rows, strides %% 128 == 0", who);
+  return WS_OK;
+}
+static bool film_on(const ws_film_desc* fm) { return fm && (fm->a || fm->b); }
+
 static int group_stats_launch(const char* who, const float* x, const ws_groups_geom* geo, const int* glen, int glen_div,
                               float eps, float* stats, void* stream) {
   int rc = geom_check(geo, who);
   if (rc != WS_OK) return rc;
   WS_REQUIRE(x && stats, "%s: null pointer", who);
+  const ws_film_desc off = {nullptr, nullptr, 0.f, 1};
   if (geom_vec4(geo))
     hipLaunchKernelGGL((group_stats_kernel<true>), dim3(geo->ngroups), dim3(256), 0, (hipStream_t)stream, x,
-                       *geo, eps, stats, glen, glen_div);
+                       *geo, eps, stats, glen, glen_div, off);
   else
     hipLaunchKernelGGL((group_stats_kernel<false>), dim3(geo->ngroups), dim3(256), 0, (hipStream_t)stream, x,
-                       *geo, eps, stats, glen, glen_div);
+                       *geo, eps, stats, glen, glen_div, off);
   return ws_check_launch(who);
+}
+
+extern "C" int ws_group_stats_film(const float* z, const ws_film_desc* film, const ws_groups_geom* geo, float eps, float* stats,
+                                   void* stream) {
+  if (!film_on(film)) return ws_group_stats(z, geo, eps, stats, stream);
+  int rc = geom_check(geo, "ws_group_stats_film");
+  if (rc != WS_OK) return rc;
+  if ((rc = film_check(film, geo, "ws_group_stats_film")) != WS_OK) return rc;
+  WS_REQUIRE(z && stats, "ws_group_stats_film: null pointer");
+  hipLaunchKernelGGL((group_stats_kernel<true, true>), dim3(geo->ngroups), dim3(256), 0, (hipStream_t)stream, z, *geo, eps,
+                     stats, nullptr, 1, *film);
+  return ws_check_launch("ws_group_stats_film");
 }
 
 extern "C" int ws_group_stats(const float* x, const ws_groups_geom* geo, float eps, float* stats,
@@ -96,11 +162,11 @@
   return group_stats_launch("ws_group_stats_len", x, geo, glen, glen_div, eps, stats, stream);
 }
 
-template <bool V4>
+template <bool V4, bool FILM = false>
 __global__ __launch_bounds__(256) void gn_bwd_reduce_kernel(
     const float* __restrict__ x, const float* __restrict__ dxn, const float* __restrict__ stats,
     const float* __restrict__ gamma, const float* const* __restrict__ gamma_tab,
-    const ws_groups_geom geo, float* __restrict__ ab) {
+    const ws_groups_geom geo, float* __restrict__ ab, const ws_film_desc fm) {
   __shared__ float red[16];
   const int g = blockIdx.x;
   const GroupView v = group_view(geo, g);
@@ -108,7 +174,17 @@
   const int n = geo.L * v.W;
   const float mean = stats[2 * (long long)g], rstd = stats[2 * (long long)g + 1];
   float s1 = 0.f, s2 = 0.f;
-  if (V4) {
+  if constexpr (FILM) {
+    FilmQuad fq(fm, geo, v.base, threadIdx.x & 31);
+    for (int i = threadIdx.x; i < (n >> 2); i += 256) {
+      const int row = i >> 5, c4 = i & 31;
+      const long long o = v.base + (long long)row * geo.rs + 4 * c4;
+      const f32x4 dg = *reinterpret_cast<const f32x4*>(dxn + o) * *reinterpret_cast<const f32x4*>(gm + 4 * c4);
+      const f32x4 xh = (fq(fm, geo, *reinterpret_cast<const f32x4*>(x + o), row, c4) - mean) * rstd;
+      s1 += (dg[0] + dg[1]) + (dg[2] + dg[3]);
+      s2 += (dg[0] * xh[0] + dg[1] * xh[1]) + (dg[2] * xh[2] + dg[3] * xh[3]);
+    }
+  } else if (V4) {
     const int w4 = v.W >> 2;
     for (int i = threadIdx.x; i < (n >> 2); i += 256) {
       const int row = i / w4, c4 = i - row * w4;
@@ -140,19 +216,34 @@
   int rc = geom_check(geo, "ws_gn_bwd_reduce");
   if (rc != WS_OK) return rc;
   WS_REQUIRE(x && dxn && stats && ab && (gamma || gamma_tab), "ws_gn_bwd_reduce: null pointer");
+  const ws_film_desc off = {nullptr, nullptr, 0.f, 1};
   if (geom_vec4(geo))
     hipLaunchKernelGGL((gn_bwd_reduce_kernel<true>), dim3(geo->ngroups), dim3(256), 0, (hipStream_t)stream,
-                       x, dxn, stats, gamma, gamma_tab, *geo, ab);
+                       x, dxn, stats, gamma, gamma_tab, *geo, ab, off);
   else
     hipLaunchKernelGGL((gn_bwd_reduce_kernel<false>), dim3(geo->ngroups), dim3(256), 0, (hipStream_t)stream,
-                       x, dxn, stats, gamma, gamma_tab, *geo, ab);
+                       x, dxn, stats, gamma, gamma_tab, *geo, ab, off);
   return ws_check_launch("ws_gn_bwd_reduce");
 }
 
+extern "C" int ws_gn_bwd_reduce_film(const float* z, const ws_film_desc* film, const float* dxn, const float* stats,
+                                     const float* gamma, const ws_groups_geom* geo, float* ab, void* stream) {
+  if (!film_on(film)) return ws_gn_bwd_reduce(z, dxn, stats, gamma, nullptr, geo, ab, stream);
+  int rc = geom_check(geo, "ws_gn_bwd_reduce_film");
+  if (rc != WS_OK) return rc;
+  if ((rc = film_check(film, geo, "ws_gn_bwd_reduce_film")) != WS_OK) return rc;
+  WS_REQUIRE(z && dxn && stats && ab && gamma, "ws_gn_bwd_reduce_film: null pointer");
+  hipLaunchKernelGGL((gn_bwd_reduce_kernel<true, true>), dim3(geo->ngroups), dim3(256), 0, (hipStream_t)stream, z, dxn, stats,
+                     gamma, nullptr, *geo, ab, *film);
+  return ws_check_launch("ws_gn_bwd_reduce_film");
+}
+
+template <bool FILM>
 __global__ __launch_bounds__(256) void gn_bwd_apply_pg_kernel(
     const float* __restrict__ x, const float* dxn, const float* __restrict__ stats, const float* __restrict__ ab,
     const float* __restrict__ gamma, const float* __restrict__ res, const ws_groups_geom geo, float* dx,
-    float* __restrict__ pslab, float* __restrict__ pout, unsigned* counter) {
+    float* __restrict__ pslab, float* __restrict__ pout, unsigned* counter, const ws_film_desc fm, int gpr,
+    float* __restrict__ fslab, float* __restrict__ da, float* __restrict__ db, unsigned* fcounter) {
   __shared__ f32x4 sh[2][8][32];
   const int g = blockIdx.x;
   const GroupView v = group_view(geo, g);
@@ -162,13 +253,28 @@
   const int c4 = threadIdx.x & 31, rl = threadIdx.x >> 5;
   const f32x4 gm = *reinterpret_cast<const f32x4*>(gamma + 4 * c4);
   f32x4 sg = {0.f, 0.f, 0.f, 0.f}, sb = {0.f, 0.f, 0.f, 0.f};
+  f32x4 fa, fb, fsa = {0.f, 0.f, 0.f, 0.f}, fsb = {0.f, 0.f, 0.f, 0.f};
+  const int frow = FILM ? g / gpr : 0;
+  if constexpr (FILM) {
+    fa = ws_film_row(fm.a, frow, 4 * c4);
+    fb = ws_film_row(fm.b, frow, 4 * c4);
+  }
   for (int row = rl; row < geo.L; row += 8) {
     const long long o = v.base + (long long)row * geo.rs + 4 * c4;
     const f32x4 d = *reinterpret_cast<const f32x4*>(dxn + o);
-    const f32x4 xh = (*reinterpret_cast<const f32x4*>(x + o) - mean) * rstd;
+    f32x4 xv = *reinterpret_cast<const f32x4*>(x + o);
+    const f32x4 zv = xv;
+    if constexpr (FILM) xv = ws_film(xv, fa, fb, fm.a0);
+    const f32x4 xh = (xv - mean) * rstd;
     f32x4 r = (d * gm - a0 - xh * a1) * rstd;
     if (res) r += *reinterpret_cast<const f32x4*>(res + o);
-    *reinterpret_cast<f32x4*>(dx + o) = r;
+    if constexpr (FILM) {
+      *reinterpret_cast<f32x4*>(dx + o) = r * (fa + fm.a0);
+      fsa += r * zv;
+      fsb += r;
+    } else {
+      *reinterpret_cast<f32x4*>(dx + o) = r;
+    }
     sg += d * xh;
     sb += d;
   }
@@ -184,6 +290,29 @@
 #pragma unroll
     for (int q = 0; q < 4; ++q) ws_st_agent(o + q, t[q]);
   }
+  if constexpr (FILM) {
+    __syncthreads();
+    sh[0][rl][c4] = fsa;
+    sh[1][rl][c4] = fsb;
+    __syncthreads();
+    if (rl < 2) {
+      f32x4 t = sh[rl][0][c4];
+#pragma unroll
+      for (int r = 1; r < 8; ++r) t += sh[rl][r][c4];
+      float* o = fslab + ((long long)g * 2 + rl) * 128 + 4 * c4;
+#pragma unroll
+      for (int q = 0; q < 4; ++q) ws_st_agent(o + q, t[q]);
+    }
+    if (ws_last_block(fcounter + frow, (unsigned)gpr)) {
+      const int which = threadIdx.x >> 7, col = threadIdx.x & 127;
+      float* dst = which == 0 ? da : db;
+      if (dst) {
+        float t = 0.f;
+        for (int k = 0; k < gpr; ++k) t += ws_ld_agent(fslab + (((long long)frow * gpr + k) * 2 + which) * 128 + col);
+        dst[(long long)frow * 128 + col] = t;
+      }
+    }
+  }
   ws_tree_sum256(pslab, gridDim.x, pout, counter);
 }
 
@@ -194,9 +323,31 @@
   if (rc != WS_OK) return rc;
   WS_REQUIRE(x && dxn && stats && ab && dx && gamma && pslab && pout && counter, "ws_gn_bwd_apply_pg: null pointer");
   WS_REQUIRE(geom_vec4(geo) && geo->nbands == 1 && geo->W == 128, "ws_gn_bwd_apply_pg: single-band groups of 128-float rows");
-  hipLaunchKernelGGL(gn_bwd_apply_pg_kernel, dim3(geo->ngroups), dim3(256), 0, (hipStream_t)stream, x, dxn, stats, ab,
-                     gamma, res, *geo, dx, pslab, pout, counter);
+  const ws_film_desc off = {nullptr, nullptr, 0.f, 1};
+  hipLaunchKernelGGL(gn_bwd_apply_pg_kernel<false>, dim3(geo->ngroups), dim3(256), 0, (hipStream_t)stream, x, dxn, stats, ab,
+                     gamma, res, *geo, dx, pslab, pout, counter, off, 1, nullptr, nullptr, nullptr, nullptr);
   return ws_check_launch("ws_gn_bwd_apply_pg");
+}
+
+extern "C" int ws_gn_bwd_apply_pg_film(const float* z, const ws_film_desc* film, const float* dxn, const float* stats,
+                                       const float* ab, const float* gamma, const float* res, const ws_groups_geom* geo,
+                                       float* dx, float* pslab, float* pout, unsigned* counter, float* fslab, float* da,
+                                       float* db, unsigned* fcounter, void* stream) {
+  if (!film_on(film)) return ws_gn_bwd_apply_pg(z, dxn, stats, ab, gamma, res, geo, dx, pslab, pout, counter, stream);
+  int rc = geom_check(geo, "ws_gn_bwd_apply_pg_film");
+  if (rc != WS_OK) return rc;
+  if ((rc = film_check(film, geo, "ws_gn_bwd_apply_pg_film")) != WS_OK) return rc;
+  WS_REQUIRE(z && dxn && stats && ab && dx && gamma && pslab && pout && counter && fslab && fcounter,
+             "ws_gn_bwd_apply_pg_film: null pointer");
+  WS_REQUIRE((!film->a || da) && (!film->b || db), "ws_gn_bwd_apply_pg_film: da / db go with a / b");
+  WS_REQUIRE(geo->gdiv == 1 && geo->rs == 128 && geo->gs1 == (long long)geo->L * 128 && film->rows_per_r % geo->L == 0 &&
+                 geo->ngroups % (film->rows_per_r / geo->L) == 0,
+             "ws_gn_bwd_apply_pg_film: groups of contiguous rows that tile the rows of a / b (L=%d, rows_per_r=%d, ngroups=%d)",
+             geo->L, film->rows_per_r, geo->ngroups);
+  hipLaunchKernelGGL(gn_bwd_apply_pg_kernel<true>, dim3(geo->ngroups), dim3(256), 0, (hipStream_t)stream, z, dxn, stats, ab,
+                     gamma, res, *geo, dx, pslab, pout, counter, *film, film->rows_per_r / geo->L, fslab, film->a ? da : nullptr,
+                     film->b ? db : nullptr, fcounter);
+  return ws_check_launch("ws_gn_bwd_apply_pg_film");
 }
 
 template <bool V4>
diff --git a/wesep_amd/dev.py b/wesep_amd/dev.py
--- a/wesep_amd/dev.py
+++ b/wesep_amd/dev.py
@@ -206,10 +206,30 @@
         return g
 
 
-def group_stats(x, geo: Geom, stats, eps=GN_EPS, glen=None, glen_div=1):
+class Film(NamedTuple):
+    a: Optional[torch.Tensor]
+    b: Optional[torch.Tensor]
+    a0: float
+    rows_per_r: int
+
+    def c(self):
+        _chk(self.a, "film.a")
+        _chk(self.b, "film.b")
+        f = L.FilmDesc()
+        f.a, f.b, f.a0, f.rows_per_r = _p(self.a), _p(self.b), self.a0, self.rows_per_r
+        return f
+
+
+def group_stats(x, geo: Geom, stats, eps=GN_EPS, glen=None, glen_div=1, film: Optional[Film] = None):
     _chk(x, "x")
     _chk(stats, "stats")
     g = geo.c()
+    if film is not None:
+        if glen is not None:
+            raise L.WesepHipError("group_stats: the folded affine has no per-group lengths")
+        fd = film.c()
+        L.check(L.lib().ws_group_stats_film(_p(x), C.byref(fd), C.byref(g), eps, _p(stats), L.stream_ptr()), "ws_group_stats_film")
+        return
     if glen is not None:
         _chk_lens(glen, -(-geo.ngroups // glen_div), "ws_group_stats_len")
         L.check(L.lib().ws_group_stats_len(_p(x), C.byref(g), _tab(glen), glen_div, eps, _p(stats), L.stream_ptr()),
@@ -242,10 +262,17 @@
     return C.c_void_p(t.data_ptr()) if t is not None else None
 
 
-def gn_bwd_reduce(x, dxn, stats, geo: Geom, ab, gamma=None, gamma_tab=None):
+def gn_bwd_reduce(x, dxn, stats, geo: Geom, ab, gamma=None, gamma_tab=None, film: Optional[Film] = None):
     for n, t in (("x", x), ("dxn", dxn), ("stats", stats), ("ab", ab), ("gamma", gamma)):
         _chk(t, n)
     g = geo.c()
+    if film is not None:
+        if gamma_tab is not None:
+            raise L.WesepHipError("gn_bwd_reduce: the folded affine takes one gamma")
+        fd = film.c()
+        L.check(L.lib().ws_gn_bwd_reduce_film(_p(x), C.byref(fd), _p(dxn), _p(stats), _p(gamma), C.byref(g), _p(ab),
+                                              L.stream_ptr()), "ws_gn_bwd_reduce_film")
+        return
     L.check(L.lib().ws_gn_bwd_reduce(_p(x), _p(dxn), _p(stats), _p(gamma), _tab(gamma_tab),
                                      C.byref(g), _p(ab), L.stream_ptr()), "ws_gn_bwd_reduce")
 
@@ -283,11 +310,23 @@
             and geo.band_off is None and geo.rs % 4 == 0 and geo.gs1 % 4 == 0 and geo.gs2 % 4 == 0)
 
 
-def gn_bwd_apply_pg(x, dxn, stats, ab, geo: Geom, dx, gamma, pslab, pout, counter, res=None):
+def gn_bwd_apply_pg(x, dxn, stats, ab, geo: Geom, dx, gamma, pslab, pout, counter, res=None, film: Optional[Film] = None,
+                    fslab=None, da=None, db=None, fcounter=None):
     for n, t in (("x", x), ("dxn", dxn), ("stats", stats), ("ab", ab), ("gamma", gamma), ("res", res), ("dx", dx),
-                 ("pslab", pslab), ("pout", pout)):
+                 ("pslab", pslab), ("pout", pout), ("fslab", fslab), ("da", da), ("db", db)):
         _chk(t, n)
     g = geo.c()
+    if film is not None:
+        R = geo.ngroups * geo.L // film.rows_per_r
+        if (fslab is None or fslab.numel() < geo.ngroups * 256 or fcounter is None or fcounter.numel() < R
+                or any(t is not None and t.numel() < R * 128 for t in (da, db, film.a, film.b))):
+            raise L.WesepHipError("gn_bwd_apply_pg: the folded affine needs fslab [ngroups, 2, 128], R counter words and "
+                                  "[R, 128] a / b / da / db")
+        fd = film.c()
+        L.check(L.lib().ws_gn_bwd_apply_pg_film(_p(x), C.byref(fd), _p(dxn), _p(stats), _p(ab), _p(gamma), _p(res), C.byref(g),
+                                                _p(dx), _p(pslab), _p(pout), _word(counter), _p(fslab), _p(da), _p(db),
+                                                _word(fcounter), L.stream_ptr()), "ws_gn_bwd_apply_pg_film")
+        return
     L.check(L.lib().ws_gn_bwd_apply_pg(_p(x), _p(dxn), _p(stats), _p(ab), _p(gamma), _p(res), C.byref(g), _p(dx),
                                        _p(pslab), _p(pout), _word(counter), L.stream_ptr()), "ws_gn_bwd_apply_pg")
 
@@ -869,7 +908,7 @@
 
 def gemm_p2b(*, A, lda: int, sm: SeqMap, Wpack, N: int, C_out, K=128, bias=None, A_bl=None, stats=None,
              gamma=None, beta=None, stat_map: Optional[StatMap] = None, run_if=None, amax=None, A_bl16=None, steps=None,
-             steps_div=1):
+             steps_div=1, film: Optional[Film] = None):
     for n, t in (("A", A), ("Wpack", Wpack), ("bias", bias), ("C", C_out), ("A_bl", A_bl), ("stats", stats),
                  ("gamma", gamma), ("beta", beta), ("A_bl16", A_bl16)):
         _chk(t, n)
@@ -887,6 +926,12 @@
         rows = (getattr(sm, "nvalid", 0) or sm.nseq) * sm.L
         _alg("gemm_nt", rows * (4 * K + 4 * N + (4 * K if A_bl is not None else 0) + (2 * K if A_bl16 is not None else 0)) + 4 * N * K,
              2 * rows * N * K)
+    if film is not None:
+        if steps is not None:
+            raise L.WesepHipError("gemm_p2b: the folded affine has no per-sequence step counts")
+        fd = film.c()
+        L.check(L.lib().ws_gemm_p2b_film(C.byref(a), C.byref(fd), L.stream_ptr()), "ws_gemm_p2b_film")
+        return
     if steps is not None:
         _chk_lens(steps, -(-(getattr(sm, "nvalid", 0) or sm.nseq) // steps_div), "ws_gemm_p2b_len")
         L.check(L.lib().ws_gemm_p2b_len(C.byref(a), _tab(steps), steps_div, L.stream_ptr()), "ws_gemm_p2b_len")
@@ -894,7 +939,8 @@
     L.check(L.lib().ws_gemm_p2b(C.byref(a), L.stream_ptr()), "ws_gemm_p2b")
 
 
-def gemm_b2p(*, A, K: int, sm: SeqMap, Wpack, C_out, ldc: int, N=128, bias=None, R=None, a_fmt=0, amax=None, a16_out=None):
+def gemm_b2p(*, A, K: int, sm: SeqMap, Wpack, C_out, ldc: int, N=128, bias=None, R=None, a_fmt=0, amax=None, a16_out=None,
+             film: Optional[Film] = None):
     for n, t in (("A", A), ("Wpack", Wpack), ("bias", bias), ("C", C_out), ("R", R), ("a16_out", a16_out)):
         _chk(t, n)
     if a16_out is not None and a_fmt != 0:
@@ -909,6 +955,10 @@
         rows = (getattr(sm, "nvalid", 0) or sm.nseq) * sm.L
         _alg("gemm_nt", rows * ((4 if a_fmt in (0, 4) else 2) * K + 4 * N * (1 + (R is not None)) + (2 * K if a16_out is not None else 0))
              + 4 * N * K, 2 * rows * N * K)
+    if film is not None:
+        fd = film.c()
+        L.check(L.lib().ws_gemm_b2p_film(C.byref(a), C.byref(fd), L.stream_ptr()), "ws_gemm_b2p_film")
+        return
     L.check(L.lib().ws_gemm_b2p(C.byref(a), L.stream_ptr()), "ws_gemm_b2p")
 
 
diff --git a/wesep_amd/functional.py b/wesep_amd/functional.py
--- a/wesep_amd/functional.py
+++ b/wesep_amd/functional.py
@@ -145,7 +145,16 @@
     return os.environ.get("WESEP_TAIL_FLUSH", "1") != "0"
 
 
-def _resrnn_blk_fwd(z, view, norm_w, norm_b, wparams, cache, grad, frames=None):
+def film_fold(z) -> bool:
+    if os.environ.get("WESEP_FILM_FOLD", "1") == "0" or not (z.is_cuda and torch.cuda.is_available()):
+        return False
+    if resrnn_mode() != "blocked" or z.dim() != 4 or z.shape[3] != 128:
+        return False
+    geo = _view_maps("time", *z.shape)[0]
+    return dev.gn_bwd_apply_pg_ok(geo) and not dev.gn_bwd_fused_ok(geo)
+
+
+def _resrnn_blk_fwd(z, view, norm_w, norm_b, wparams, cache, grad, frames=None, film=None):
     _need_cuda(z, "ResRNN")
     wih_f, whh_f, proj_b = wparams[0], wparams[1], wparams[9]
     R, K, Tf, N = z.shape
@@ -155,18 +164,21 @@
     d = z.device
     geo, smap, seq, _ = _view_maps(view, R, K, Tf, N)
     ragged = frames is not None and view == "time"
+    if film is not None and (view != "time" or frames is not None):
+        raise L.WesepHipError("ResRNN: the folded speaker-fusion affine belongs to the time view of rectangular batches")
+    fk = dict(film=film) if film is not None else {}
     stats = _empty(d, geo.ngroups, 2)
     if ragged:
         dev.group_stats(z, geo, stats, glen=frames, glen_div=K)
     else:
-        dev.group_stats(z, geo, stats)
+        dev.group_stats(z, geo, stats, **fk)
     cache = cache if cache is not None else _NO_CACHE
     sig = cache.begin(wparams)
     plan = make_plan(seq, d, grad, gn_geo=geo, ragged=ragged) if ragged else make_plan(seq, d, grad, gn_geo=geo)
     W = WeightPacks(cache, sig, plan.lmode, plan.pair_rfmt, *wparams[:9])
     steps = dict(steps=(frames, K)) if ragged else {}
     out, saved = blstm_forward(plan, W, z, seq, res=z, bias=proj_b,
-                               norm=dict(stats=stats, gamma=norm_w, beta=norm_b, stat_map=smap), **steps)
+                               norm=dict(stats=stats, gamma=norm_w, beta=norm_b, stat_map=smap), **steps, **fk)
     return out, stats, plan, W, saved
 
 
@@ -174,13 +186,19 @@
 
     @staticmethod
     def forward(ctx, z, dummy, box, cache, view, norm_w, norm_b, wih_f, whh_f, bih_f, bhh_f, wih_r, whh_r, bih_r,
-                bhh_r, proj_w, proj_b):
+                bhh_r, proj_w, proj_b, film_a=None, film_b=None, film_a0=1.0):
         z = z.contiguous()
         d = z.device
+        film = None
+        if film_a is not None or film_b is not None:
+            film_a = film_a.contiguous() if film_a is not None else None
+            film_b = film_b.contiguous() if film_b is not None else None
+            film = dev.Film(film_a, film_b, float(film_a0), z.shape[1] * z.shape[2])
         out, stats, plan, W, saved = _resrnn_blk_fwd(
             z, view, norm_w, norm_b, (wih_f, whh_f, bih_f, bhh_f, wih_r, whh_r, bih_r, bhh_r, proj_w, proj_b), cache,
-            any(ctx.needs_input_grad))
-        ctx.save_for_backward(z, stats, norm_w, *saved)
+            any(ctx.needs_input_grad), film=film)
+        ctx.save_for_backward(z, stats, norm_w, *saved, film_a, film_b)
+        ctx.film_a0 = float(film_a0)
         if view == "time" and box is not None and plan.grad:
             key = (d.type, d.index)
             _TIME_LEFT[key] = _TIME_LEFT.get(key, 0) + 1
@@ -191,7 +209,7 @@
     @staticmethod
     def backward(ctx, dout):
         consume_once(ctx, "ResRNN")
-        z, stats, norm_w, gates, cbuf, hcat, xn, hcat16 = ctx.saved_tensors
+        z, stats, norm_w, gates, cbuf, hcat, xn, hcat16, film_a, film_b = ctx.saved_tensors
         plan, W, box = ctx.plan, ctx.packs, ctx.box
         dout = dout.contiguous()
         R, K, Tf, N = z.shape
@@ -209,7 +227,17 @@
         dxn, dxn_r = blstm_dxn(plan, W, dg, amax, dxn2, seq, P)
         dz = torch.empty_like(z)
         dgb = _empty(d, 2, N)
-        if dev.gn_bwd_fused_ok(geo):
+        da = db = None
+        if film_a is not None or film_b is not None:
+            film = dev.Film(film_a, film_b, ctx.film_a0, K * Tf)
+            ab = _empty(d, geo.ngroups, 2)
+            dev.gn_bwd_reduce(z, dxn, stats, geo, ab, gamma=norm_w, film=film)
+            pslab = _empty(d, geo.ngroups + dev.tree_groups(geo.ngroups), 2, N)
+            da = _empty(d, R, N) if film_a is not None else None
+            db = _empty(d, R, N) if film_b is not None else None
+            dev.gn_bwd_apply_pg(z, dxn, stats, ab, geo, dz, norm_w, pslab, dgb, zero_words(d, 1 + dev.tree_groups(geo.ngroups)),
+                                res=dout, film=film, fslab=_empty(d, geo.ngroups, 2, N), da=da, db=db, fcounter=zero_words(d, R))
+        elif dev.gn_bwd_fused_ok(geo):
             ns2 = min(1024, -(-geo.ngroups // 4))
             pslab = _empty(d, ns2 + dev.tree_groups(ns2), 2, N)
             dev.gn_bwd_fused(z, dxn, stats, geo, norm_w, dz, ns2, pslab, res=dout, pout=dgb,
@@ -229,7 +257,7 @@
             dev.gn_bwd_apply(z, dxn, stats, ab, geo, dz, gamma=norm_w, res=dout)
             dgb = _reduce_new(pslab, ns2, 2 * N, (2, N))
         gd = torch.zeros((), device=d) if box is not None else None
-        return (dz, gd, None, None, None, dgb[0], dgb[1]) + tuple(wg)
+        return (dz, gd, None, None, None, dgb[0], dgb[1]) + tuple(wg) + (da, db, None)
 
 
 def pack_prefetch() -> bool:
@@ -272,7 +300,10 @@
     return WGradCarrierFn.apply(box, *params), box
 
 
-def resrnn(z, view, norm_w, norm_b, *params, carrier=None, cache=None, frames=None):
+def resrnn(z, view, norm_w, norm_b, *params, carrier=None, cache=None, frames=None, film=None):
+    if film is not None and (frames is not None or resrnn_mode() != "blocked" or view != "time"):
+        raise L.WesepHipError("resrnn: film= goes with the time view of the blocked path (functional.film_fold)")
+    fa, fb, fa0 = film if film is not None else (None, None, 1.0)
     if frames is not None:
         if torch.is_grad_enabled() or resrnn_mode() != "blocked":
             raise L.WesepHipError("ResRNN: per-row lengths are an inference feature of the blocked path "
@@ -282,9 +313,9 @@
     if resrnn_mode() != "blocked":
         return ResRNNFn.apply(z, view, norm_w, norm_b, *params)
     if carrier is None:
-        return ResRNNBlkFn.apply(z, None, None, cache, view, norm_w, norm_b, *params)
+        return ResRNNBlkFn.apply(z, None, None, cache, view, norm_w, norm_b, *params, fa, fb, fa0)
     dummy, box = carrier
-    return ResRNNBlkFn.apply(z, dummy, box, cache, view, norm_w, norm_b, *(p.detach() for p in params))
+    return ResRNNBlkFn.apply(z, dummy, box, cache, view, norm_w, norm_b, *(p.detach() for p in params), fa, fb, fa0)
 
 
 def _w2d(w):
diff --git a/wesep_amd/models/bsrnn.py b/wesep_amd/models/bsrnn.py
--- a/wesep_amd/models/bsrnn.py
+++ b/wesep_amd/models/bsrnn.py
@@ -44,11 +44,12 @@
     def make_carrier(self):
         return F_.make_wgrad_carrier(self._wparams())
 
-    def forward(self, z, view="time", carrier=None, frames=None):
+    def forward(self, z, view="time", carrier=None, frames=None, film=None):
         if frames is not None:
             return F_.resrnn(z, view, self.norm.weight, self.norm.bias, *self._wparams(), cache=self._packs, frames=frames)
+        fk = dict(film=film) if film is not None else {}
         return F_.resrnn(z, view, self.norm.weight, self.norm.bias, *self._wparams(), carrier=carrier,
-                         cache=self._packs)
+                         cache=self._packs, **fk)
 
 
 class BSNet(nn.Module):
@@ -60,11 +61,11 @@
         self.band_rnn = ResRNN(self.feature_dim, self.feature_dim * 2, bidirectional)
         self.band_comm = ResRNN(self.feature_dim, self.feature_dim * 2, bidirectional)
 
-    def forward(self, z, dummy: Optional[torch.Tensor] = None, carriers=None, frames=None):
+    def forward(self, z, dummy: Optional[torch.Tensor] = None, carriers=None, frames=None, film=None):
         c_t, c_b = carriers if carriers is not None else (None, None)
         if frames is not None:
             return self.band_comm(self.band_rnn(z, "time", frames=frames), "band")
-        return self.band_comm(self.band_rnn(z, "time", c_t), "band", c_b)
+        return self.band_comm(self.band_rnn(z, "time", c_t, film=film), "band", c_b)
 
 
 class FuseSeparation(nn.Module):
@@ -96,13 +97,18 @@
     def forward(self, z, spk_embedding, nch=None, carriers=None, frames=None):
         if carriers is None:
             carriers = self.make_carriers(z.device)
+        film = None
         for i, layer in enumerate(self.separation):
             if isinstance(layer, BSNet) and frames is not None:
                 z = layer(z, frames=frames)
             elif isinstance(layer, BSNet):
-                z = layer(z, spk_embedding, carriers[i])
+                z, film = layer(z, spk_embedding, carriers[i], film=film), None
             else:
-                z = layer(z, spk_embedding)
+                nxt = self.separation[i + 1] if i + 1 < len(self.separation) else None
+                if isinstance(nxt, BSNet) and frames is None and F_.film_fold(z):
+                    film = layer.affine_operands(spk_embedding)
+                if film is None:
+                    z = layer(z, spk_embedding)
         return z
 
 
diff --git a/wesep_amd/modules/common/speaker.py b/wesep_amd/modules/common/speaker.py
--- a/wesep_amd/modules/common/speaker.py
+++ b/wesep_amd/modules/common/speaker.py
@@ -50,10 +50,13 @@
             nn.init.zeros_(fc.weight)
             nn.init.zeros_(fc.bias)
 
-    def forward(self, embed, x):
+    def operands(self, embed):
         g = F_.LinearFn.apply(embed, self.gamma_fcs[0].weight, self.gamma_fcs[0].bias)
         b = F_.LinearFn.apply(embed, self.beta_fcs[0].weight, self.beta_fcs[0].bias)
-        return F_.AffineFn.apply(x, g, b, 1.0)
+        return g, b, 1.0
+
+    def forward(self, embed, x):
+        return F_.AffineFn.apply(x, *self.operands(embed))
 
 
 class SpeakerFuseLayer(nn.Module):
@@ -70,14 +73,21 @@
         else:
             raise ValueError("Fuse type not defined.")
 
-    def forward(self, x, embed):
+    def affine_operands(self, embed):
+        if self.fuse_type == "concat":
+            return None
         if embed.dim() == 4:
             embed = embed[:, 0, :, 0]
         embed = embed.contiguous()
+        if self.fuse_type == "additive":
+            return None, self.fc(embed), 1.0
+        if self.fuse_type == "multiply":
+            return self.fc(embed), None, 0.0
+        return self.fc.operands(embed)
+
+    def forward(self, x, embed):
         if self.fuse_type == "concat":
-            return F_.ConcatFuseFn.apply(x, embed, self.fc.linear.weight, self.fc.linear.bias)
-        if self.fuse_type == "additive":
-            return F_.AffineFn.apply(x, None, self.fc(embed), 1.0)
-        if self.fuse_type == "multiply":
-            return F_.AffineFn.apply(x, self.fc(embed), None, 0.0)
-        return self.fc(embed, x)
+            if embed.dim() == 4:
+                embed = embed[:, 0, :, 0]
+            return F_.ConcatFuseFn.apply(x, embed.contiguous(), self.fc.linear.weight, self.fc.linear.bias)
+        return F_.AffineFn.apply(x, *self.affine_operands(embed))
```

Measured after the change: 364.5 utterances/s, median of 6. 1.01x the previous value.
